# shuaigroup/Renormalizer

Measured on AMD Instinct MI355X. Metric: TDVP-PS sweep site-updates/sec at (Nsite=50, Dbond=256, dphys=2/16), higher is better.
Workload: dtype c128

## Files before the change

### renormalizer_amd/csrc/mpse_cholqr.hip

```cpp
#include <type_traits>

#include "mpse_device.h"
#include "mpse_internal.h"

typedef double v4d __attribute__((ext_vector_type(4)));

namespace {

struct CqBlk {
  long long ws_off;
  long long part_off;
  long long t_off;
  long long row_off, col_off;
  int mm, nn, P, T;
  int nchunk, rpc;
  int koff, pad;
};

__device__ __forceinline__ v4d mfma(double a, double b, v4d c) {
  return __builtin_amdgcn_mfma_f64_16x16x4f64(a, b, c, 0, 0, 0);
}
__device__ __forceinline__ double readlane_d(double v, int l) {
  const int lo = __builtin_amdgcn_readlane(__double2loint(v), l);
  const int hi = __builtin_amdgcn_readlane(__double2hiint(v), l);
// ... 487 lines not shown
        }
        ar[s][r] = gr;
        ai[s][r] = gi;
      }
    }
  }
  int bad = 0;
  for (int p = 0; p < P; ++p) {
    const int buf = p & 1;
#pragma unroll
    for (int s = 0; s < NS; ++s)
      if (tq[s] == p) {
#pragma unroll
        for (int r = 0; r < 4; ++r) sRow[buf][tc[s] - p][(kq + 4 * r) * 16 + x] = make_double2(ar[s][r], ai[s][r]);
      }
    __syncthreads();
    int badp = 0;
    panel_eliminate<CPLX>(sRow[buf], 16 * (P - p), p, P, nn, Rt, sDinv, last, tid, &badp, dyn ? sThr + 16 * p : nullptr);
    if (badp) bad = 1;
    __syncthreads();
#pragma unroll
    for (int s = 0; s < NS; ++s)
      if (tq[s] > p) {
        const double2* ta = sRow[buf][tq[s] - p];
        const double2* tb = sRow[buf][tc[s] - p];
#pragma unroll
        for (int kk = 0; kk < 4; ++kk) {
          const double2 xv = ta[(4 * kk + kq) * 16 + x], yv = tb[(4 * kk + kq) * 16 + x];
          ar[s] = mfma(-xv.x, yv.x, ar[s]);
          if constexpr (CPLX) {
            ar[s] = mfma(-xv.y, yv.y, ar[s]);
            ai[s] = mfma(-xv.x, yv.y, ai[s]);
            ai[s] = mfma(xv.y, yv.x, ai[s]);
          }
        }
      }
  }
  if (bad) {
    atomicOr(status, 1);
    if (gflag) atomicOr(gflag, 1);
  }
}

template <bool CPLX>
__global__ __launch_bounds__(256) void k_cq_trsm(double* __restrict__ ws, const double* __restrict__ R,
                                                  const double* __restrict__ Rprev, double* __restrict__ Rout,
                                                  const CqBlk* __restrict__ blks, const int* __restrict__ status, int nrb_max,
                                                  int rmul, const int* __restrict__ done) {
  constexpr int E = CPLX ? 2 : 1;
  if (done && done[blockIdx.y]) return;
  const CqBlk B = blks[blockIdx.y];
  const int tid = threadIdx.x, lane = tid & 63, wave = __builtin_amdgcn_readfirstlane(tid >> 6), x = lane & 15, kq = lane >> 4;
  const int P = B.P, nn = B.nn;
  const double* Rt = R + B.t_off * 256 * E;
  __shared__ double sXr[2][16 * 17], sXi[2][16 * 17];
  __shared__ double2 sAcc[4][256];
  if ((int)blockIdx.x >= nrb_max) {
    if (!rmul) return;
    const int t = (int)blockIdx.x - nrb_max;
    if (t >= B.T) return;
    int q, c;
    tile_decode(t, P, q, c);
    const double* Rp = Rprev + B.t_off * 256 * E;
    v4d ar = {0, 0, 0, 0}, ai = {0, 0, 0, 0};
    for (int s = q + wave; s <= c; s += 4) {
      const double* ta = Rt + (long long)tile_index(q, s, P) * 256 * E;
      const double* tb = Rp + (long long)tile_index(s, c, P) * 256 * E;
#pragma unroll
      for (int kk = 0; kk < 4; ++kk) {
        double xr, xi, yr, yi;
        ld2<CPLX>(ta, x * 16 + 4 * kk + kq, xr, xi);
        ld2<CPLX>(tb, (4 * kk + kq) * 16 + x, yr, yi);
        ar = mfma(xr, yr, ar);
        if constexpr (CPLX) {
          ar = mfma(-xi, yi, ar);
          ai = mfma(xr, yi, ai);
          ai = mfma(xi, yr, ai);
        }
      }
    }
#pragma unroll
    for (int r = 0; r < 4; ++r) sAcc[wave][(kq + 4 * r) * 16 + x] = make_double2(ar[r], ai[r]);
    __syncthreads();
    double2 v = sAcc[0][tid];
#pragma unroll
    for (int w = 1; w < 4; ++w) {
      v.x += sAcc[w][tid].x;
      v.y += sAcc[w][tid].y;
    }
    st2<CPLX>(Rout + B.t_off * 256 * E, (long long)t * 256 + tid, v.x, v.y);
    return;
  }
  const int r0 = 16 * blockIdx.x;
  if (r0 >= B.mm) return;
  double* A = ws + B.ws_off * E;
  const long long mm = B.mm;
  const int mode = status[1 + blockIdx.y];
  v4d ar[4], ai[4];
#pragma unroll
  for (int s = 0; s < 4; ++s) {
    const int p = wave + 4 * s;
    ar[s] = v4d{0, 0, 0, 0};
    ai[s] = v4d{0, 0, 0, 0};
    if (p < P) {
      const int col = min(16 * p + x, nn - 1);
#pragma unroll
      for (int r = 0; r < 4; ++r) {
        const int row = min(r0 + kq + 4 * r, B.mm - 1);
        double vr, vi;
        ld2<CPLX>(A, (long long)col * mm + row, vr, vi);
        ar[s][r] = vr;
        ai[s][r] = vi;
      }
    }
  }
  asm volatile("" ::: "memory");
#pragma unroll
  for (int s = 0; s < 4; ++s) {
    const int p = wave + 4 * s;
    if (p < P) {
#pragma unroll
      for (int r = 0; r < 4; ++r)
        if (!(r0 + kq + 4 * r < B.mm && 16 * p + x < nn)) ar[s][r] = ai[s][r] = 0.0;
    }
  }
  auto store_panel = [&](int p, const v4d& vr, const v4d& vi) {
    const int col = 16 * p + x;
    if (col < nn) {
#pragma unroll
      for (int r = 0; r < 4; ++r) {
        const int row = r0 + kq + 4 * r;
        if (row < B.mm) st2<CPLX>(A, (long long)col * mm + row, vr[r], vi[r]);
      }
    }
  };
  if (mode == 1) {
    const int arow = min(r0 + x, B.mm - 1);
    const bool rok = r0 + x < B.mm;
#pragma unroll
    for (int s = 0; s < 4; ++s) {
      const int p = wave + 4 * s;
      if (p >= P) break;
      for (int q = 0; q <= p; ++q) {
        const double* tb = Rt + (long long)tile_index(q, p, P) * 256 * E;
#pragma unroll
        for (int kk = 0; kk < 4; ++kk) {
          const int acol = 16 * q + 4 * kk + kq;
          double xr = 0.0, xi = 0.0, yr, yi;
          ld2<CPLX>(A, (long long)min(acol, nn - 1) * mm + arow, xr, xi);
          if (!(rok && acol < nn)) xr = xi = 0.0;
          ld2<CPLX>(tb, (4 * kk + kq) * 16 + x, yr, yi);
          if (q == p && 4 * kk + kq == x) yr -= 1.0;
          ar[s] = mfma(-xr, yr, ar[s]);
          if constexpr (CPLX) {
            ar[s] = mfma(xi, yi, ar[s]);
            ai[s] = mfma(-xr, yi, ai[s]);
            ai[s] = mfma(-xi, yr, ai[s]);
          }
        }
      }
    }
    __syncthreads();
#pragma unroll
    for (int s = 0; s < 4; ++s)
      if (wave + 4 * s < P) store_panel(wave + 4 * s, ar[s], ai[s]);
    return;
  }
  double rr[16], ri[16];
  auto load_rcol = [&](int q) {
    const double* td = Rt + (long long)tile_index(q, q, P) * 256 * E;
#pragma unroll
    for (int t = 0; t < 16; ++t) ld2<CPLX>(td, t * 16 + x, rr[t], ri[t]);
  };
  for (int q = 0; q < P; ++q) {
    const int owner = q & 3, slot = q >> 2, buf = q & 1;
    if (wave == owner) {
      load_rcol(q);
      asm volatile("" ::: "memory");
      double dj = rr[0];
#pragma unroll
      for (int t = 1; t < 16; ++t) dj = x == t ? rr[t] : dj;
      const double dinv = fast_rcp(dj);
#pragma unroll
      for (int t = 0; t < 16; ++t) {
        if (t >= x) rr[t] = ri[t] = 0.0;
      }
      v4d vr, vi;
      vr = slot == 0 ? ar[0] : slot == 1 ? ar[1] : slot == 2 ? ar[2] : ar[3];
      vi = slot == 0 ? ai[0] : slot == 1 ? ai[1] : slot == 2 ? ai[2] : ai[3];
      auto step = [&](auto tc) {
        constexpr int t = decltype(tc)::value;
        const double dt = row_share<t>(dinv);
#pragma unroll
        for (int r = 0; r < 4; ++r) {
          const double br = row_share<t>(vr[r]) * dt;
          const double bi = CPLX ? row_share<t>(vi[r]) * dt : 0.0;
          vr[r] -= br * rr[t] - bi * ri[t];
          if constexpr (CPLX) vi[r] -= br * ri[t] + bi * rr[t];
        }
      };
      step(std::integral_constant<int, 0>{});
      step(std::integral_constant<int, 1>{});
      step(std::integral_constant<int, 2>{});
      step(std::integral_constant<int, 3>{});
      step(std::integral_constant<int, 4>{});
      step(std::integral_constant<int, 5>{});
      step(std::integral_constant<int, 6>{});
      step(std::integral_constant<int, 7>{});
      step(std::integral_constant<int, 8>{});
      step(std::integral_constant<int, 9>{});
      step(std::integral_constant<int, 10>{});
      step(std::integral_constant<int, 11>{});
      step(std::integral_constant<int, 12>{});
      step(std::integral_constant<int, 13>{});
      step(std::integral_constant<int, 14>{});
#pragma unroll
      for (int r = 0; r < 4; ++r) {
        vr[r] *= dinv;
        vi[r] *= dinv;
      }
#pragma unroll
      for (int r = 0; r < 4; ++r) {
        sXr[buf][(kq + 4 * r) * 17 + x] = vr[r];
        sXi[buf][(kq + 4 * r) * 17 + x] = vi[r];
      }
      store_panel(q, vr, vi);
    }
    lds_barrier();
#pragma unroll
    for (int s = 0; s < 4; ++s) {
      const int p = wave + 4 * s;
      if (p > q && p < P) {
        const double* tb = Rt + (long long)tile_index(q, p, P) * 256 * E;
        double yr[4], yi[4];
#pragma unroll
        for (int kk = 0; kk < 4; ++kk) ld2<CPLX>(tb, (4 * kk + kq) * 16 + x, yr[kk], yi[kk]);
        asm volatile("" ::: "memory");
#pragma unroll
        for (int kk = 0; kk < 4; ++kk) {
          const double xr = sXr[buf][x * 17 + 4 * kk + kq], xi = sXi[buf][x * 17 + 4 * kk + kq];
          ar[s] = mfma(-xr, yr[kk], ar[s]);
          if constexpr (CPLX) {
            ar[s] = mfma(xi, yi[kk], ar[s]);
            ai[s] = mfma(-xr, yi[kk], ai[s]);
            ai[s] = mfma(-xi, yr[kk], ai[s]);
          }
        }
      }
    }
  }
}

template <bool CPLX>
__global__ void k_cq_scatter(double* U, double* Vt, const double* __restrict__ ws, const double* __restrict__ R,
                             const double* __restrict__ R2, long long K,
                             long long ncol, const long long* __restrict__ drows, const long long* __restrict__ dcols,
                             const CqBlk* __restrict__ blks, int herm, const int* __restrict__ status, double* dstat,
                             const int* __restrict__ done, int* __restrict__ words) {
  constexpr int E = CPLX ? 2 : 1;
  const CqBlk B = blks[blockIdx.y];
  if (blockIdx.x == 0 && blockIdx.y == 0 && threadIdx.x == 0) {
    dstat[0] = (double)status[0];
    int n2 = 0;
    for (int b = 0; b < (int)gridDim.y; ++b) n2 += done[b] != 0;
    dstat[1] = (double)n2;
    if (words) {
      atomicAdd(words + 2, (int)gridDim.y);
      atomicAdd(words + 3, n2);
    }
  }
  const double* q = ws + B.ws_off * E;
  const double* Rt = (done[blockIdx.y] ? R2 : R) + B.t_off * 256 * E;
  const long long* rows = drows + B.row_off;
  const long long* cols = dcols + B.col_off;
  const int mm = B.mm, nn = B.nn, k = B.nn;
  const long long koff = B.koff;
  const long long tq = (long long)mm * k, total = tq + (long long)k * nn;
  const long long stride = (long long)gridDim.x * blockDim.x;
  for (long long t = (long long)blockIdx.x * blockDim.x + threadIdx.x; t < total; t += stride) {
    if (t < tq) {
      double vr, vi;
      if (!herm) {
        const int c = (int)(t % k), r = (int)(t / k);
        ld2<CPLX>(q, r + (long long)c * mm, vr, vi);
        st2<CPLX>(U, rows[r] * K + koff + c, vr, vi);
      } else {
        const int r = (int)(t % mm), c = (int)(t / mm);
        ld2<CPLX>(q, r + (long long)c * mm, vr, vi);
        st2<CPLX>(Vt, (koff + c) * ncol + cols[r], vr, -vi);
      }
    } else {
      const long long u = t - tq;
      const int c = (int)(u % nn), i = (int)(u / nn);
      double vr = 0.0, vi = 0.0;
      if (i <= c) ld2<CPLX>(Rt, (long long)tile_index(i >> 4, c >> 4, B.P) * 256 + (i & 15) * 16 + (c & 15), vr, vi);
      if (!herm)
        st2<CPLX>(Vt, (koff + i) * ncol + cols[c], vr, vi);
      else
        st2<CPLX>(U, rows[c] * K + koff + i, vr, -vi);
    }
  }
}

template <bool CPLX>
int cholqr_run(mpse_ctx* ctx, double* ws, const QrBlk* blks, int nblk, const long long* drows, const long long* dcols,
               int herm, void* U, void* Vt, long long K, long long ncol, bool* ok) {
  MPSE_TRY(qr_words(ctx));
  int* gflag = ctx->qr_optimistic ? ctx->qr_words_dev : nullptr;
  constexpr size_t es = CPLX ? 16 : 8;
  std::vector<CqBlk> cb(nblk);
  long long part_tot = 0, t_tot = 0;
  int max_gram = 1, max_T = 1, max_nrb = 1, max_P = 1;
  long long max_sc = 1;
  long long groups = 0;
  for (int b = 0; b < nblk; ++b) {
    const int P2 = ((blks[b].nn + 15) / 16 + 1) / 2;
    groups += P2 * (P2 + 1) / 2;
  }
  for (int b = 0; b < nblk; ++b) {
    CqBlk& c = cb[b];
    c.ws_off = blks[b].ws_off;
    c.mm = blks[b].mm;
    c.nn = blks[b].nn;
    c.P = (c.nn + 15) / 16;
    c.T = c.P * (c.P + 1) / 2;
    c.row_off = blks[b].row_off;
    c.col_off = blks[b].col_off;
    c.koff = blks[b].prm_off;
    c.pad = 0;
    int want = (int)((8LL * ctx->n_cu + groups - 1) / groups);
    if (want < 1) want = 1;
    if (want > 64) want = 64;
    int rpc = (c.mm + want - 1) / want;
    if (rpc < 32) rpc = 32;
    rpc = (rpc + 3) & ~3;
    c.rpc = rpc;
    c.nchunk = (c.mm + rpc - 1) / rpc;
    c.part_off = part_tot;
    c.t_off = t_tot;
    part_tot += (long long)((c.nchunk + 3) / 4) * c.T * 256;
    t_tot += c.T;
    {
      const int P2 = (c.P + 1) / 2, T2 = P2 * (P2 + 1) / 2;
      max_gram = std::max(max_gram, ((c.nchunk + 3) / 4) * T2);
    }
    max_T = std::max(max_T, c.T);
    max_P = std::max(max_P, c.P);
    max_nrb = std::max(max_nrb, (c.mm + 15) / 16);
    max_sc = std::max<long long>(max_sc, (long long)c.mm * c.nn + (long long)c.nn * c.nn);
  }
  const size_t db = (size_t(nblk) * sizeof(CqBlk) + 15) & ~size_t(15);
  const size_t pb = size_t(part_tot) * es, tb = size_t(t_tot) * 256 * es, ib = size_t(t_tot) * 2 * sizeof(double);
  const size_t sb = ((2 * size_t(nblk) + 1) * sizeof(int) + 15) & ~size_t(15);
  TmpBuf M(ctx);
  MPSE_TRY(M.alloc(db + pb + 6 * tb + ib + sb + 16));
  char* base = static_cast<char*>(M.p);
  MPSE_TRY(stage_h2d(ctx, base, cb.data(), size_t(nblk) * sizeof(CqBlk)));
  const CqBlk* dblk = reinterpret_cast<const CqBlk*>(base);
  double* part = reinterpret_cast<double*>(base + db);
  double* G = reinterpret_cast<double*>(base + db + pb);
  double* Rb[5];
  for (int i = 0; i < 5; ++i) Rb[i] = reinterpret_cast<double*>(base + db + pb + (1 + i) * tb);
  double* tinfo = reinterpret_cast<double*>(base + db + pb + 6 * tb);
  int* status = reinterpret_cast<int*>(base + db + pb + 6 * tb + ib);
  const int* done = status + 1 + nblk;
  double* dstat = reinterpret_cast<double*>(base + db + pb + 6 * tb + ib + sb);
  static const double theta = [] {
    const char* e = getenv("MPSE_CHOLQR_THETA");
    return e ? atof(e) : 1e-12;
  }();
  static const double tau = [] {
    const char* e = getenv("MPSE_CHOLQR_TAU");
    return e ? atof(e) : 0.1;
  }();
  const double* racc = nullptr;
  for (int pass = 1; pass <= 3; ++pass) {
    double* Rcur = Rb[pass - 1];
    const int* dn = pass == 3 ? done : nullptr;
    hipLaunchKernelGGL((k_cq_gram<CPLX>), dim3(max_gram, nblk), dim3(256), 0, ctx->stream, (const double*)ws, part, dblk,
                       status, pass == 1 ? 2 * nblk + 1 : 0, dn);
    hipLaunchKernelGGL((k_cq_reduce<CPLX>), dim3(max_T, nblk), dim3(256), 0, ctx->stream, (const double*)part, G, tinfo, dblk,
                       dn);
    if (max_P <= 10)
      hipLaunchKernelGGL((k_cq_chol_rl<CPLX>), dim3(nblk), dim3(512), 0, ctx->stream, (const double*)G,
                         (const double*)tinfo, Rcur, dblk, status, pass, gflag, nblk, theta, tau);
    else
      hipLaunchKernelGGL((k_cq_chol<CPLX>), dim3(nblk), dim3(512), 0, ctx->stream, (const double*)G, (const double*)tinfo,
                         Rcur, dblk, status, pass, gflag, nblk, theta, tau);
    double* Rout = pass == 2 ? Rb[3] : Rb[4];
    const int rmul = pass >= 2 ? 1 : 0;
    const dim3 tg(max_nrb + (rmul ? max_T : 0), nblk);
    hipLaunchKernelGGL((k_cq_trsm<CPLX>), tg, dim3(256), 0, ctx->stream, ws, (const double*)Rcur, racc, Rout, dblk,
                       (const int*)status, max_nrb, rmul, dn);
    racc = pass == 1 ? Rcur : Rout;
  }
  int nb = (int)((max_sc + 255) / 256);
  if (nb > 8192) nb = 8192;
  hipLaunchKernelGGL((k_cq_scatter<CPLX>), dim3(nb, nblk), dim3(256), 0, ctx->stream, (double*)U, (double*)Vt, (const double*)ws,
                     (const double*)Rb[4], (const double*)Rb[3], K, ncol, drows, dcols, dblk, herm, (const int*)status, dstat,
                     done, ctx->qr_words_dev);
  MPSE_HIP(ctx, hipGetLastError());
  if (gflag) {
    *ok = true;
    return MPSE_OK;
  }
  MPSE_TRY(publish_and_wait(ctx, dstat, 1, mpse_ctx::PIN_QR_STATUS));
  *ok = ctx->pinned[mpse_ctx::PIN_QR_STATUS] == 0.0;
  return MPSE_OK;
}

}

bool cholqr_eligible(const mpse_ctx* ctx, const QrBlk* blks, int nblk) {
  static const int env_mode = [] {
    const char* e = getenv("MPSE_CHOLQR");
    return e ? atoi(e) : 1;
  }();
  const int mode = ctx->qr_scheme >= 0 ? ctx->qr_scheme : env_mode;
  static const int min_rows = [] {
    const char* e = getenv("MPSE_CHOLQR_MINROWS");
    return e ? atoi(e) : 256;
  }();
  if (mode == 0 || nblk <= 0) return false;
  int max_mm = 0, max_nn = 0;
  for (int b = 0; b < nblk; ++b) {
    if (blks[b].mm < blks[b].nn || blks[b].k != blks[b].nn || blks[b].nn > 256) return false;
    max_mm = std::max(max_mm, blks[b].mm);
    max_nn = std::max(max_nn, blks[b].nn);
  }
  if (mode >= 2) return true;
  return max_mm >= min_rows && max_nn >= 96;
}

int cholqr_blocks(mpse_ctx* ctx, bool cplx, double* ws, const QrBlk* blks, int nblk, const long long* drows,
                  const long long* dcols, int herm, void* U, void* Vt, long long K, long long ncol, bool* ok) {
  *ok = false;
  if (cplx) return cholqr_run<true>(ctx, ws, blks, nblk, drows, dcols, herm, U, Vt, K, ncol, ok);
  return cholqr_run<false>(ctx, ws, blks, nblk, drows, dcols, herm, U, Vt, K, ncol, ok);
}
```

### renormalizer_amd/csrc/mpse_core.hip

```cpp
#include "mpse_internal.h"
#include "mpse_plans.h"

int mpse_fail(mpse_ctx* ctx, int code, const char* fmt, ...) {
  if (ctx) {
    va_list ap;
    va_start(ap, fmt);
    vsnprintf(ctx->err, sizeof(ctx->err), fmt, ap);
    va_end(ap);
  }
  return code;
}

__global__ __launch_bounds__(256) void k_zero8(unsigned long long* dst, long long n) {
  for (long long i = (long long)blockIdx.x * 256 + threadIdx.x; i < n; i += (long long)gridDim.x * 256) dst[i] = 0ull;
}
__global__ __launch_bounds__(256) void k_copy8(unsigned long long* dst, const unsigned long long* __restrict__ src,
                                               long long n) {
  for (long long i = (long long)blockIdx.x * 256 + threadIdx.x; i < n; i += (long long)gridDim.x * 256) dst[i] = src[i];
}

__global__ __launch_bounds__(256) void k_zero8x2(unsigned long long* a, long long na, unsigned long long* b, long long nb) {
  for (long long i = (long long)blockIdx.x * 256 + threadIdx.x; i < na + nb; i += (long long)gridDim.x * 256) {
    if (i < na)
      a[i] = 0ull;
    else
      b[i - na] = 0ull;
  }
}

int device_zero2(mpse_ctx* ctx, void* a, size_t abytes, void* b, size_t bbytes) {
  if (((reinterpret_cast<uintptr_t>(a) | reinterpret_cast<uintptr_t>(b) | abytes | bbytes) & 7) != 0 || !abytes || !bbytes) {
    MPSE_TRY(device_zero(ctx, a, abytes));
    return device_zero(ctx, b, bbytes);
  }
  const long long na = (long long)(abytes / 8), nb = (long long)(bbytes / 8);
  long long blocks = (na + nb + 255) / 256;
  if (blocks > 2048) blocks = 2048;
  hipLaunchKernelGGL(k_zero8x2, dim3((unsigned)blocks), dim3(256), 0, ctx->stream, static_cast<unsigned long long*>(a), na,
                     static_cast<unsigned long long*>(b), nb);
  MPSE_HIP(ctx, hipGetLastError());
  return MPSE_OK;
}

int device_zero(mpse_ctx* ctx, void* dst, size_t bytes) {
  if (!bytes) return MPSE_OK;
  if ((reinterpret_cast<uintptr_t>(dst) & 7) == 0 && (bytes & 7) == 0) {
    const long long n = (long long)(bytes / 8);
    long long blocks = (n + 255) / 256;
    if (blocks > 2048) blocks = 2048;
    hipLaunchKernelGGL(k_zero8, dim3((unsigned)blocks), dim3(256), 0, ctx->stream, static_cast<unsigned long long*>(dst), n);
    MPSE_HIP(ctx, hipGetLastError());
    return MPSE_OK;
  }
  MPSE_HIP(ctx, hipMemsetAsync(dst, 0, bytes, ctx->stream));
  return MPSE_OK;
}

int stage_h2d(mpse_ctx* ctx, void* dst, const void* src_host, size_t bytes) {
  if (!bytes) return MPSE_OK;
  if (!ctx->stage || bytes > ctx->stage_size / 4) return mpse_memcpy_h2d(ctx, dst, src_host, bytes);
  const size_t need = (bytes + 255) & ~size_t(255);
  if (ctx->stage_pos + need > ctx->stage_size) {
    MPSE_HIP(ctx, hipStreamSynchronize(ctx->stream));
    ctx->stage_pos = 0;
  }
  char* slot = ctx->stage + ctx->stage_pos;
  memcpy(slot, src_host, bytes);
  if (ctx->stage_dev && (reinterpret_cast<uintptr_t>(dst) & 7) == 0 && (bytes & 7) == 0 && bytes <= (size_t(1) << 20)) {
    const size_t words = bytes / 8;
    ctx->stage_pos += need;
    __sync_synchronize();
    long long blocks = (long long)((words + 255) / 256);
    if (blocks > 256) blocks = 256;
    hipLaunchKernelGGL(k_copy8, dim3((unsigned)blocks), dim3(256), 0, ctx->stream, static_cast<unsigned long long*>(dst),
                       reinterpret_cast<const unsigned long long*>(ctx->stage_dev + (slot - ctx->stage)),
                       (long long)words);
    MPSE_HIP(ctx, hipGetLastError());
    return MPSE_OK;
  }
  ctx->stage_pos += need;
  MPSE_HIP(ctx, hipMemcpyAsync(dst, slot, bytes, hipMemcpyHostToDevice, ctx->stream));
  return MPSE_OK;
}

void prof_drain(mpse_ctx* ctx) {
  for (auto& r : ctx->prof_pending) {
    float ms = 0.f;
    if (hipEventElapsedTime(&ms, r.e0, r.e1) == hipSuccess) {
      ctx->prof_ms[r.variant] += ms;
      ctx->prof_flops[r.variant] += r.flops;
      ctx->prof_bytes[r.variant] += r.bytes;
      ctx->prof_launches[r.variant] += 1;
    }
    ctx->prof_free_events.push_back(r.e0);
    ctx->prof_free_events.push_back(r.e1);
  }
  ctx->prof_pending.clear();
}

bool prof_begin(mpse_ctx* ctx, int variant, double flops, double bytes, mpse_ctx::ProfRec* rec) {
  if (!ctx->prof_on || (variant != 6 && ctx->prof_counter++ % ctx->prof_stride != 0)) return false;
  auto get_event = [&](hipEvent_t* e) {
    if (!ctx->prof_free_events.empty()) {
      *e = ctx->prof_free_events.back();
      ctx->prof_free_events.pop_back();
      return true;
    }
    return hipEventCreate(e) == hipSuccess;
  };
  if (!get_event(&rec->e0)) return false;
  if (!get_event(&rec->e1)) {
    ctx->prof_free_events.push_back(rec->e0);
    return false;
  }
  rec->variant = variant;
  rec->flops = flops;
  rec->bytes = bytes;
  if (hipEventRecord(rec->e0, ctx->stream) != hipSuccess) {
    ctx->prof_free_events.push_back(rec->e0);
    ctx->prof_free_events.push_back(rec->e1);
    return false;
  }
  return true;
}

void prof_end(mpse_ctx* ctx, const mpse_ctx::ProfRec& rec) {
  (void)hipEventRecord(rec.e1, ctx->stream);
  ctx->prof_pending.push_back(rec);
}

namespace {
__global__ void k_copy16(double2* __restrict__ dst, const double2* __restrict__ src, long long n) {
  const long long stride = (long long)gridDim.x * blockDim.x;
  for (long long i = (long long)blockIdx.x * blockDim.x + threadIdx.x; i < n; i += stride) dst[i] = src[i];
}
}

static void defer_update_hold(mpse_ctx* ctx) {
  const bool hold = ctx->defer_recording >= 0 || !ctx->defer_ops[0].empty() || !ctx->defer_ops[1].empty();
  std::lock_guard<std::mutex> lock(ctx->pool_mu);
  ctx->defer_hold = hold;
  if (hold) return;
  for (void* p : ctx->defer_frees) {
    auto it = ctx->live.find(p);
    if (it == ctx->live.end()) continue;
    ctx->free_blocks.emplace(it->second, p);
    ctx->in_use_bytes -= it->second;
    ctx->live.erase(it);
  }
  ctx->defer_frees.clear();
}

int defer_replay(mpse_ctx* ctx, int status) {
  const int list = ctx->defer_armed;
  if (list < 0) return status;
  ctx->defer_armed = -1;
  std::vector<std::function<int()>> ops;
  ops.swap(ctx->defer_ops[list]);
  if (status == MPSE_OK)
    for (auto& f : ops) {
      status = f();
      if (status != MPSE_OK) break;
    }
  ops.clear();
  defer_update_hold(ctx);
  return status;
}

extern "C" {

int mpse_prof_enable(mpse_ctx* ctx, int on) {
  if (!ctx) return MPSE_ERR_ARG;
  MPSE_HIP(ctx, hipStreamSynchronize(ctx->stream));
  prof_drain(ctx);
  ctx->prof_on = on != 0;
  ctx->prof_stride = on > 1 ? on : 1;
  ctx->prof_counter = 0;
  return MPSE_OK;
}

int mpse_prof_reset(mpse_ctx* ctx) {
  if (!ctx) return MPSE_ERR_ARG;
  MPSE_HIP(ctx, hipStreamSynchronize(ctx->stream));
  prof_drain(ctx);
  for (int i = 0; i < mpse_ctx::PROF_NVAR; ++i) {
    ctx->prof_ms[i] = ctx->prof_flops[i] = ctx->prof_bytes[i] = 0;
    ctx->prof_launches[i] = 0;
  }
  ctx->prof_svd_sweeps = 0;
  if (ctx->prof_ktiles) {
    MPSE_HIP(ctx, hipMemsetAsync(ctx->prof_ktiles, 0, 4 * sizeof(unsigned long long), ctx->stream));
    MPSE_HIP(ctx, hipStreamSynchronize(ctx->stream));
  }
  return MPSE_OK;
}

int mpse_prof_get_ktiles(mpse_ctx* ctx, int variant, int64_t* ktiles) {
  if (!ctx || !ktiles || variant < 0 || variant > 3) return MPSE_ERR_ARG;
  MPSE_BIND(ctx);
  *ktiles = 0;
  if (!ctx->prof_ktiles) return MPSE_OK;
  unsigned long long v[4];
  MPSE_HIP(ctx, hipMemcpyAsync(v, ctx->prof_ktiles, sizeof(v), hipMemcpyDeviceToHost, ctx->stream));
  MPSE_HIP(ctx, hipStreamSynchronize(ctx->stream));
  *ktiles = (int64_t)v[variant];
  return MPSE_OK;
}

int mpse_prof_get_svd_sweeps(mpse_ctx* ctx, int64_t* sweeps) {
  if (!ctx || !sweeps) return MPSE_ERR_ARG;
  *sweeps = ctx->prof_svd_sweeps;
  return MPSE_OK;
}

int mpse_prof_get(mpse_ctx* ctx, int variant, double* total_ms, double* total_flops, double* total_bytes,
                  int64_t* launches) {
  if (!ctx || variant < 0 || variant >= mpse_ctx::PROF_NVAR) return MPSE_ERR_ARG;
  MPSE_HIP(ctx, hipStreamSynchronize(ctx->stream));
  prof_drain(ctx);
  if (variant == 0 && ctx->gemm_trace) {
    const char* path = getenv("MPSE_GEMM_TRACE");
    unsigned long long n = 0;
    if (path && hipMemcpy(&n, ctx->gemm_trace, sizeof(n), hipMemcpyDeviceToHost) == hipSuccess) {
      if (n > GEMM_TRACE_CAP) n = GEMM_TRACE_CAP;
      std::vector<unsigned long long> rec(size_t(n) * GEMM_TRACE_WORDS);
      if (n && hipMemcpy(rec.data(), ctx->gemm_trace + 1, rec.size() * sizeof(unsigned long long), hipMemcpyDeviceToHost) == hipSuccess) {
        if (FILE* fh = fopen(path, "wb")) {
          fwrite(rec.data(), sizeof(unsigned long long), rec.size(), fh);
          fclose(fh);
        }
      }
    }
  }
  if (total_ms) *total_ms = ctx->prof_ms[variant];
  if (total_flops) *total_flops = ctx->prof_flops[variant];
  if (total_bytes) *total_bytes = ctx->prof_bytes[variant];
  if (launches) *launches = ctx->prof_launches[variant];
  return MPSE_OK;
}

const char* mpse_version(void) { return "mpsengine 0.1 (gfx950)"; }

const char* mpse_last_error(const mpse_ctx* ctx) { return ctx ? ctx->err : "null context"; }

int mpse_ctx_create(int device, mpse_ctx** out) {
  if (!out) return MPSE_ERR_ARG;
  *out = nullptr;
  int ndev = 0;
  if (hipGetDeviceCount(&ndev) != hipSuccess || ndev <= 0) return MPSE_ERR_HIP;
  if (device < 0 || device >= ndev) return MPSE_ERR_ARG;
  mpse_ctx* ctx = new mpse_ctx();
  ctx->device = device;
  if (hipSetDevice(device) != hipSuccess) {
    delete ctx;
    return MPSE_ERR_HIP;
  }
  hipDeviceProp_t prop;
  if (hipGetDeviceProperties(&prop, device) == hipSuccess) {
    ctx->n_cu = prop.multiProcessorCount;
    if (ctx->n_cu > 0) mpse_plan::fold_cus() = ctx->n_cu;
    snprintf(ctx->dev_name, sizeof(ctx->dev_name), "%s (%s)", prop.name, prop.gcnArchName);
  }
  if (hipStreamCreateWithFlags(&ctx->stream, hipStreamNonBlocking) != hipSuccess ||
      hipHostMalloc((void**)&ctx->pinned, mpse_ctx::PIN_DOUBLES * sizeof(double)) != hipSuccess ||
      hipMalloc((void**)&ctx->dscratch, (size_t(1) << 16) * sizeof(double)) != hipSuccess ||
      hipMalloc((void**)&ctx->prof_ktiles, 4 * sizeof(unsigned long long)) != hipSuccess ||
      hipHostMalloc((void**)&ctx->stage, size_t(8) << 20) != hipSuccess) {
    delete ctx;
    return MPSE_ERR_HIP;
  }
  (void)hipMemsetAsync(ctx->dscratch + (size_t(1) << 16) - 8, 0, 8 * sizeof(double), ctx->stream);
  (void)hipMemsetAsync(ctx->prof_ktiles, 0, 4 * sizeof(unsigned long long), ctx->stream);
  (void)hipStreamSynchronize(ctx->stream);
  const char* pin_map = getenv("MPSE_PINNED_MAP");
  if ((pin_map && pin_map[0] == '0') || hipHostGetDevicePointer((void**)&ctx->pinned_dev, ctx->pinned, 0) != hipSuccess)
    ctx->pinned_dev = nullptr;
  {
    if (hipHostGetDevicePointer((void**)&ctx->stage_dev, ctx->stage, 0) != hipSuccess)
      ctx->stage_dev = nullptr;
    (void)hipGetLastError();
  }
  ctx->pinned[mpse_ctx::PIN_SEQ] = 0.0;
  ctx->stage_size = size_t(8) << 20;
  *out = ctx;
  return MPSE_OK;
}

static int pool_trim_locked(mpse_ctx* ctx) {
  MPSE_HIP(ctx, hipStreamSynchronize(ctx->stream));
  for (auto& kv : ctx->free_blocks) {
    (void)hipFree(kv.second);
    ctx->pool_bytes -= kv.first;
  }
  ctx->free_blocks.clear();
  return MPSE_OK;
}

int mpse_pool_trim(mpse_ctx* ctx) {
  if (!ctx) return MPSE_ERR_ARG;
  MPSE_BIND(ctx);
  std::lock_guard<std::mutex> lock(ctx->pool_mu);
  return pool_trim_locked(ctx);
}

int mpse_ctx_destroy(mpse_ctx* ctx) {
  if (!ctx) return MPSE_ERR_ARG;
  (void)hipSetDevice(ctx->device);
  (void)hipStreamSynchronize(ctx->stream);
  prof_drain(ctx);
  for (auto e : ctx->prof_free_events) (void)hipEventDestroy(e);
  for (auto& kv : ctx->free_blocks) (void)hipFree(kv.second);
  for (auto& kv : ctx->live) (void)hipFree(kv.first);
  if (ctx->pinned) (void)hipHostFree(ctx->pinned);
  if (ctx->stage) (void)hipHostFree(ctx->stage);
  if (ctx->dscratch) (void)hipFree(ctx->dscratch);
  if (ctx->prof_ktiles) (void)hipFree(ctx->prof_ktiles);
  if (ctx->stream) (void)hipStreamDestroy(ctx->stream);
  delete ctx;
  return MPSE_OK;
}

int mpse_sync(mpse_ctx* ctx) {
  if (!ctx) return MPSE_ERR_ARG;
  MPSE_BIND(ctx);
  MPSE_HIP(ctx, hipStreamSynchronize(ctx->stream));
  if (!ctx->prof_pending.empty()) prof_drain(ctx);
  return MPSE_OK;
}

int mpse_device_info(mpse_ctx* ctx, char* name, size_t name_len, int* n_cu, void** stream) {
  if (!ctx) return MPSE_ERR_ARG;
  if (name && name_len) snprintf(name, name_len, "%s", ctx->dev_name);
  if (n_cu) *n_cu = ctx->n_cu;
  if (stream) *stream = (void*)ctx->stream;
  return MPSE_OK;
}

static size_t bucket_of(size_t bytes) {
  if (bytes < 256) return 256;
  if (bytes <= (size_t(1) << 20)) return (bytes + 255) & ~size_t(255);
  size_t p = size_t(1) << 20;
  while ((p << 1) <= bytes) p <<= 1;
  size_t step = p >> 3;
  return ((bytes + step - 1) / step) * step;
}

int mpse_malloc(mpse_ctx* ctx, size_t bytes, void** dptr) {
  if (!ctx || !dptr) return MPSE_ERR_ARG;
  MPSE_BIND(ctx);
  std::lock_guard<std::mutex> lock(ctx->pool_mu);
  size_t b = bucket_of(bytes);
  auto it = ctx->free_blocks.find(b);
  void* p = nullptr;
  if (it != ctx->free_blocks.end()) {
    p = it->second;
    ctx->free_blocks.erase(it);
  } else {
    hipError_t e = hipMalloc(&p, b);
    ++ctx->n_device_allocs;
    if (e != hipSuccess) {
      (void)hipGetLastError();
      pool_trim_locked(ctx);
      e = hipMalloc(&p, b);
      if (e != hipSuccess) {
        (void)hipGetLastError();
        *dptr = nullptr;
        return mpse_fail(ctx, MPSE_ERR_OOM, "hipMalloc(%zu) failed: %s (pool %zu B, in use %zu B)", b,
                         hipGetErrorString(e), ctx->pool_bytes, ctx->in_use_bytes);
      }
    }
    ctx->pool_bytes += b;
  }
  ctx->live[p] = b;
  ctx->in_use_bytes += b;
  *dptr = p;
  return MPSE_OK;
}

int mpse_free(mpse_ctx* ctx, void* dptr) {
  if (!ctx) return MPSE_ERR_ARG;
  if (!dptr) return MPSE_OK;
  std::lock_guard<std::mutex> lock(ctx->pool_mu);
  auto it = ctx->live.find(dptr);
  if (it == ctx->live.end()) return mpse_fail(ctx, MPSE_ERR_ARG, "mpse_free: unknown pointer %p", dptr);
  if (!ctx->wsite_info.empty()) ctx->wsite_info.erase(dptr);
  if (ctx->defer_hold) {
    ctx->defer_frees.push_back(dptr);
    return MPSE_OK;
  }
  ctx->free_blocks.emplace(it->second, dptr);
  ctx->in_use_bytes -= it->second;
  ctx->live.erase(it);
  return MPSE_OK;
}


int mpse_defer_begin(mpse_ctx* ctx, int list) {
  if (!ctx || list < 0 || list > 1) return MPSE_ERR_ARG;
  if (ctx->defer_recording >= 0) return mpse_fail(ctx, MPSE_ERR_ARG, "mpse_defer_begin: already recording");
  if (ctx->defer_armed == list) return mpse_fail(ctx, MPSE_ERR_ARG, "mpse_defer_begin: list %d is armed", list);
  ctx->defer_ops[list].clear();
  ctx->defer_recording = list;
  defer_update_hold(ctx);
  return MPSE_OK;
}

int mpse_defer_end(mpse_ctx* ctx) {
  if (!ctx) return MPSE_ERR_ARG;
  if (ctx->defer_recording < 0) return mpse_fail(ctx, MPSE_ERR_ARG, "mpse_defer_end: not recording");
  ctx->defer_recording = -1;
  defer_update_hold(ctx);
  return MPSE_OK;
}

int mpse_defer_arm(mpse_ctx* ctx, int list) {
  if (!ctx || list < 0 || list > 1) return MPSE_ERR_ARG;
  if (ctx->defer_recording >= 0) return mpse_fail(ctx, MPSE_ERR_ARG, "mpse_defer_arm: still recording");
  ctx->defer_armed = list;
  return MPSE_OK;
}

int mpse_defer_discard(mpse_ctx* ctx) {
  if (!ctx) return MPSE_ERR_ARG;
  ctx->defer_ops[0].clear();
  ctx->defer_ops[1].clear();
  ctx->defer_recording = ctx->defer_armed = -1;
  defer_update_hold(ctx);
  return MPSE_OK;
}

int mpse_defer_run(mpse_ctx* ctx, int list) {
  if (!ctx || list < 0 || list > 1) return MPSE_ERR_ARG;
  if (ctx->defer_recording >= 0) return mpse_fail(ctx, MPSE_ERR_ARG, "mpse_defer_run: still recording");
  MPSE_BIND(ctx);
  ctx->defer_armed = list;
  return defer_replay(ctx, MPSE_OK);
}


int mpse_mem_info(mpse_ctx* ctx, size_t* pool_bytes, size_t* in_use_bytes, size_t* device_free,
                  size_t* device_total) {
  if (!ctx) return MPSE_ERR_ARG;
  MPSE_BIND(ctx);
  if (pool_bytes) *pool_bytes = ctx->pool_bytes;
  if (in_use_bytes) *in_use_bytes = ctx->in_use_bytes;
  size_t f = 0, t = 0;
  MPSE_HIP(ctx, hipMemGetInfo(&f, &t));
  if (device_free) *device_free = f;
  if (device_total) *device_total = t;
  return MPSE_OK;
}

int mpse_memcpy_h2d(mpse_ctx* ctx, void* dst, const void* src_host, size_t bytes) {
  if (!ctx || (bytes && (!dst || !src_host))) return MPSE_ERR_ARG;
  MPSE_BIND(ctx);
  if (!bytes) return MPSE_OK;
  wsite_written(ctx, dst, bytes);
  MPSE_HIP(ctx, hipMemcpyAsync(dst, src_host, bytes, hipMemcpyHostToDevice, ctx->stream));
  MPSE_HIP(ctx, hipStreamSynchronize(ctx->stream));
  return MPSE_OK;
}

int mpse_memcpy_d2h(mpse_ctx* ctx, void* dst_host, const void* src, size_t bytes) {
  if (!ctx || (bytes && (!dst_host || !src))) return MPSE_ERR_ARG;
  MPSE_BIND(ctx);
  if (!bytes) return MPSE_OK;
  MPSE_HIP(ctx, hipMemcpyAsync(dst_host, src, bytes, hipMemcpyDeviceToHost, ctx->stream));
  MPSE_HIP(ctx, hipStreamSynchronize(ctx->stream));
  return MPSE_OK;
}

int mpse_memcpy_d2d(mpse_ctx* ctx, void* dst, const void* src, size_t bytes) {
  if (!ctx || (bytes && (!dst || !src))) return MPSE_ERR_ARG;
  MPSE_BIND(ctx);
  if (!bytes) return MPSE_OK;
  wsite_written(ctx, dst, bytes);
  if (((reinterpret_cast<uintptr_t>(dst) | reinterpret_cast<uintptr_t>(src)) & 15) == 0 && (bytes & 15) == 0) {
    const size_t n = bytes / 16;
    size_t blocks = (n + 255) / 256;
    if (blocks > 4096) blocks = 4096;
    hipLaunchKernelGGL(k_copy16, dim3((unsigned)blocks), dim3(256), 0, ctx->stream, reinterpret_cast<double2*>(dst),
                       reinterpret_cast<const double2*>(src), (long long)n);
    MPSE_HIP(ctx, hipGetLastError());
    return MPSE_OK;
  }
  MPSE_HIP(ctx, hipMemcpyAsync(dst, src, bytes, hipMemcpyDeviceToDevice, ctx->stream));
  return MPSE_OK;
}

int mpse_memcpy_2d(mpse_ctx* ctx, void* dst, size_t dpitch, const void* src, size_t spitch, size_t width_bytes,
                   size_t height) {
  if (!ctx || ((width_bytes && height) && (!dst || !src))) return MPSE_ERR_ARG;
  MPSE_BIND(ctx);
  if (!width_bytes || !height) return MPSE_OK;
  wsite_written(ctx, dst, dpitch * (height - 1) + width_bytes);
  MPSE_HIP(ctx, hipMemcpy2DAsync(dst, dpitch, src, spitch, width_bytes, height, hipMemcpyDeviceToDevice, ctx->stream));
  return MPSE_OK;
}

int mpse_memset_zero(mpse_ctx* ctx, void* dst, size_t bytes) {
  if (!ctx || (bytes && !dst)) return MPSE_ERR_ARG;
  MPSE_BIND(ctx);
  wsite_written(ctx, dst, bytes);
  return device_zero(ctx, dst, bytes);
}

}

namespace {
__global__ void k_publish(const double* __restrict__ src, double* dst, int count, volatile double* seq_slot, double seq) {
  for (int i = threadIdx.x; i < count; i += blockDim.x) dst[i] = src[i];
  __threadfence_system();
  __syncthreads();
  if (threadIdx.x == 0) {
    *seq_slot = seq;
    __threadfence_system();
  }
}
}

int publish_wait_seq(mpse_ctx* ctx, double seq, const double* dsrc, int count, int slot) {
  volatile double* flag = ctx->pinned + mpse_ctx::PIN_SEQ;
  for (long long spins = 0; *flag != seq; ++spins) {
    if (spins > 2000000000LL || ((spins & 0xfffff) == 0xfffff && hipStreamQuery(ctx->stream) == hipSuccess && *flag != seq)) {
      MPSE_HIP(ctx, hipStreamSynchronize(ctx->stream));
      MPSE_HIP(ctx, hipMemcpy(ctx->pinned + slot, dsrc, size_t(count) * sizeof(double), hipMemcpyDeviceToHost));
      return MPSE_OK;
    }
  }
  __sync_synchronize();
  return MPSE_OK;
}

PublishAt publish_target(mpse_ctx* ctx, bool wait_here, int slot) {
  if (!wait_here || !ctx->pinned_dev) return PublishAt{nullptr, nullptr, 0.0};
  return PublishAt{ctx->pinned_dev + slot, ctx->pinned_dev + mpse_ctx::PIN_SEQ, double(++ctx->publish_seq)};
}

static int publish_wait(mpse_ctx* ctx, const PublishAt& at, const void* dsrc, size_t stride, int B, int W, int slot) {
  if (at.seq != 0.0) {
    MPSE_TRY(publish_wait_seq(ctx, at.seq, static_cast<const double*>(dsrc), W, slot));
    if (B == 1 || ctx->pinned[mpse_ctx::PIN_SEQ] == at.seq) return MPSE_OK;
  }
  const size_t row = size_t(W) * sizeof(double);
  if (B == 1)
    MPSE_HIP(ctx, hipMemcpyAsync(ctx->pinned + slot, dsrc, row, hipMemcpyDeviceToHost, ctx->stream));
  else
    MPSE_HIP(ctx, hipMemcpy2DAsync(ctx->pinned + slot, row, dsrc, stride, row, size_t(B), hipMemcpyDeviceToHost, ctx->stream));
  MPSE_HIP(ctx, hipStreamSynchronize(ctx->stream));
  return MPSE_OK;
}

int publish_collect(mpse_ctx* ctx, const PublishAt& at, const void* dsrc, size_t stride, int B, int W, int slot,
                    void* host_out) {
  MPSE_TRY(publish_wait(ctx, at, dsrc, stride, B, W, slot));
  if (ctx->prof_pending.size() > 2048) prof_drain(ctx);
  memcpy(host_out, ctx->pinned + slot, size_t(B) * W * sizeof(double));
  return MPSE_OK;
}

int publish_and_wait(mpse_ctx* ctx, const double* dsrc, int count, int slot) {
  if (count < 0 || count > 1024 || slot < 0 || slot + count > mpse_ctx::PIN_SLOTS_END)
    return mpse_fail(ctx, MPSE_ERR_ARG, "publish: range");
  const PublishAt at = publish_target(ctx, true, slot);
  if (at.pub) {
    hipLaunchKernelGGL(k_publish, dim3(1), dim3(64), 0, ctx->stream, dsrc, at.pub, count, at.seq_slot, at.seq);
    MPSE_HIP(ctx, hipGetLastError());
  }
  return publish_wait(ctx, at, dsrc, 0, 1, count, slot);
}
```

### renormalizer_amd/csrc/mpse_gemm.hip

```cpp
#include <cstdlib>

#include "mpse_device.h"
#include "mpse_internal.h"
#include "mpse_plans.h"

typedef double v4d __attribute__((ext_vector_type(4)));

static unsigned long long* gemm_trace_ptr(const mpse_ctx* ctx) {
  static const bool f0_only = [] {
    const char* e = getenv("MPSE_GEMM_TRACE_ONLY");
    return e && e[0] == 'f';
  }();
  return (ctx->prof_on && !f0_only) ? ctx->gemm_trace : nullptr;
}

namespace {

struct IdxMap {
  long long s_hi, s_lo;
  int ext, lo;
};

constexpr int GMAX_GRP = 8, GMAX_SEG = 4, GMAX_MIX = 8;
struct GMix {
// ... 597 lines not shown
  int kt_done = 0;
  if constexpr (KS && MPSE_GEMM_PIPE) {
    int nk = kt_end;
    if (kt < kt_end) {
      stage_to_lds(0);
      nk = next_kt(kt + 1);
      if (nk < kt_end) {
        load_tile(nk);
      }
      lds_barrier();
      if (g.trace) tr2 = __builtin_readcyclecounter();
      read_frag(0, 0);
    }
    const bool any = kt < kt_end;
    while (nk < kt_end) {
      ++kt_done;
      read_frag(1, 1);
      mfma_group(0);
      read_frag(0, 2);
      mfma_group(1);
      read_frag(1, 3);
      mfma_group(0);
      lds_barrier();
      mfma_group_staging(1);
      const int after = next_kt(nk + 1);
      if (after < kt_end) load_tile(after);
      kt = nk;
      nk = after;
      lds_barrier();
      read_frag(0, 0);
    }
    if (any) {
      ++kt_done;
      read_frag(1, 1);
      mfma_group(0);
      read_frag(0, 2);
      mfma_group(1);
      read_frag(1, 3);
      mfma_group(0);
      mfma_group(1);
    }
  } else {
  while (kt < kt_end) {
    ++kt_done;
    __syncthreads();
    if (g.trace && kt_done == 1) tr2 = __builtin_readcyclecounter();
    stage_to_lds(0);
    __syncthreads();
    const int nk = next_kt(kt + 1);
    if (nk < kt_end) {
      load_tile(nk);
    }
    kt = nk;

    read_frag(0, 0);
#pragma unroll
    for (int kk = 0; kk < BK / 4; ++kk) {
      const int cb = kk & 1;
      if (kk + 1 < BK / 4) read_frag(cb ^ 1, kk + 1);
      mfma_group(cb);
    }
  }
  }

  if (g.trace) tr3 = __builtin_readcyclecounter();
  struct TraceEnd {
    const GemmArgs& g;
    unsigned long long t0, rt0, &t1, &t2, &t3;
    int tid;
    int& ktd;
    __device__ ~TraceEnd() {
      if (g.trace && tid == 0) trace_record(g, CA, CB, t0, rt0, t1, t2, t3, ktd);
    }
  } trace_end{g, tr0, rt0, tr1, tr2, tr3, tid, kt_done};
  if (g.kt_counter && tid == 0 && kt_done) atomicAdd(g.kt_counter, (unsigned long long)kt_done);
  if constexpr (M3) {
#pragma unroll
    for (int i = 0; i < WI; ++i)
#pragma unroll
      for (int j = 0; j < 2; ++j) {
        acc_im[i][j] = acc_im[i][j] - acc_re[i][j] - acc_t2[i][j];
        acc_re[i][j] = acc_re[i][j] - acc_t2[i][j];
      }
  }
  if (g.ksplit > 1) {
    double* wsb = g.ws + (long long)bs * g.M * g.N * EC;
#pragma unroll
    for (int j = 0; j < 2; ++j) {
      const int gj = tn * TBN + wn * 32 + j * 16 + (lane & 15);
      if (gj >= g.N) continue;
#pragma unroll
      for (int i = 0; i < WI; ++i)
#pragma unroll
        for (int r = 0; r < 4; ++r) {
          const int gi = tm * TBM + wm * WROWS + i * 16 + (lane >> 4) + 4 * r;
          if (gi >= g.M) continue;
          double* p = wsb + ((long long)gi * g.N + gj) * EC;
          if constexpr (CC)
            *reinterpret_cast<double2*>(p) = make_double2(acc_re[i][j][r], acc_im[i][j][r]);
          else
            *p = acc_re[i][j][r];
        }
    }
    return;
  }
  double dre = 0.0, dim = 0.0;
  constexpr bool PRE = CA && CB;
  double2 pre_c[PRE ? WI : 1][2][4], pre_y[PRE ? WI : 1][2][4];
  const bool need_c = GRP ? (gp.use_beta != 0 && half == 0) : g.use_beta != 0, need_y = g.dot_y != nullptr;
  bool mix_on = false;
  if constexpr (GRP && PRE) mix_on = need_c && g.gg.nmix > 0 && grp == g.gg.mix_grp;
  if constexpr (GRP && PRE) {
    if (mix_on) {
      const int d = g.gg.mix_d;
      __syncthreads();
      for (int x = tid; x < g.gg.nmix * BM; x += NT) {
        const GMix& m = g.gg.mix[x / BM];
        const int sg = (x % BM) % d, e = sg + m.delta;
        double w = 0.0;
        if (e >= 0 && e < d) w = g.gg.mix_w[(((long long)m.b * d + sg) * d + e) * g.gg.mix_wr + m.f];
        smem[x] = w;
      }
      __syncthreads();
#pragma unroll
      for (int j = 0; j < 2; ++j)
#pragma unroll
        for (int i = 0; i < WI; ++i)
#pragma unroll
          for (int r = 0; r < 4; ++r) pre_c[i][j][r] = make_double2(0.0, 0.0);
      for (int t = 0; t < g.gg.nmix; ++t) {
        const double* src = g.gg.mix[t].src;
        const int delta = g.gg.mix[t].delta;
        double2 v[WI][2][4];
#pragma unroll
        for (int j = 0; j < 2; ++j) {
          const int gj = min(tn * TBN + wn * 32 + j * 16 + (lane & 15), g.N - 1);
#pragma unroll
          for (int i = 0; i < WI; ++i)
#pragma unroll
            for (int r = 0; r < 4; ++r) {
              const int gi = tm * TBM + wm * WROWS + i * 16 + (lane >> 4) + 4 * r + delta;
              const int gc = min(max(gi, 0), g.M - 1);
              v[i][j][r] = *reinterpret_cast<const double2*>(src + ((long long)gc * g.gg.mix_ld + gj) * 2);
            }
        }
#pragma unroll
        for (int i = 0; i < WI; ++i)
#pragma unroll
          for (int r = 0; r < 4; ++r) {
            const double w = smem[t * BM + wm * WROWS + i * 16 + (lane >> 4) + 4 * r];
#pragma unroll
            for (int j = 0; j < 2; ++j) {
              pre_c[i][j][r].x = w != 0.0 ? fma(w, v[i][j][r].x, pre_c[i][j][r].x) : pre_c[i][j][r].x;
              pre_c[i][j][r].y = w != 0.0 ? fma(w, v[i][j][r].y, pre_c[i][j][r].y) : pre_c[i][j][r].y;
            }
          }
      }
    }
  }
  if (PRE && (need_c || need_y)) {
#pragma unroll
    for (int j = 0; j < 2; ++j) {
      const int gj = min(tn * TBN + wn * 32 + j * 16 + (lane & 15), g.N - 1);
      const long long coffn = idx_off(g.nC, gj);
      const long long cinn = g.Cin ? idx_off(g.nCin, gj) : 0;
#pragma unroll
      for (int i = 0; i < WI; ++i)
#pragma unroll
        for (int r = 0; r < 4; ++r) {
          const int gi = min(tm * TBM + wm * WROWS + i * 16 + (lane >> 4) + 4 * r, g.M - 1);
          const long long co = idx_off(g.mC, gi) + coffn;
          if (need_c && !mix_on) {
            const double* pin = g.Cin ? g.Cin + (idx_off(g.mCin, gi) + cinn) * EC : C + co * EC;
            if constexpr (CC)
              pre_c[i][j][r] = *reinterpret_cast<const double2*>(pin);
            else
              pre_c[i][j][r] = make_double2(*pin, 0.0);
          }
          if (need_y) {
            if constexpr (CC)
              pre_y[i][j][r] = reinterpret_cast<const double2*>(g.dot_y)[co];
            else
              pre_y[i][j][r] = make_double2(g.dot_y[co], 0.0);
          }
        }
    }
  }
  constexpr bool HAND = GRP && PRE && WI == 1;
  bool hand = false;
  auto hslot = [&]() { return smem + 1024 + (((wm >> 1) * 2 + wn) * 64 + lane) * 2; };
  if constexpr (HAND) {
    hand = g.gg.dot4 != 0 && need_y;
    if (hand) __syncthreads();
  }
#pragma unroll
  for (int j = 0; j < 2; ++j) {
    const int gj = tn * TBN + wn * 32 + j * 16 + (lane & 15);
    if (gj >= g.N) continue;
    if constexpr (HAND) {
      if (hand) {
        if (wm & 1) __syncthreads();
        if ((wm & 1) || j > 0) dre = hslot()[0], dim = hslot()[1];
      }
    }
    const long long coffn = idx_off(g.nC, gj);
#pragma unroll
    for (int i = 0; i < WI; ++i) {
#pragma unroll
      for (int r = 0; r < 4; ++r) {
        const int gi = tm * TBM + wm * WROWS + i * 16 + (lane >> 4) + 4 * r;
        if (gi >= g.M) continue;
        const long long co = idx_off(g.mC, gi) + coffn;
        double* p = C + co * EC;
        const double xr = acc_re[i][j][r];
        if constexpr (CC) {
          const double xi = acc_im[i][j][r];
          double2 o;
          o.x = g.alpha_re * xr - g.alpha_im * xi;
          o.y = g.alpha_re * xi + g.alpha_im * xr;
          if (need_c) {
            double2 c0;
            if constexpr (PRE)
              c0 = pre_c[i][j][r];
            else
              c0 = *reinterpret_cast<const double2*>(g.Cin ? g.Cin + (idx_off(g.mCin, gi) + idx_off(g.nCin, gj)) * EC : C + co * EC);
            o.x += g.beta_re * c0.x - g.beta_im * c0.y;
            o.y += g.beta_re * c0.y + g.beta_im * c0.x;
          }
          *reinterpret_cast<double2*>(p) = o;
          if (need_y) {
            if constexpr (PRE)
              dot_acc(dre, dim, o, pre_y[i][j][r]);
            else
              dot_acc(dre, dim, o, reinterpret_cast<const double2*>(g.dot_y)[co]);
          }
        } else {
          double o = g.alpha_re * xr;
          if (need_c) o += g.beta_re * (g.Cin ? g.Cin[idx_off(g.mCin, gi) + idx_off(g.nCin, gj)] : *p);
          *p = o;
          if (need_y) dre += o * g.dot_y[co];
        }
      }
    }
    if constexpr (HAND) {
      if (hand) {
        if (!((wm & 1) && j == 1)) hslot()[0] = dre, hslot()[1] = dim;
        if (!(wm & 1)) {
          __syncthreads();
          if (j == 0) __syncthreads();
        } else if (j == 0) {
          __syncthreads();
        }
      }
    }
  }
  if constexpr (HAND) {
    if (hand && !(wm & 1)) dre = dim = 0.0;
  }
  if constexpr (WS == 2) {
    if (g.dot_y) {
      __shared__ double s_dot[2 * (NT / 64)];
      dre = wave_sum(dre);
      dim = wave_sum(dim);
      if (lane == 0) {
        s_dot[2 * wave] = dre;
        s_dot[2 * wave + 1] = dim;
      }
      __syncthreads();
      dre = dim = 0.0;
#pragma unroll
      for (int w = 0; w < NT / 64; ++w) {
        dre += s_dot[2 * w];
        dim += s_dot[2 * w + 1];
      }
      if (tid == 0) {
        const long long slot = (long long)bs * ntile + (long long)tm * g.tiles_n + tn;
        g.dot_part[2 * slot] = dre;
        g.dot_part[2 * slot + 1] = dim;
      }
    }
  }
}

__device__ __forceinline__ void bitonic_desc(unsigned* key, int tid, int n) {
  for (int size = 2; size <= n; size <<= 1)
    for (int stride = size >> 1; stride > 0; stride >>= 1) {
      if (tid < (n >> 1)) {
        const int lo = 2 * tid - (tid & (stride - 1)), hi = lo + stride;
        const bool desc = (lo & size) == 0;
        const unsigned a = key[lo], b = key[hi];
        if ((a < b) == desc) {
          key[lo] = b;
          key[hi] = a;
        }
      }
      __syncthreads();
    }
}
__device__ __forceinline__ int pow2_at_least(int x) {
  int n = 2;
  while (n < x) n <<= 1;
  return n;
}
__global__ __launch_bounds__(1024) void k_tile_order(const unsigned long long* __restrict__ amask,
                                                       const unsigned long long* __restrict__ bmask, int nkw, int nkt,
                                                       int tiles_m, int tiles_n, int by_die, int* __restrict__ perm,
                                                       const int* __restrict__ skip, const GemmGroups gg,
                                                       unsigned char* __restrict__ flags_out, int flags_pitch,
                                                       int om_M, int om_N) {
  if (skip && *skip) return;
  __shared__ unsigned key[2048], ckey[2048];
  __shared__ int colw[2048];
  __shared__ unsigned char die_of[2048], dead[2048];
  const int ntile = tiles_m * tiles_n, tid = threadIdx.x;
  const bool part = by_die && tiles_n % 8 == 0 && tiles_n <= 2048;
  for (int c = tid; c < 2048; c += 1024) colw[c] = 0;
  __syncthreads();
  for (int i = tid; i < 2048; i += 1024) {
    unsigned cnt = 0;
    dead[i] = 0;
    if (i < ntile) {
      const int tm = i / tiles_n, tn = i - tm * tiles_n;
      if (gg.ngrp > 0) {
        const int grp = tm / gg.tiles_m_grp, tml = tm - grp * gg.tiles_m_grp;
        const GGrp& G = gg.g[grp];
        const bool off = gg.omask && !mpse_plan::out_tile_live(gg.omask, gg.om_pitch, gg.om_d, om_N, om_M, tm, tn);
        dead[i] = off ? 1 : 0;
        for (int q = 0; q < G.nseg; ++q)
          for (int l = 0; l < gg.nkt_seg; ++l) {
            unsigned v = off ? 0 : 1;
            if (G.seg[q].am) v &= G.seg[q].am[(long long)tml * gg.am_pitch + l];
            if (G.seg[q].bm) v &= G.seg[q].bm[(long long)tn * gg.bm_pitch + l];
            cnt += v;
            if (flags_out) flags_out[(long long)i * flags_pitch + q * gg.nkt_seg + l] = (unsigned char)v;
          }
        if (flags_out)
          for (int l = G.nseg * gg.nkt_seg; l < flags_pitch; ++l) flags_out[(long long)i * flags_pitch + l] = 0;
      } else {
        for (int w = 0; w < nkw; ++w) {
          unsigned long long x = 0x0101010101010101ull;
          if (amask) x &= amask[(long long)tm * nkw + w];
          if (bmask) x &= bmask[(long long)tn * nkw + w];
          const int valid = nkt - 8 * w;
          if (valid < 8) x &= (1ull << (8 * valid)) - 1ull;
          cnt += __popcll(x);
        }
      }
      if (part) atomicAdd(&colw[tn], (int)cnt);
    }
    key[i] = cnt;
  }
  __syncthreads();
  if (part) {
    for (int c = tid; c < 2048; c += 1024) ckey[c] = c < tiles_n ? ((unsigned)colw[c] << 11) | (unsigned)(2047 - c) : 0u;
    __syncthreads();
    bitonic_desc(ckey, tid, pow2_at_least(tiles_n));
    for (int r = tid; r < tiles_n; r += 1024) {
      const int c = 2047 - (int)(ckey[r] & 2047u), r16 = r & 15;
      die_of[c] = (unsigned char)(r16 < 8 ? r16 : 15 - r16);
    }
    __syncthreads();
  }
  for (int i = tid; i < 2048; i += 1024) {
    unsigned k = 0;
    if (i < ntile) {
      const unsigned die = part ? die_of[i % tiles_n] : 0u;
      k = (die << 28) | (key[i] << 16) | (unsigned)(0xFFFF - i);
    }
    key[i] = k;
  }
  __syncthreads();
  bitonic_desc(key, tid, pow2_at_least(ntile));
  const int per_die = ntile / 8;
  for (int i = tid; i < ntile; i += 1024) {
    const int s = part ? (7 - (i & 7)) * per_die + (i >> 3) : i;
    const int t = 0xFFFF - (int)(key[s] & 0xFFFFu);
    perm[i] = dead[t] ? ~t : t;
  }
}

template <bool CC>
__global__ __launch_bounds__(256) void k_splitk_reduce(const GemmArgs g, int batch) {
  constexpr int EC = CC ? 2 : 1;
  if (g.skip && *g.skip) return;
  const long long mn = (long long)g.M * g.N;
  const int rows = g.M * batch;
  double dre = 0.0, dim = 0.0;
  for (int row = blockIdx.y; row < rows; row += gridDim.y) {
    const int b = row / g.M;
    const int i = row - b * g.M;
    const double* wrow = g.ws + ((long long)b * g.ksplit * mn + (long long)i * g.N) * EC;
    double* crow = g.C + ((long long)b * g.sbC + idx_off(g.mC, i)) * EC;
    for (int j = blockIdx.x * 256 + threadIdx.x; j < g.N; j += gridDim.x * 256) {
      const double* w = wrow + (long long)j * EC;
      double xr = 0, xi = 0;
      int s = 0;
      for (; s + 4 <= g.ksplit; s += 4) {
        if constexpr (CC) {
          const double2 v0 = *reinterpret_cast<const double2*>(w + (long long)s * mn * EC);
          const double2 v1 = *reinterpret_cast<const double2*>(w + (long long)(s + 1) * mn * EC);
          const double2 v2 = *reinterpret_cast<const double2*>(w + (long long)(s + 2) * mn * EC);
          const double2 v3 = *reinterpret_cast<const double2*>(w + (long long)(s + 3) * mn * EC);
          xr += v0.x;
          xi += v0.y;
          xr += v1.x;
          xi += v1.y;
          xr += v2.x;
          xi += v2.y;
          xr += v3.x;
          xi += v3.y;
        } else {
          const double v0 = w[(long long)s * mn], v1 = w[(long long)(s + 1) * mn];
          const double v2 = w[(long long)(s + 2) * mn], v3 = w[(long long)(s + 3) * mn];
          xr += v0;
          xr += v1;
          xr += v2;
          xr += v3;
        }
      }
      for (; s < g.ksplit; ++s) {
        if constexpr (CC) {
          const double2 v = *reinterpret_cast<const double2*>(w + (long long)s * mn * EC);
          xr += v.x;
          xi += v.y;
        } else {
          xr += w[(long long)s * mn];
        }
      }
      const long long co = idx_off(g.nC, j);
      double* p = crow + co * EC;
      const double* pin = g.Cin ? g.Cin + (idx_off(g.mCin, i) + idx_off(g.nCin, j)) * EC : p;
      if constexpr (CC) {
        double2 o = make_double2(g.alpha_re * xr - g.alpha_im * xi, g.alpha_re * xi + g.alpha_im * xr);
        if (g.use_beta) {
          const double2 c0 = *reinterpret_cast<const double2*>(pin);
          o.x += g.beta_re * c0.x - g.beta_im * c0.y;
          o.y += g.beta_re * c0.y + g.beta_im * c0.x;
        }
        *reinterpret_cast<double2*>(p) = o;
        if (g.dot_y) dot_acc(dre, dim, o, reinterpret_cast<const double2*>(g.dot_y)[idx_off(g.mC, i) + co]);
      } else {
        double o = g.alpha_re * xr;
        if (g.use_beta) o += g.beta_re * (*pin);
        *p = o;
        if (g.dot_y) dre += o * g.dot_y[idx_off(g.mC, i) + co];
      }
    }
  }
  if (g.dot_y) {
    block_allsum2(dre, dim);
    if (threadIdx.x == 0) {
      const long long bid = (long long)blockIdx.y * gridDim.x + blockIdx.x;
      g.dot_part[2 * bid] = dre;
      g.dot_part[2 * bid + 1] = dim;
    }
  }
}

struct OccOperand {
  const double* base;
  IdxMap rmap, kmap;
  int nrows, tiles, cplx, kfast;
  long long sb;
  unsigned char* flags;
};
__global__ __launch_bounds__(256) void k_tile_occ(OccOperand oa, OccOperand ob, int K, int nkw, int batch,
                                                  const int* skip) {
  if (skip && *skip) return;
  const int wave = threadIdx.x >> 6, lane = threadIdx.x & 63;
  const int kt = blockIdx.x * 4 + wave, t = blockIdx.y;
  const bool second = (int)blockIdx.z >= batch;
  const OccOperand& o = second ? ob : oa;
  const int b = second ? blockIdx.z - batch : blockIdx.z;
  if (t >= o.tiles || kt * BK >= K) return;
  const int E = o.cplx ? 2 : 1;
  const double* base = o.base + (long long)b * o.sb * E;
  bool nz = false;
  if (o.kfast) {
    const int k = kt * BK + (lane & 15);
    const bool kin = k < K;
    const long long ko = idx_off(o.kmap, kin ? k : K - 1);
    double v0[16], v1[16];
#pragma unroll
    for (int i = 0; i < 16; ++i) {
      const int r = min(t * BM + i * 4 + (lane >> 4), o.nrows - 1);
      const double* q = base + (idx_off(o.rmap, r) + ko) * E;
      v0[i] = q[0];
      v1[i] = o.cplx ? q[1] : 0.0;
    }
#pragma unroll
    for (int i = 0; i < 16; ++i) {
      const bool in = (t * BM + i * 4 + (lane >> 4)) < o.nrows && kin;
      nz |= in && (v0[i] != 0.0 || v1[i] != 0.0);
    }
  } else {
    const int r = t * BM + lane;
    if (r < o.nrows) {
      const double* p = base + idx_off(o.rmap, r) * E;
      double v0[16], v1[16];
#pragma unroll
      for (int i = 0; i < 16; ++i) {
        const int k = min(kt * BK + i, K - 1);
        const double* q = p + idx_off(o.kmap, k) * E;
        v0[i] = q[0];
        v1[i] = o.cplx ? q[1] : 0.0;
      }
#pragma unroll
      for (int i = 0; i < 16; ++i) nz |= (kt * BK + i < K) && (v0[i] != 0.0 || v1[i] != 0.0);
    }
  }
  const bool any = __ballot(nz) != 0ull;
  if (lane == 0) o.flags[((long long)b * o.tiles + t) * nkw * 8 + kt] = any ? 1 : 0;
}

bool to_map(const mpse_index& s, IdxMap* m) {
  if (s.ext < 0 || s.ext > 0x7fffffffLL) return false;
  m->ext = (int)s.ext;
  long long lo = s.lo_ext <= 0 ? 1 : s.lo_ext;
  m->s_hi = s.s_hi;
  m->s_lo = s.s_lo;
  if (lo >= s.ext) {
    m->s_hi = 0;
  } else if (lo == 1) {
    m->s_lo = s.s_hi;
    m->s_hi = 0;
    lo = s.ext;
  } else if (s.s_hi == lo * s.s_lo) {
    m->s_hi = 0;
    lo = s.ext;
  }
  if (lo >= s.ext) lo = 0x7fffffffLL;
  m->lo = (int)lo;
  return true;
}

inline bool is_single(const IdxMap& m) { return m.lo == 0x7fffffff; }

template <bool CPLX>
__global__ __launch_bounds__(256) void k_transpose_inner(double* out, const double* in, long long d0, int d1,
                                                         int d2, int conj) {
  constexpr int E = CPLX ? 2 : 1;
  __shared__ double tile[32][33 * E];
  const int tx = threadIdx.x & 31, ty = threadIdx.x >> 5;
  const int t1 = (d1 + 31) / 32, t2 = (d2 + 31) / 32;
  long long bid = blockIdx.x;
  const long long b0 = bid / ((long long)t1 * t2);
  const int rem = (int)(bid - b0 * t1 * t2);
  const int by = rem / t2, bx = rem - by * t2;
  const double* src = in + b0 * (long long)d1 * d2 * E;
  double* dst = out + b0 * (long long)d1 * d2 * E;
  for (int yy = ty; yy < 32; yy += 8) {
    int y = by * 32 + yy, x = bx * 32 + tx;
    if (y < d1 && x < d2) {
      const double* p = src + ((long long)y * d2 + x) * E;
      tile[yy][tx * E] = p[0];
      if (CPLX) tile[yy][tx * E + 1] = conj ? -p[1] : p[1];
    }
  }
  __syncthreads();
  for (int yy = ty; yy < 32; yy += 8) {
    int x = bx * 32 + yy, y = by * 32 + tx;
    if (y < d1 && x < d2) {
      double* p = dst + ((long long)x * d1 + y) * E;
      p[0] = tile[tx][yy * E];
      if (CPLX) p[1] = tile[tx][yy * E + 1];
    }
  }
}

inline int n_cu_of(const mpse_ctx* ctx) { return ctx->n_cu > 0 ? ctx->n_cu : 256; }

long long fastest(const IdxMap& m) { return m.ext <= 1 ? (long long)1 << 60 : (m.s_lo < 0 ? -m.s_lo : m.s_lo); }

bool span_ok(const IdxMap& m, const IdxMap& k, bool cplx) {
  if (m.s_hi < 0 || m.s_lo < 0 || k.s_hi < 0 || k.s_lo < 0) return false;
  auto span = [](const IdxMap& x) {
    if (x.ext <= 1) return 0.0;
    if (x.lo == 0x7fffffff) return double(x.ext - 1) * double(x.s_lo);
    return double((x.ext - 1) / x.lo) * double(x.s_hi) + double(x.lo - 1) * double(x.s_lo);
  };
  return (span(m) + span(k) + 1.0) * (cplx ? 16.0 : 8.0) < 4.0e9;
}
bool fast_ok(const GemmArgs& g, bool ca, bool cb) { return span_ok(g.mA, g.kA, ca) && span_ok(g.nB, g.kB, cb); }

bool fill_maps(GemmArgs& g, const mpse_index& ma, const mpse_index& ka, const mpse_index& kb, const mpse_index& nb,
               const mpse_index& mc, const mpse_index& nc) {
  if (!to_map(ma, &g.mA) || !to_map(ka, &g.kA) || !to_map(kb, &g.kB) || !to_map(nb, &g.nB) || !to_map(mc, &g.mC) ||
      !to_map(nc, &g.nC))
    return false;
  g.M = g.mA.ext, g.N = g.nB.ext, g.K = g.kA.ext;
  g.tiles_m = g.mtiles_m = (g.M + BM - 1) / BM;
  g.tiles_n = g.mtiles_n = (g.N + BN - 1) / BN;
  g.a_kfast = fastest(g.kA) <= fastest(g.mA);
  g.b_kfast = fastest(g.kB) <= fastest(g.nB);
  return true;
}

SolveScope::OccKey occ_key(const void* p, const IdxMap& rm, const IdxMap& km, long long sb, long long batch, bool cplx) {
  SolveScope::OccKey k;
  memset(&k, 0, sizeof(k));
  k.ptr = p;
  k.r_ext = rm.ext, k.r_lo = rm.lo, k.r_shi = rm.s_hi, k.r_slo = rm.s_lo;
  k.k_ext = km.ext, k.k_lo = km.lo, k.k_shi = km.s_hi, k.k_slo = km.s_lo;
  k.sb = sb, k.nrows = rm.ext, k.tiles = (rm.ext + BM - 1) / BM, k.nkw = ((km.ext + BK - 1) / BK + 7) / 8;
  k.batch = (int)batch, k.K = km.ext, k.cplx = cplx ? 1 : 0;
  return k;
}
size_t occ_bytes(const SolveScope::OccKey& k) { return size_t(k.batch) * k.tiles * k.nkw * 8; }

struct OccMask {
  void* mask = nullptr;
  bool scan = false;
  bool stable = true;
};
int occ_mask_source(mpse_ctx* ctx, SolveScope* keep, const SolveScope::OccKey& key, const void* given, void* tmp,
                    OccMask* m) {
  m->stable = keep || given;
  if (keep)
    for (const auto& e : keep->occ_cache)
      if (memcmp(&e.key, &key, sizeof(key)) == 0) {
        m->mask = e.mask;
        return MPSE_OK;
      }
  m->scan = !given;
  if (given) {
    m->mask = const_cast<void*>(given);
  } else if (keep) {
    MPSE_TRY(mpse_malloc(ctx, occ_bytes(key), &m->mask));
    keep->occ_cache.push_back({key, m->mask});
  } else {
    m->mask = tmp;
  }
  return MPSE_OK;
}
OccOperand occ_operand(const SolveScope::OccKey& k, const IdxMap& rm, const IdxMap& km, int kfast, const OccMask& m) {
  return OccOperand{static_cast<const double*>(k.ptr), rm, km, k.nrows, m.scan ? k.tiles : 0, k.cplx, kfast, k.sb,
                    static_cast<unsigned char*>(m.mask)};
}

int perm_source(mpse_ctx* ctx, SolveScope* keep, SolveScope::PermEntry key, size_t bytes, TmpBuf& tmp, int** perm,
                bool* sort) {
  *sort = false;
  if (keep)
    for (const auto& e : keep->perm_cache)
      if (e.amask == key.amask && e.bmask == key.bmask && e.tiles_m == key.tiles_m && e.tiles_n == key.tiles_n &&
          e.nkt == key.nkt) {
        *perm = static_cast<int*>(e.perm);
        return MPSE_OK;
      }
  *sort = true;
  if (keep) {
    MPSE_TRY(mpse_malloc(ctx, bytes, &key.perm));
    keep->perm_cache.push_back(key);
    *perm = static_cast<int*>(key.perm);
  } else {
    MPSE_TRY(tmp.alloc(bytes));
    *perm = tmp.as<int>();
  }
  return MPSE_OK;
}

void launch_gemm(mpse_ctx* ctx, const GemmArgs& g, long long nwg, bool ca, bool cb, bool fast, bool wide, bool grouped,
                 dim3 rgrid = dim3(0), int batch = 1) {
  using Kern = void (*)(const GemmArgs);
  static const Kern plain[4][3] = {
      {k_gemm<true, true, true, 2, 1>, k_gemm<true, true, true, 2>, k_gemm<true, true, false, 2>},
      {k_gemm<true, false, true, 2, 1>, k_gemm<true, false, true, 2>, k_gemm<true, false, false, 2>},
      {k_gemm<false, true, true, 2, 1>, k_gemm<false, true, true, 2>, k_gemm<false, true, false, 2>},
      {k_gemm<false, false, true, 2, 1>, k_gemm<false, false, true, 2>, k_gemm<false, false, false, 2>}};
  static void (*const reduce[2])(const GemmArgs, int) = {k_splitk_reduce<true>, k_splitk_reduce<false>};
  static const Kern groups[2][2] = {
      {k_gemm<true, true, true, 2, 1, true>, k_gemm<true, true, true, 2, 2, true>},
      {k_gemm<false, true, true, 2, 1, true>, k_gemm<false, true, true, 2, 2, true>}};
  const int form = fast && wide ? 0 : fast ? 1 : 2;
  const Kern k = grouped ? groups[ca ? 0 : 1][form] : plain[(ca ? 0 : 2) + (cb ? 0 : 1)][form];
  hipLaunchKernelGGL(k, dim3((unsigned)nwg), dim3(form == 0 ? 512 : 256), 0, ctx->stream, g);
  if (rgrid.x) hipLaunchKernelGGL(reduce[(ca || cb) ? 0 : 1], rgrid, dim3(256), 0, ctx->stream, g, batch);
}

void count_paths(long long* gp, const mpse_plan::GemmPlan& p, bool batched) {
  const bool masked = p.fast && p.masks;
  ++gp[mpse_ctx::GP_LAUNCH];
  gp[mpse_ctx::GP_GENERAL] += !p.fast;
  gp[mpse_ctx::GP_WIDE] += p.wide;
  gp[mpse_ctx::GP_SPLIT_B1] += p.ksplit > 1 && !batched;
  gp[mpse_ctx::GP_SPLIT_BN] += p.ksplit > 1 && batched;
  gp[mpse_ctx::GP_DIE1] += p.die_group == 1;
  gp[mpse_ctx::GP_DIE2] += p.die_group == 2;
  gp[mpse_ctx::GP_SKEW] += !p.order && !p.die_group;
  gp[mpse_ctx::GP_ORDER] += p.order;
  gp[mpse_ctx::GP_MASK] += masked;
  gp[mpse_ctx::GP_MASK_GLOBAL] += masked && p.nkw > 64;
}
void count_paths(long long* gp, const GroupedDesc& d) {
  ++gp[mpse_ctx::GP_GROUPED];
  gp[mpse_ctx::GP_GROUPED_SPLIT2] += d.split2;
  gp[mpse_ctx::GP_GROUPED_MIX] += d.nmix > 0;
}

}

static int gemm_impl(mpse_ctx* ctx, const mpse_gemm_desc* d, const void* A, const void* B, void* C, int skip_zero,
                     SolveScope* sc, ProductReq* rq) {
  if (!ctx || !d) return MPSE_ERR_ARG;
  MPSE_BIND(ctx);
  if ((d->dtype_a != MPSE_F64 && d->dtype_a != MPSE_C128) || (d->dtype_b != MPSE_F64 && d->dtype_b != MPSE_C128))
    return mpse_fail(ctx, MPSE_ERR_ARG, "mpse_gemm: unknown dtype");
  if (d->m_a.ext != d->m_c.ext || d->n_b.ext != d->n_c.ext || d->k_a.ext != d->k_b.ext)
    return mpse_fail(ctx, MPSE_ERR_SHAPE, "mpse_gemm: extents disagree (M %lld/%lld N %lld/%lld K %lld/%lld)",
                     (long long)d->m_a.ext, (long long)d->m_c.ext, (long long)d->n_b.ext, (long long)d->n_c.ext,
                     (long long)d->k_a.ext, (long long)d->k_b.ext);
  if (d->m_a.ext == 0 || d->n_b.ext == 0 || d->batch <= 0) return MPSE_OK;
  if (!A || !B || !C) return mpse_fail(ctx, MPSE_ERR_ARG, "mpse_gemm: null operand");
  GemmArgs g = {};
  g.A = (const double*)A;
  g.B = (const double*)B;
  g.C = (double*)C;
  if (!fill_maps(g, d->m_a, d->k_a, d->k_b, d->n_b, d->m_c, d->n_c))
    return mpse_fail(ctx, MPSE_ERR_SHAPE, "mpse_gemm: extent out of range");
  g.sbA = d->sb_a;
  g.sbB = d->sb_b;
  g.sbC = d->sb_c;
  const bool ca = d->dtype_a == MPSE_C128, cb = d->dtype_b == MPSE_C128;
  g.conjA = d->conj_a && ca;
  g.conjB = d->conj_b && cb;
  g.alpha_re = d->alpha_re;
  g.alpha_im = d->alpha_im;
  g.beta_re = d->beta_re;
  g.beta_im = d->beta_im;
  g.use_beta = (d->beta_re != 0.0 || d->beta_im != 0.0);
  if (rq && rq->cin) {
    if (d->batch != 1 || !g.use_beta || !to_map(rq->cin_m, &g.mCin) || !to_map(rq->cin_n, &g.nCin) ||
        g.mCin.ext != g.mC.ext || g.nCin.ext != g.nC.ext)
      return mpse_fail(ctx, MPSE_ERR_ARG, "mpse_gemm: beta source needs batch == 1, beta != 0 and the extents of C");
    g.Cin = static_cast<const double*>(rq->cin);
  }
  g.skip = sc ? sc->skip : nullptr;
  g.skew = 1;
  if (!ctx->gemm_trace_checked) {
    ctx->gemm_trace_checked = true;
    if (getenv("MPSE_GEMM_TRACE")) {
      void* pt = nullptr;
      if (hipMalloc(&pt, (1 + GEMM_TRACE_CAP * GEMM_TRACE_WORDS) * sizeof(unsigned long long)) == hipSuccess) {
        (void)hipMemsetAsync(pt, 0, sizeof(unsigned long long), ctx->stream);
        ctx->gemm_trace = static_cast<unsigned long long*>(pt);
      }
    }
  }
  g.trace = gemm_trace_ptr(ctx);

  MatvecReq::Dot* dot = rq ? rq->dot : nullptr;
  const bool compact = is_single(g.mC) && is_single(g.nC) && g.mC.s_lo == g.N && (g.nC.s_lo == 1 || g.N == 1);
  const bool slices = rq && rq->slices && compact && d->alpha_re == 1.0 && d->alpha_im == 0.0;
  const mpse_plan::GemmPlan p = mpse_plan::launch_plan(
      {g.M, g.N, g.K, d->batch, n_cu_of(ctx), ca, cb, skip_zero, is_single(g.kA) && is_single(g.kB), fast_ok(g, ca, cb),
       dot != nullptr, dot ? dot->cap : 0, slices, slices ? rq->slices_cap : 0, g.use_beta != 0});
  if (p.nwg > 0x7fffffffLL) return mpse_fail(ctx, MPSE_ERR_SHAPE, "mpse_gemm: grid too large");
  g.ksplit = p.ksplit;
  g.kt_per_split = p.kt_per_split;
  g.slice_fast = g.ksplit > 1 && d->batch == 1;
  g.die_group = p.die_group;
  TmpBuf WSB(ctx), MSK(ctx), PERM(ctx);
  if (p.leave_slices) {
    g.ws = static_cast<double*>(rq->slices);
    rq->slices_used = g.ksplit;
  } else if (g.ksplit > 1) {
    MPSE_TRY(WSB.alloc(p.ws_bytes));
    g.ws = WSB.as<double>();
  }
  if (p.dot_producers) {
    g.dot_y = static_cast<const double*>(dot->y);
    g.dot_part = dot->part;
    dot->nb_out = (int)p.dot_producers;
  }
  mpse_ctx::ProfRec rec;
  const int variant = (ca ? 1 : 0) + (cb ? 2 : 0);
  const double mnk = double(g.M) * double(g.N) * double(g.K) * double(d->batch);
  const bool prof_this = prof_begin(
      ctx, variant, mnk * ((ca && cb) ? 8.0 : (ca || cb) ? 4.0 : 2.0),
      double(d->batch) * (double(g.M) * g.K * (ca ? 16 : 8) + double(g.K) * g.N * (cb ? 16 : 8) +
                          double(g.M) * g.N * ((ca || cb) ? 16 : 8) * (g.use_beta ? 2 : 1)),
      &rec);
  g.kt_counter = prof_this && ctx->prof_ktiles ? ctx->prof_ktiles + variant : nullptr;

  OccMask ma, mb;
  if (p.masks) {
    g.nkw = p.nkw;
    const bool sa = skip_zero & 1, sb = skip_zero & 2;
    const SolveScope::OccKey ka = occ_key(g.A, g.mA, g.kA, g.sbA, d->batch, ca);
    const SolveScope::OccKey kb = occ_key(g.B, g.nB, g.kB, g.sbB, d->batch, cb);
    SolveScope* const keep_a = sa && sc && sc->in_env(g.A) ? sc : nullptr;
    SolveScope* const keep_b = sb && sc && sc->in_env(g.B) ? sc : nullptr;
    const void* centre = (sb && sc && sc->in_krylov(g.B) && d->batch == 1 && (long long)occ_bytes(kb) == sc->cmask.bytes)
                             ? sc->cmask.ptr : nullptr;
    const size_t tmp_a = sa && !keep_a ? occ_bytes(ka) : 0, tmp_b = sb && !keep_b && !centre ? occ_bytes(kb) : 0;
    if (tmp_a + tmp_b) MPSE_TRY(MSK.alloc(tmp_a + tmp_b));
    if (sa) MPSE_TRY(occ_mask_source(ctx, keep_a, ka, nullptr, MSK.p, &ma));
    if (sb) MPSE_TRY(occ_mask_source(ctx, keep_b, kb, centre, MSK.as<char>() + tmp_a, &mb));
    if (ma.scan || mb.scan) {
      const OccOperand oa = occ_operand(ka, g.mA, g.kA, g.a_kfast, ma), ob = occ_operand(kb, g.nB, g.kB, g.b_kfast, mb);
      const dim3 og((p.nkt + 3) / 4, oa.tiles > ob.tiles ? oa.tiles : ob.tiles, (unsigned)(2 * d->batch));
      hipLaunchKernelGGL(k_tile_occ, og, dim3(256), 0, ctx->stream, oa, ob, g.K, g.nkw, (int)d->batch, g.skip);
    }
    g.amask = static_cast<const unsigned long long*>(ma.mask);
    g.bmask = static_cast<const unsigned long long*>(mb.mask);
  }

  if (p.order) {
    SolveScope* const keep = sc && sc->keeps_env_masks && ma.stable && mb.stable ? sc : nullptr;
    int* pp = nullptr;
    bool sort = false;
    MPSE_TRY(perm_source(ctx, keep, {g.amask, g.bmask, g.tiles_m, g.tiles_n, p.nkt, nullptr},
                         size_t(g.tiles_m) * g.tiles_n * sizeof(int), PERM, &pp, &sort));
    if (sort)
      hipLaunchKernelGGL(k_tile_order, dim3(1), dim3(1024), 0, ctx->stream, g.amask, g.bmask, g.nkw, p.nkt, g.tiles_m,
                         g.tiles_n, 1, pp, g.skip, GemmGroups(), (unsigned char*)nullptr, 0, 0, 0);
    g.perm = pp;
  }

  count_paths(ctx->gemm_paths, p, d->batch > 1);
  const bool reduce = g.ksplit > 1 && !p.leave_slices;
  launch_gemm(ctx, g, p.nwg, ca, cb, p.fast, p.wide, false, reduce ? dim3((unsigned)p.rgx, (unsigned)p.rgy) : dim3(0),
              (int)d->batch);
  if (prof_this) prof_end(ctx, rec);
  MPSE_HIP(ctx, hipGetLastError());
  return MPSE_OK;
}

int occ_mask_get(mpse_ctx* ctx, SolveScope* sc, const void* ptr, int dtype, mpse_index r, mpse_index k,
                 TmpBuf& tmp, const unsigned char** flags, int* pitch, bool* stable) {
  IdxMap rm, km;
  if (!to_map(r, &rm) || !to_map(k, &km) || !is_single(km))
    return mpse_fail(ctx, MPSE_ERR_SHAPE, "occupancy scan: K index must be single level");
  const SolveScope::OccKey key = occ_key(ptr, rm, km, 0, 1, dtype == MPSE_C128);
  SolveScope* const keep = sc && sc->in_env(ptr) ? sc : nullptr;
  OccMask m;
  if (!keep) MPSE_TRY(tmp.alloc(occ_bytes(key)));
  MPSE_TRY(occ_mask_source(ctx, keep, key, nullptr, tmp.p, &m));
  if (m.scan) {
    const OccOperand oa = occ_operand(key, rm, km, fastest(km) <= fastest(rm), m);
    OccOperand ob = oa;
    ob.tiles = 0;
    hipLaunchKernelGGL(k_tile_occ, dim3(((key.K + BK - 1) / BK + 3) / 4, key.tiles, 2), dim3(256), 0, ctx->stream, oa, ob,
                       key.K, key.nkw, 1, sc ? sc->skip : nullptr);
    MPSE_HIP(ctx, hipGetLastError());
  }
  *flags = static_cast<const unsigned char*>(m.mask);
  *pitch = key.nkw * 8;
  *stable = m.stable;
  return MPSE_OK;
}

static double grouped_bytes(const GroupedDesc& d, double M, double N, double K, bool ca) {
  const void* seen[3][GMAX_GRP * GMAX_SEG + GMAX_MIX];
  int n[3] = {0, 0, 0};
  auto fresh = [&](int w, const void* p) {
    for (int i = 0; i < n[w]; ++i)
      if (seen[w][i] == p) return false;
    seen[w][n[w]++] = p;
    return true;
  };
  double bytes = 0.0, betas = 0.0;
  for (int i = 0; i < d.ngrp; ++i) {
    for (int q = 0; q < d.grp[i].nseg; ++q) {
      if (fresh(0, d.grp[i].seg[q].A)) bytes += M * K * (ca ? 16.0 : 8.0);
      if (fresh(1, d.grp[i].seg[q].B)) bytes += K * N * 16.0;
    }
    bytes += M * N * 16.0;
    betas += d.grp[i].beta != 0.0 ? 1.0 : 0.0;
  }
  if (d.nmix > 0) {
    betas -= 1.0;
    const int w = (K == N && ca) ? 0 : 2;
    for (int t = 0; t < d.nmix; ++t)
      if (fresh(w, d.mix[t].src)) bytes += M * N * 16.0;
  }
  return bytes + betas * M * N * 16.0;
}

int gemm_grouped(mpse_ctx* ctx, const GroupedDesc& d, SolveScope* sc, MatvecReq::Dot* dot,
                 const MatvecReq::OutMask* om) {
  GemmArgs g = {};
  if (d.ngrp < 1 || d.ngrp > GMAX_GRP) return mpse_fail(ctx, MPSE_ERR_ARG, "grouped product: 1 .. %d groups", GMAX_GRP);
  if (!fill_maps(g, d.ma, d.ka, d.kb, d.nb, d.mc, d.nc))
    return mpse_fail(ctx, MPSE_ERR_SHAPE, "grouped product: extent out of range");
  if (g.M != g.mC.ext || g.N != g.nC.ext || g.K != g.kB.ext) return mpse_fail(ctx, MPSE_ERR_SHAPE, "grouped product: extents disagree");
  if (g.M == 0 || g.N == 0) return MPSE_OK;
  const bool ca = d.dta == MPSE_C128, cb = d.dtb == MPSE_C128;
  if (!is_single(g.kA) || !is_single(g.kB) || !fast_ok(g, ca, cb) || g.K % BK != 0 || g.K < BK ||
      (d.ngrp > 1 && g.M % BM != 0) || !cb)
    return mpse_fail(ctx, MPSE_ERR_SHAPE, "grouped product: needs single-level K indices, K a multiple of %d, group "
                     "heights a multiple of %d and a complex second operand", BK, BM);
  if (d.split2 && (d.ngrp != 1 || !d.c2 || g.M % BM != 0))
    return mpse_fail(ctx, MPSE_ERR_ARG, "grouped product: halved tiles need one group, whole tile rows and a second result");
  g.alpha_re = 1.0, g.beta_re = 1.0;
  g.ksplit = 1;
  g.skip = sc ? sc->skip : nullptr;
  g.skew = 1;
  g.trace = gemm_trace_ptr(ctx);
  GemmGroups& gg = g.gg;
  gg.ngrp = d.ngrp, gg.tiles_m_grp = g.mtiles_m, gg.nkt_seg = g.K / BK;
  gg.am_pitch = d.am_pitch, gg.bm_pitch = d.bm_pitch;
  gg.split2 = d.split2 ? 1 : 0;
  gg.C2 = static_cast<double*>(d.c2);
  gg.cpd = n_cu_of(ctx) / 8;
  int max_seg = 0;
  double segs = 0;
  bool any_mask = false, any_beta = false;
  for (int i = 0; i < d.ngrp; ++i) {
    const GroupedGrp& s = d.grp[i];
    if (s.nseg < 1 || s.nseg > GMAX_SEG || !s.C) return mpse_fail(ctx, MPSE_ERR_ARG, "grouped product: bad group");
    gg.g[i].C = static_cast<double*>(s.C);
    gg.g[i].nseg = s.nseg;
    gg.g[i].use_beta = s.beta != 0.0 ? 1 : 0;
    if (s.beta != 0.0 && s.beta != 1.0) return mpse_fail(ctx, MPSE_ERR_ARG, "grouped product: beta must be 0 or 1");
    any_beta = any_beta || s.beta != 0.0;
    for (int q = 0; q < s.nseg; ++q) {
      if (!s.seg[q].A || !s.seg[q].B) return mpse_fail(ctx, MPSE_ERR_ARG, "grouped product: null operand");
      gg.g[i].seg[q] = GSeg{static_cast<const double*>(s.seg[q].A), static_cast<const double*>(s.seg[q].B), s.seg[q].am, s.seg[q].bm};
      any_mask = any_mask || s.seg[q].am || s.seg[q].bm;
    }
    max_seg = s.nseg > max_seg ? s.nseg : max_seg;
    segs += s.nseg;
  }
  g.A = gg.g[0].seg[0].A, g.B = gg.g[0].seg[0].B, g.C = gg.g[0].C;
  g.use_beta = any_beta;
  if (d.nmix > 0) {
    if (!ca || d.nmix > GMAX_MIX || d.mix_grp < 0 || d.mix_grp >= d.ngrp || d.grp[d.mix_grp].beta != 1.0 || !d.mix_w ||
        d.mix_d < 1 || BM % d.mix_d != 0 || g.M % BM != 0 || d.mix_wr < 1 || d.mix_ld < g.N)
      return mpse_fail(ctx, MPSE_ERR_ARG, "grouped product: bad epilogue mix");
    gg.nmix = d.nmix, gg.mix_grp = d.mix_grp, gg.mix_d = d.mix_d, gg.mix_wr = d.mix_wr, gg.mix_ld = d.mix_ld;
    gg.mix_w = static_cast<const double*>(d.mix_w);
    for (int t = 0; t < d.nmix; ++t) {
      if (!d.mix[t].src || d.mix[t].delta <= -d.mix_d || d.mix[t].delta >= d.mix_d)
        return mpse_fail(ctx, MPSE_ERR_ARG, "grouped product: bad epilogue mix term");
      gg.mix[t] = GMix{static_cast<const double*>(d.mix[t].src), d.mix[t].b, d.mix[t].f, d.mix[t].delta, 0};
    }
  }

  const int nkt_max = max_seg * gg.nkt_seg;
  const long long nwg_all = (long long)((g.M + BM - 1) / BM) * g.tiles_n * (d.split2 ? 2 : 1);
  const int om_d = om && om->mask && om->row > 0 && om->row % g.N == 0 ? om->row / g.N : 0;
  const bool om_fits = om_d > 0 && d.ngrp == 1 && dot && nwg_all <= dot->cap && g.M % om_d == 0 &&
                       (g.M / om_d + 15) / 16 <= om->pitch && om->row % 64 == 0;
  const mpse_plan::GroupedPlan p =
      mpse_plan::grouped_plan(g.M, g.N, d.ngrp, nkt_max, any_mask, d.split2, ca, n_cu_of(ctx), om_fits);
  const long long ntile = (long long)p.tiles_m * p.tiles_n;
  if (ntile > 0x7fffffffLL) return mpse_fail(ctx, MPSE_ERR_SHAPE, "grouped product: grid too large");
  g.tiles_m = p.tiles_m;
  g.nkw = p.nkw;
  g.die_group = p.die_group;
  if (dot && d.ngrp == 1 && p.nwg >= 1 && p.nwg <= dot->cap) {
    g.dot_y = static_cast<const double*>(dot->y);
    g.dot_part = dot->part;
    dot->nb_out = (int)p.nwg;
  }
  const bool out_mask = om_fits && p.order && g.dot_y;
  if (out_mask) gg.omask = om->mask, gg.om_pitch = om->pitch, gg.om_d = om_d;
  mpse_ctx::ProfRec rec;
  const int variant = (ca ? 1 : 0) + (cb ? 2 : 0);
  const double mnk = double(g.M) * double(g.N) * double(g.K) * segs;
  const bool prof_this = prof_begin(ctx, variant, mnk * ((ca && cb) ? 8.0 : 4.0),
                                    grouped_bytes(d, double(g.M), double(g.N), double(g.K), ca),
                                    &rec);
  g.kt_counter = prof_this && ctx->prof_ktiles ? ctx->prof_ktiles + variant : nullptr;

  TmpBuf PERM(ctx);
  if (p.order) {
    const size_t perm_bytes = (size_t(ntile) * sizeof(int) + 7) & ~size_t(7), flag_pitch = size_t(g.nkw) * 8;
    int* pp = nullptr;
    bool sort = false;
    MPSE_TRY(perm_source(ctx, sc && sc->keeps_env_masks && d.masks_stable ? sc : nullptr,
                         {gg.g[0].seg[0].am, gg.g[0].seg[0].bm, g.tiles_m, g.tiles_n,
                          nkt_max + 1000 * d.ngrp + (out_mask ? 1000000 : 0), nullptr},
                         perm_bytes + size_t(ntile) * flag_pitch, PERM, &pp, &sort));
    if (sort)
      hipLaunchKernelGGL(k_tile_order, dim3(1), dim3(1024), 0, ctx->stream, (const unsigned long long*)nullptr,
                         (const unsigned long long*)nullptr, 0, nkt_max, g.tiles_m, g.tiles_n, d.split2 ? 0 : 1, pp,
                         g.skip, gg, reinterpret_cast<unsigned char*>(pp) + perm_bytes, (int)flag_pitch, g.M, g.N);
    g.perm = pp;
    g.gg.flags = reinterpret_cast<const unsigned long long*>(reinterpret_cast<const char*>(pp) + perm_bytes);
  }

  count_paths(ctx->gemm_paths, d);
  ctx->gemm_paths[mpse_ctx::GP_GROUPED_OUTMASK] += out_mask;
  const bool om_wide = out_mask && d.split2 && ca && !p.wide && g.N % BN == 0;
  gg.dot4 = om_wide ? 1 : 0;
  launch_gemm(ctx, g, p.nwg, ca, cb, true, p.wide || om_wide, true);
  if (prof_this) prof_end(ctx, rec);
  MPSE_HIP(ctx, hipGetLastError());
  return MPSE_OK;
}

extern "C" int mpse_gemm(mpse_ctx* ctx, const mpse_gemm_desc* d, const void* A, const void* B, void* C) {
  if (ctx && d && MPSE_RECORDING(ctx)) {
    const mpse_gemm_desc dc = *d;
    ctx->defer_ops[ctx->defer_recording].push_back([ctx, dc, A, B, C] { return mpse_gemm(ctx, &dc, A, B, C); });
    return MPSE_OK;
  }
  return gemm_impl(ctx, d, A, B, C, d ? (d->skip_zero_tiles & 3) : 0, nullptr, nullptr);
}

extern "C" int mpse_gemm_path_stats(mpse_ctx* ctx, int64_t* counts, int n) {
  if (!ctx || n < 0 || (n > 0 && !counts)) return MPSE_ERR_ARG;
  for (int i = 0; i < n && i < mpse_ctx::GP_COUNT; ++i) counts[i] = ctx->gemm_paths[i];
  return MPSE_OK;
}

int gemm_call(mpse_ctx* ctx, int dta, int dtb, int conja, int conjb, mpse_index ma, mpse_index ka, mpse_index kb,
              mpse_index nb, mpse_index mc, mpse_index nc, int64_t batch, int64_t sba, int64_t sbb, int64_t sbc,
              const void* A, const void* B, void* C, double alpha, double beta, int skip_zero, SolveScope* sc,
              ProductReq* rq) {
  mpse_gemm_desc d;
  d.dtype_a = dta;
  d.dtype_b = dtb;
  d.conj_a = conja;
  d.conj_b = conjb;
  d.m_a = ma;
  d.k_a = ka;
  d.k_b = kb;
  d.n_b = nb;
  d.m_c = mc;
  d.n_c = nc;
  d.batch = batch;
  d.sb_a = sba;
  d.sb_b = sbb;
  d.sb_c = sbc;
  d.alpha_re = alpha;
  d.alpha_im = 0.0;
  d.beta_re = beta;
  d.beta_im = 0.0;
  d.skip_zero_tiles = skip_zero;
  return gemm_impl(ctx, &d, A, B, C, skip_zero, sc, rq);
}

extern "C" int mpse_transpose_inner(mpse_ctx* ctx, int dtype, void* out, const void* in, int64_t d0, int64_t d1,
                                    int64_t d2, int conj) {
  if (!ctx) return MPSE_ERR_ARG;
  MPSE_BIND(ctx);
  if (d0 <= 0 || d1 <= 0 || d2 <= 0) return MPSE_OK;
  if (!out || !in) return MPSE_ERR_ARG;
  long long nblk = d0 * ((d1 + 31) / 32) * ((d2 + 31) / 32);
  if (nblk > 0x7fffffffLL) return mpse_fail(ctx, MPSE_ERR_SHAPE, "transpose grid too large");
  wsite_written(ctx, out, size_t(d0) * size_t(d1) * size_t(d2) * dtype_size(dtype));
  if (dtype == MPSE_C128)
    hipLaunchKernelGGL((k_transpose_inner<true>), dim3((unsigned)nblk), dim3(256), 0, ctx->stream, (double*)out,
                       (const double*)in, (long long)d0, (int)d1, (int)d2, conj);
  else
    hipLaunchKernelGGL((k_transpose_inner<false>), dim3((unsigned)nblk), dim3(256), 0, ctx->stream, (double*)out,
                       (const double*)in, (long long)d0, (int)d1, (int)d2, 0);
  MPSE_HIP(ctx, hipGetLastError());
  return MPSE_OK;
}
```

### renormalizer_amd/csrc/mpse_heff0.hip

```cpp
#include "mpse_device.h"
#include "mpse_internal.h"

typedef double v4d __attribute__((ext_vector_type(4)));

namespace {

__device__ __forceinline__ v4d mfma(double a, double b, v4d c) {
  return __builtin_amdgcn_mfma_f64_16x16x4f64(a, b, c, 0, 0, 0);
}

constexpr int F0_TMAX = 16;
struct F0Term {
  int b, e, x, pad;
  double w;
};
struct F0Info {
  int unit;
  int nt;
  unsigned long long lts;
  unsigned long long frn;
  unsigned long long cts;
  unsigned bpack, epack;
  double w[4];
};
struct F0Args {
  const double* L;
  const double* Rt;
  const double* C;
  double* parts;
  const double* y;
  double* dot_part;
  const unsigned char* FL;
  const unsigned char* FC;
  const unsigned char* FR;
  const unsigned long long* mask;
  const F0Term* terms;
  const int* nterm;
  const int* skip;
  const F0Info* info;
  long long n;
  int Dl, Dr, wl, wr, d, ntl, ntr, nkc, fc_pitch;
  unsigned long long* trace;
};

__device__ __forceinline__ void f0_transpose(double2* __restrict__ rt, const double2* __restrict__ r, int D, int w, int blk,
                                             int nblk) {
  const long long n = (long long)D * w * D;
  const long long stride = (long long)nblk * 256;
  for (long long i = (long long)blk * 256 + threadIdx.x; i < n; i += stride) {
    const int l = (int)(i % D);
    const long long bk = i / D;
    rt[i] = r[(long long)l * w * D + bk];
  }
}

__device__ __forceinline__ void f0_flags(const double2* __restrict__ E, int D, int w, int nt, unsigned char* __restrict__ F,
                                         int rt, int b) {
  __shared__ int s_f[64];
  const int row = threadIdx.x >> 4, col = threadIdx.x & 15;
  if (threadIdx.x < 64) s_f[threadIdx.x] = 0;
  __syncthreads();
  const double2* base = E + ((long long)(16 * rt + row) * w + b) * D;
  for (int ct = 0; ct < nt; ++ct) {
    const double2 v = base[16 * ct + col];
    if (v.x != 0.0 || v.y != 0.0) s_f[ct] = 1;
  }
  __syncthreads();
  if ((int)threadIdx.x < nt) F[((long long)rt * w + b) * nt + threadIdx.x] = s_f[threadIdx.x] ? 1 : 0;
}

__global__ __launch_bounds__(256) void k_f0_prepare(const double2* __restrict__ L, const double2* __restrict__ R,
                                                     double2* __restrict__ rt, unsigned char* __restrict__ FL,
                                                     unsigned char* __restrict__ FR, int Dl, int Dr, int wl, int wr, int ntl,
                                                     int ntr, const int* __restrict__ skip) {
  if (skip && *skip) return;
  int blk = blockIdx.x;
  if (blk < ntl * wl) {
    f0_flags(L, Dl, wl, ntl, FL, blk / wl, blk % wl);
    return;
  }
  blk -= ntl * wl;
  if (blk < ntr * wr) {
    f0_flags(R, Dr, wr, ntr, FR, blk / wr, blk % wr);
    return;
  }
  blk -= ntr * wr;
  f0_transpose(rt, R, Dr, wr, blk, (int)gridDim.x - ntl * wl - ntr * wr);
}

__global__ __launch_bounds__(1024) void k_f0_valid(const unsigned char* __restrict__ FL, const unsigned char* __restrict__ FC,
                                                    const unsigned char* __restrict__ FR, const F0Term* __restrict__ terms,
                                                    const int* __restrict__ nterm, int wl, int wr, int d, int ntl, int ntr,
                                                    int nkc, int fc_pitch, unsigned long long* __restrict__ mask,
                                                    const int* __restrict__ skip) {
  if (skip && *skip) return;
  __shared__ unsigned long long s1[64], s2[64];
  const int nparts = wr * nkc, tid = threadIdx.x;
  if (tid < 64) s1[tid] = s2[tid] = 0;
  __syncthreads();
  for (int t = tid; t < ntl * nparts; t += 1024) {
    const int at = t / nparts, s = t - at * nparts, f = s / nkc, kc = s - f * nkc;
    bool any = false;
    for (int q = 0; q < nterm[f]; ++q) {
      const F0Term tm = terms[f * F0_TMAX + q];
      for (int ct = 0; ct < ntl; ++ct)
        any = any || (FL[((long long)at * wl + tm.b) * ntl + ct] && (!FC || FC[(tm.e * nkc + kc) * fc_pitch + ct]));
    }
    if (any) atomicOr(&s1[at], 1ull << s);
  }
  for (int t = tid; t < ntr * nparts; t += 1024) {
    const int lt = t / nparts, s = t - lt * nparts, f = s / nkc, kc = s - f * nkc;
    bool any = false;
    for (int j = 0; j < 4; ++j) {
      const int kt = 4 * kc + j;
      if (kt < ntr) any = any || FR[((long long)lt * wr + f) * ntr + kt];
    }
    if (any) atomicOr(&s2[lt], 1ull << s);
  }
  __syncthreads();
  for (int t = tid; t < ntl * d * ntr; t += 1024) {
    const int row = t / ntr, lt = t - row * ntr;
    mask[t] = s1[row / d] & s2[lt];
  }
}

__global__ __launch_bounds__(1024) void k_f0_plan(const unsigned char* __restrict__ FL, const unsigned char* __restrict__ FC,
                                                   const unsigned char* __restrict__ FR, const F0Term* __restrict__ terms,
                                                   const int* __restrict__ nterm, int wl, int wr, int d, int ntl, int ntr,
                                                   int nkc, int fc_pitch, unsigned long long* __restrict__ mask, int n_cu,
                                                   F0Info* __restrict__ info, int compact, const int* __restrict__ skip) {
  if (skip && *skip) return;
  constexpr int WMAX = 256, MROWS = 1024;
  __shared__ unsigned long long s1[64], s2[64];
  __shared__ int hist[WMAX], start[WMAX], s_nw;
  __shared__ unsigned long long mL[MROWS], mR[MROWS], mC[64];
  __shared__ F0Term sT[16 * F0_TMAX];
  __shared__ int sNT[16];
  const int nparts = wr * nkc, tid = threadIdx.x, lane = tid & 63, wave = tid >> 6, nu = ntl * nparts * d;
  auto rows_to_masks = [&](const unsigned char* F, int nrows, int nt, int pitch, unsigned long long* out) {
    for (int r0 = wave; r0 < nrows; r0 += 64) {
      unsigned char v[4];
#pragma unroll
      for (int j = 0; j < 4; ++j) {
        const int r = r0 + 16 * j;
        v[j] = (r < nrows && lane < nt) ? F[(long long)r * pitch + lane] : (unsigned char)0;
      }
#pragma unroll
      for (int j = 0; j < 4; ++j) {
        const int r = r0 + 16 * j;
        const unsigned long long m = __ballot(v[j] != 0);
        if (r < nrows && lane == 0) out[r] = m;
      }
    }
  };
  rows_to_masks(FL, ntl * wl, ntl, ntl, mL);
  rows_to_masks(FR, ntr * wr, ntr, ntr, mR);
  if (FC) rows_to_masks(FC, d * nkc, ntl, fc_pitch, mC);
  for (int i = tid; i < wr * F0_TMAX; i += 1024) sT[i] = terms[i];
  if (tid < wr) sNT[tid] = nterm[tid];
  if (tid < 64) s1[tid] = s2[tid] = 0;
  for (int i = tid; i < WMAX; i += 1024) hist[i] = 0;
  if (tid == 0) s_nw = 0;
  __syncthreads();
  const unsigned long long all_c = ntl >= 64 ? ~0ull : ((1ull << ntl) - 1);
  auto c_tiles = [&](int at, const F0Term& tm, int kc) {
    return mL[at * wl + tm.b] & (FC ? mC[tm.e * nkc + kc] : all_c);
  };
  auto k_tiles = [&](int lt, int f, int kc) {
    return (unsigned)((mR[lt * wr + f] >> (4 * kc)) & 0xfull);
  };
  for (int t = tid; t < ntl * nparts; t += 1024) {
    const int at = t / nparts, sp = t - at * nparts, f = sp / nkc, kc = sp - f * nkc;
    bool any = false;
    for (int q = 0; q < sNT[f]; ++q) any = any || c_tiles(at, sT[f * F0_TMAX + q], kc) != 0;
    if (any) atomicOr(&s1[at], 1ull << sp);
  }
  for (int t = tid; t < ntr * nparts; t += 1024) {
    const int lt = t / nparts, sp = t - lt * nparts, f = sp / nkc, kc = sp - f * nkc;
    if (k_tiles(lt, f, kc)) atomicOr(&s2[lt], 1ull << sp);
  }
  __syncthreads();
  for (int t = tid; t < ntl * d * ntr; t += 1024) {
    const int row = t / ntr, lt = t - row * ntr;
    mask[t] = s1[row / d] & s2[lt];
  }
  auto record = [&](int u, F0Info& I) {
    const int x = u % d, wg0 = u / d, at = wg0 / nparts, sp = wg0 - at * nparts, f = sp / nkc, kc = sp - f * nkc;
    I = F0Info{};
    I.unit = u;
    I.nt = -1;
    int nlt = 0, nct = 0, nt = 0;
    if ((s1[at] >> sp) & 1ull)
      for (int lt = 0; lt < ntr; ++lt)
        if ((s2[lt] >> sp) & 1ull) {
          ++nlt;
          I.lts |= 1ull << lt;
          if (lt < 16) I.frn |= (unsigned long long)k_tiles(lt, f, kc) << (4 * lt);
        }
    if (nlt)
      for (int q = 0; q < sNT[f]; ++q) {
        const F0Term tm = sT[f * F0_TMAX + q];
        if (tm.x != x) continue;
        const unsigned long long c = c_tiles(at, tm, kc);
        nct += __builtin_popcountll(c);
        if (compact && nt < 4) {
          I.cts |= (c & 0xffffull) << (16 * nt);
          I.bpack |= (unsigned)tm.b << (8 * nt), I.epack |= (unsigned)tm.e << (8 * nt), I.w[nt] = tm.w;
        }
        ++nt;
      }
    if (compact) I.nt = nt;
    return nlt ? min(WMAX - 1, 1 + nct + nlt) : 0;
  };
  F0Info mine;
  int myw = 0;
  for (int u = tid; u < nu; u += 1024) {
    F0Info I;
    const int w = record(u, I);
    if (u == tid) mine = I, myw = w;
    atomicAdd(&hist[w], 1);
    if (w) atomicAdd(&s_nw, 1);
  }
  __syncthreads();
  if (tid < WMAX) {
    int acc = 0;
    for (int w = tid + 1; w < WMAX; ++w) acc += hist[w];
    start[tid] = acc;
  }
  __syncthreads();
  const int nw = s_nw;
  for (int u = tid; u < nu; u += 1024) {
    F0Info I;
    int w;
    if (u == tid)
      I = mine, w = myw;
    else
      w = record(u, I);
    const int rank = start[w] + atomicAdd(&hist[w], -1) - 1;
    int pos = rank;
    if (rank >= n_cu && rank < nw) pos = n_cu + (nw - 1 - rank);
    info[pos] = I;
  }
}

__global__ __launch_bounds__(256, 2) void k_heff0_fused(const F0Args g) {
  constexpr int DX = 1;
  constexpr int NW = 4;
  const int tid = threadIdx.x, lane = tid & 63, wave = __builtin_amdgcn_readfirstlane(tid >> 6), x = lane & 15,
            kq = lane >> 4;
  __shared__ double sTr[DX][16 * 65], sTi[DX][16 * 65];
  __shared__ double s_dot[8];
  F0Info I;
  if (g.info) {
    I = g.info[blockIdx.x];
  } else {
    I.unit = (int)blockIdx.x;
    I.nt = -1;
  }
  asm volatile("" ::: "memory");
  if (g.skip && *g.skip) return;
  unsigned long long tr[4] = {0, 0, 0, 0};
  const unsigned long long rt0 = g.trace ? __builtin_amdgcn_s_memrealtime() : 0ull;
  if (g.trace) tr[0] = __builtin_readcyclecounter();
  int tr_ct = 0, tr_lt = 0, tr_x = 0;
  auto trace_out = [&]() {
    if (g.trace && tid == 0) {
      const unsigned long long slot = atomicAdd(g.trace, 1ull);
      if (slot < GEMM_TRACE_CAP) {
        unsigned long long* r = g.trace + 1 + slot * GEMM_TRACE_WORDS;
        const unsigned hw = __builtin_amdgcn_s_getreg((31 << 11) | 4), xc = __builtin_amdgcn_s_getreg((31 << 11) | 20);
        r[0] = ((unsigned long long)(gridDim.x / g.d) << 32) | (unsigned long long)blockIdx.x;
        r[1] = (1ull << 63) | ((unsigned long long)g.d << 32) | (unsigned long long)tr_x;
        r[2] = (unsigned long long)(unsigned)tr_ct | ((unsigned long long)(unsigned)tr_lt << 16) |
               ((unsigned long long)(((xc & 0xf) << 16) | (hw & 0xffff)) << 32);
        r[3] = tr[0], r[4] = tr[1], r[5] = tr[2], r[6] = tr[3];
        r[7] = __builtin_readcyclecounter();
        r[8] = rt0;
        r[9] = __builtin_amdgcn_s_memrealtime();
      }
    }
  };
  const int nparts = g.wr * g.nkc;
  const bool compact = I.nt >= 0;
  const int wg = I.unit;
  const int wg0 = wg / g.d;
  const int xo_wg = wg - wg0 * g.d;
  tr_x = xo_wg;
  const int at = wg0 / nparts, s = wg0 - at * nparts, f = s / g.nkc, kc = s - f * g.nkc;
  const unsigned long long lts =
      compact ? I.lts
              : __ballot(lane < g.ntr && ((g.mask[(long long)at * g.d * g.ntr + min(lane, g.ntr - 1)] >> s) & 1ull));
  if (lts == 0) {
    if (g.dot_part && tid == 0) {
      g.dot_part[2 * wg] = 0.0;
      g.dot_part[2 * wg + 1] = 0.0;
    }
    trace_out();
    return;
  }
  const int wcolt = wave;
  const int a0 = 16 * at, k0 = 64 * kc + 16 * wcolt;
  const bool wcol = k0 < g.Dr;
  unsigned frn = 0;
  if (compact) {
    frn = lane < 16 ? (unsigned)((I.frn >> (4 * lane)) & 0xfull) : 0u;
  } else if (lane < g.ntr) {
#pragma unroll
    for (int jj = 0; jj < 4; ++jj) {
      const int kt = 4 * kc + jj;
      if (kt < g.ntr && g.FR[((long long)lane * g.wr + f) * g.ntr + kt]) frn |= 1u << jj;
    }
  }
  const int lc = min(lane, g.ntl - 1);
  const int nt = compact ? I.nt : g.nterm[f];
  v4d t1[DX], t2[DX], t3[DX];
#pragma unroll
  for (int i = 0; i < DX; ++i) {
    t1[i] = v4d{0, 0, 0, 0};
    t2[i] = v4d{0, 0, 0, 0};
    t3[i] = v4d{0, 0, 0, 0};
  }
  double2 av[3][4], bv[3][4];
  for (int q = 0; q < nt; ++q) {
    int b, te;
    double wv;
    unsigned long long cts;
    if (compact) {
      b = (int)((I.bpack >> (8 * q)) & 0xffu), te = (int)((I.epack >> (8 * q)) & 0xffu);
      wv = q == 0 ? I.w[0] : q == 1 ? I.w[1] : q == 2 ? I.w[2] : I.w[3];
      cts = (I.cts >> (16 * q)) & 0xffffull;
    } else {
      const F0Term tm = g.terms[f * F0_TMAX + q];
      b = tm.b, te = tm.e, wv = tm.w;
      if (tm.x != xo_wg) continue;
      cts = __ballot(lane < g.ntl && g.FL[((long long)at * g.wl + b) * g.ntl + lc] &&
                     (!g.FC || g.FC[(long long)(te * g.nkc + kc) * g.fc_pitch + lc]));
    }
    const double2* La = reinterpret_cast<const double2*>(g.L) + ((long long)(a0 + x) * g.wl + b) * g.Dl + kq;
    const double2* Cb = reinterpret_cast<const double2*>(g.C) + ((long long)kq * g.d + te) * g.Dr + (wcol ? k0 : 0) + x;
    const long long cstride = (long long)g.d * g.Dr;
    auto load1 = [&](int slot, int ct) {
#pragma unroll
      for (int kk = 0; kk < 4; ++kk) {
        const int c = 16 * ct + 4 * kk;
        av[slot][kk] = La[c];
        bv[slot][kk] = Cb[(long long)c * cstride];
      }
    };
    auto mul1 = [&](int slot) {
#pragma unroll
      for (int kk = 0; kk < 4; ++kk) {
        const double ar = av[slot][kk].x * wv, ai = av[slot][kk].y * wv;
#pragma unroll
        for (int i = 0; i < DX; ++i) {
          {
            t1[i] = mfma(ar, bv[slot][kk].x, t1[i]);
            t2[i] = mfma(ai, bv[slot][kk].y, t2[i]);
            t3[i] = mfma(ar + ai, bv[slot][kk].x + bv[slot][kk].y, t3[i]);
          }
        }
      }
    };
    if (g.trace) {
      if (!tr[1]) tr[1] = __builtin_readcyclecounter();
      tr_ct += __builtin_popcountll(cts);
    }
    if (wcol && cts) {
      unsigned long long m = cts;
      auto next_ct = [&]() {
        const int ct = m ? (int)__builtin_ctzll(m) : -1;
        m &= m - (m ? 1 : 0);
        return ct;
      };
      int c0 = next_ct(), c1 = next_ct(), c2 = next_ct();
      if (c0 >= 0) load1(0, c0);
      if (c1 >= 0) load1(1, c1);
      if (c2 >= 0) load1(2, c2);
      while (c0 >= 0) {
        asm volatile("" ::: "memory");
        mul1(0);
        c0 = next_ct();
        if (c0 >= 0) load1(0, c0);
        asm volatile("" ::: "memory");
        if (c1 < 0) break;
        mul1(1);
        c1 = next_ct();
        if (c1 >= 0) load1(1, c1);
        asm volatile("" ::: "memory");
        if (c2 < 0) break;
        mul1(2);
        c2 = next_ct();
        if (c2 >= 0) load1(2, c2);
      }
    }
  }
  if (g.trace) {
    tr[2] = __builtin_readcyclecounter();
    tr_lt = __builtin_popcountll(lts);
  }
  double dre = 0.0, dim = 0.0;
  const double2* Rb = reinterpret_cast<const double2*>(g.Rt) + ((long long)f * g.Dr + 64 * kc + kq) * g.Dr + x;
  double2* part = reinterpret_cast<double2*>(g.parts) + (long long)s * g.n;
  auto nth_tile = [&](unsigned long long m, int n) {
    for (int i = 0; i < n && m; ++i) m &= m - 1;
    return m ? (int)__builtin_ctzll(m) : -1;
  };
  auto k_tiles = [&](int lt) {
    return (unsigned)__builtin_amdgcn_readlane((int)frn, lt);
  };
  double2 rv[2][16], yv2[2][DX][4];
  auto load2 = [&](int slot, int lt) {
#pragma unroll
    for (int ks = 0; ks < 16; ++ks) {
      const long long krow = min((long long)(4 * ks), (long long)(g.Dr - 1 - 64 * kc - kq));
      rv[slot][ks] = Rb[krow * g.Dr + 16 * lt];
    }
    if (g.y) {
#pragma unroll
      for (int i = 0; i < DX; ++i)
#pragma unroll
        for (int r = 0; r < 4; ++r)
          yv2[slot][i][r] =
              reinterpret_cast<const double2*>(g.y)[((long long)(a0 + kq + 4 * r) * g.d + xo_wg) * g.Dr + 16 * lt + x];
    }
  };
  auto mul2 = [&](int slot, int lt, unsigned kts) {
#pragma unroll
    for (int i = 0; i < DX; ++i) {
      v4d o1 = {0, 0, 0, 0}, o2 = {0, 0, 0, 0}, o3 = {0, 0, 0, 0};
#pragma unroll
      for (int ks = 0; ks < 16; ++ks) {
        if ((kts >> (ks >> 2)) & 1u) {
          const double xr = sTr[i][x * 65 + 4 * ks + kq], xi = sTi[i][x * 65 + 4 * ks + kq];
          o1 = mfma(xr, rv[slot][ks].x, o1);
          o2 = mfma(xi, rv[slot][ks].y, o2);
          o3 = mfma(xr + xi, rv[slot][ks].x + rv[slot][ks].y, o3);
        }
      }
      const v4d orr = o1 - o2, oi = o3 - o1 - o2;
#pragma unroll
      for (int r = 0; r < 4; ++r) {
        const long long e = ((long long)(a0 + kq + 4 * r) * g.d + xo_wg) * g.Dr + 16 * lt + x;
        part[e] = make_double2(orr[r], oi[r]);
        if (g.y) {
          const double2 yv = yv2[slot][i][r];
          dre += orr[r] * yv.x + oi[r] * yv.y;
          dim += orr[r] * yv.y - oi[r] * yv.x;
        }
      }
    }
  };
  int idx = wave;
  int lt0 = nth_tile(lts, idx), lt1 = -1;
  unsigned kt0 = 0, kt1 = 0;
  if (lt0 >= 0) {
    kt0 = k_tiles(lt0);
    load2(0, lt0);
  }
  asm volatile("" ::: "memory");
#pragma unroll
  for (int i = 0; i < DX; ++i)
#pragma unroll
    for (int r = 0; r < 4; ++r) {
      sTr[i][(kq + 4 * r) * 65 + 16 * wcolt + x] = t1[i][r] - t2[i][r];
      sTi[i][(kq + 4 * r) * 65 + 16 * wcolt + x] = t3[i][r] - t1[i][r] - t2[i][r];
    }
  __syncthreads();
  while (lt0 >= 0) {
    idx += NW;
    lt1 = nth_tile(lts, idx);
    if (lt1 >= 0) {
      kt1 = k_tiles(lt1);
      load2(1, lt1);
    }
    asm volatile("" ::: "memory");
    mul2(0, lt0, kt0);
    if (lt1 < 0) break;
    idx += NW;
    lt0 = nth_tile(lts, idx);
    if (lt0 >= 0) {
      kt0 = k_tiles(lt0);
      load2(0, lt0);
    }
    asm volatile("" ::: "memory");
    mul2(1, lt1, kt1);
  }
  if (g.trace) tr[3] = __builtin_readcyclecounter();
  if (g.dot_part) {
    dre = wave_sum(dre);
    dim = wave_sum(dim);
    if (lane == 0) {
      s_dot[2 * wave] = dre;
      s_dot[2 * wave + 1] = dim;
    }
    __syncthreads();
    if (tid == 0) {
      double ar = 0.0, ai = 0.0;
#pragma unroll
      for (int w8 = 0; w8 < NW; ++w8) {
        ar += s_dot[2 * w8];
        ai += s_dot[2 * w8 + 1];
      }
      g.dot_part[2 * wg] = ar;
      g.dot_part[2 * wg + 1] = ai;
    }
  }
  trace_out();
}

}

int heff0_fused_parts(const mpse_heff* h, int dtype) {
  static const int mode = [] {
    const char* e = getenv("MPSE_HEFF0");
    return e ? atoi(e) : 1;
  }();
  if (mode == 0 || dtype != MPSE_C128 || h->l_dtype != MPSE_C128 || h->r_dtype != MPSE_C128) return 0;
  const mpse_dims& d = h->dims;
  const int64_t Dl = d.Dl_ket, Dr = d.Dr_ket;
  if (h->nsite == 0) {
    if (d.wr != d.wl) return 0;
  } else if (h->nsite == 1) {
    if (d.d0 != 2 || h->w_dtype != MPSE_F64 || !h->W0 || Dr % 64) return 0;
  } else {
    return 0;
  }
  if ((d.Dl_bra > 0 && d.Dl_bra != Dl) || (d.Dr_bra > 0 && d.Dr_bra != Dr) || d.danc > 1) return 0;
  if (Dl % 16 || Dr % 16 || Dl > 1024 || Dr > 1024 || d.wl < 1 || d.wr < 1 || d.wl > 16 || d.wr > 16) return 0;
  const int64_t min_d = mode >= 2 ? 16 : 128;
  if (Dl < min_d || Dr < min_d) return 0;
  const int64_t nparts = d.wr * ((Dr + 63) / 64);
  if (nparts > 64) return 0;
  return (int)nparts;
}

int heff0_fused_try(mpse_ctx* ctx, int dtype, const mpse_heff* h, const void* C, const double* w_host,
                    SolveScope* sc, MatvecReq* mv, bool* taken) {
  *taken = false;
  const int nparts = heff0_fused_parts(h, dtype);
  if (nparts == 0 || !mv || !mv->parts.ptr || !mv->parts.masked_ok) return MPSE_OK;
  MatvecReq::Parts& pr = mv->parts;
  MatvecReq::Dot* dot = mv->dot.y ? &mv->dot : nullptr;
  const int Dl = (int)h->dims.Dl_ket, Dr = (int)h->dims.Dr_ket, wl = (int)h->dims.wl, wr = (int)h->dims.wr;
  const int d = h->nsite == 1 ? (int)h->dims.d0 : 1;
  if (h->nsite == 1 && !w_host) return MPSE_OK;
  const long long n = (long long)Dl * d * Dr;
  if (pr.n != n || pr.cap_elems < (long long)nparts * n) return MPSE_OK;
  const int ntl = Dl / 16, ntr = Dr / 16, nkc = (Dr + 63) / 64;
  const int nwg = ntl * nparts;
  if (dot && nwg * d > dot->cap) return MPSE_OK;
  std::vector<F0Term> terms(size_t(wr) * F0_TMAX);
  std::vector<int> nterm(wr, 0);
  for (int f = 0; f < wr; ++f) {
    if (h->nsite == 0) {
      terms[size_t(f) * F0_TMAX] = F0Term{f, 0, 0, 0, 1.0};
      nterm[f] = 1;
      continue;
    }
    for (int b = 0; b < wl; ++b)
      for (int x = 0; x < d; ++x)
        for (int e = 0; e < d; ++e) {
          const double v = w_host[((size_t(b) * d + x) * d + e) * wr + f];
          if (v == 0.0) continue;
          if (nterm[f] == F0_TMAX) return MPSE_OK;
          terms[size_t(f) * F0_TMAX + nterm[f]++] = F0Term{b, e, x, 0, v};
        }
  }
  const unsigned char* FC = nullptr;
  int fc_pitch = 0;
  {
    const long long nkw = (ntl + 7) / 8;
    const char* pc = static_cast<const char*>(C);
    if (sc && sc->in_krylov(pc) && sc->cmask.bytes == (long long)d * nkc * nkw * 8) {
      FC = static_cast<const unsigned char*>(sc->cmask.ptr);
      fc_pitch = (int)(nkw * 8);
    }
  }
  const size_t rt_bytes = size_t(wr) * Dr * Dr * 16;
  const size_t fl_bytes = (size_t(ntl) * wl * ntl + 15) & ~size_t(15), fr_bytes = (size_t(ntr) * wr * ntr + 15) & ~size_t(15);
  const size_t tm_bytes = terms.size() * sizeof(F0Term), nt_bytes = (size_t(wr) * sizeof(int) + 15) & ~size_t(15);
  const size_t mk_bytes = size_t(ntl) * d * ntr * 8;
  const size_t nu = size_t(nwg) * d;
  const size_t od_bytes = (nu * sizeof(F0Info) + 15) & ~size_t(15);
  bool compact = ntl <= 16 && ntr <= 16 && wl <= 255 && d <= 255;
  for (int f = 0; f < wr && compact; ++f)
    for (int x = 0; x < d; ++x) {
      int c = 0;
      for (int q = 0; q < nterm[f]; ++q) c += terms[size_t(f) * F0_TMAX + q].x == x;
      if (c > 4) compact = false;
    }
  if (!sc) return MPSE_OK;
  const int* skip = sc->skip;
  SolveScope::F0Cache& fc = sc->f0;
  char* base = nullptr;
  const bool hit = fc.buf && fc.L == h->L && fc.R == h->R && fc.W == h->W0 && fc.cmask == (const void*)FC && fc.Dl == Dl &&
                   fc.Dr == Dr && fc.w == wr && fc.nsite == h->nsite;
  const size_t o_fl = rt_bytes, o_fr = o_fl + fl_bytes, o_tm = o_fr + fr_bytes, o_nt = o_tm + tm_bytes, o_mk = o_nt + nt_bytes;
  const size_t o_od = o_mk + mk_bytes, tot_bytes = o_od + od_bytes;
  static const bool order_on = [] {
    const char* e = getenv("MPSE_F0_ORDER");
    return !(e && e[0] == '0');
  }();
  if (hit) {
    base = static_cast<char*>(fc.buf);
  } else {
    void* p = nullptr;
    if (fc.buf) mpse_free(ctx, fc.buf);
    fc = SolveScope::F0Cache();
    MPSE_TRY(mpse_malloc(ctx, tot_bytes, &p));
    fc.buf = p, fc.L = h->L, fc.R = h->R, fc.W = h->W0, fc.cmask = FC, fc.Dl = Dl, fc.Dr = Dr, fc.w = wr, fc.nsite = h->nsite;
    base = static_cast<char*>(p);
    {
      std::vector<char> up(tm_bytes + nt_bytes, 0);
      memcpy(up.data(), terms.data(), tm_bytes);
      memcpy(up.data() + tm_bytes, nterm.data(), size_t(wr) * sizeof(int));
      MPSE_TRY(stage_h2d(ctx, base + o_tm, up.data(), up.size()));
    }
    const long long nel = (long long)wr * Dr * Dr;
    int nb = (int)((nel + 255) / 256);
    if (nb > 2048) nb = 2048;
    hipLaunchKernelGGL(k_f0_prepare, dim3(ntl * wl + ntr * wr + nb), dim3(256), 0, ctx->stream,
                       static_cast<const double2*>(h->L), static_cast<const double2*>(h->R), reinterpret_cast<double2*>(base),
                       reinterpret_cast<unsigned char*>(base + o_fl), reinterpret_cast<unsigned char*>(base + o_fr), Dl, Dr, wl,
                       wr, ntl, ntr, skip);
    if (order_on)
      hipLaunchKernelGGL(k_f0_plan, dim3(1), dim3(1024), 0, ctx->stream, reinterpret_cast<const unsigned char*>(base + o_fl), FC,
                         reinterpret_cast<const unsigned char*>(base + o_fr), reinterpret_cast<const F0Term*>(base + o_tm),
                         reinterpret_cast<const int*>(base + o_nt), wl, wr, d, ntl, ntr, nkc, fc_pitch,
                         reinterpret_cast<unsigned long long*>(base + o_mk), ctx->n_cu > 0 ? ctx->n_cu : 256,
                         reinterpret_cast<F0Info*>(base + o_od), compact ? 1 : 0, skip);
    else
      hipLaunchKernelGGL(k_f0_valid, dim3(1), dim3(1024), 0, ctx->stream, reinterpret_cast<const unsigned char*>(base + o_fl), FC,
                         reinterpret_cast<const unsigned char*>(base + o_fr), reinterpret_cast<const F0Term*>(base + o_tm),
                         reinterpret_cast<const int*>(base + o_nt), wl, wr, d, ntl, ntr, nkc, fc_pitch,
                         reinterpret_cast<unsigned long long*>(base + o_mk), skip);
  }
  F0Args g{};
  g.L = static_cast<const double*>(h->L);
  g.Rt = reinterpret_cast<const double*>(base);
  g.C = static_cast<const double*>(C);
  g.parts = static_cast<double*>(pr.ptr);
  g.FL = reinterpret_cast<const unsigned char*>(base + o_fl);
  g.FC = FC;
  g.FR = reinterpret_cast<const unsigned char*>(base + o_fr);
  g.terms = reinterpret_cast<const F0Term*>(base + o_tm);
  g.nterm = reinterpret_cast<const int*>(base + o_nt);
  g.mask = reinterpret_cast<const unsigned long long*>(base + o_mk);
  g.skip = skip;
  g.info = order_on ? reinterpret_cast<const F0Info*>(base + o_od) : nullptr;
  g.trace = ctx->prof_on ? ctx->gemm_trace : nullptr;
  g.n = n;
  g.Dl = Dl, g.Dr = Dr, g.wl = wl, g.wr = wr, g.d = d, g.ntl = ntl, g.ntr = ntr, g.nkc = nkc, g.fc_pitch = fc_pitch;
  if (dot) {
    g.y = static_cast<const double*>(dot->y);
    g.dot_part = dot->part;
    dot->nb_out = nwg * d;
  }
  {
    const double fl = h->nsite == 0 ? 8.0 * wr * double(Dl) * Dr * (double(Dl) + Dr)
                                    : 8.0 * double(Dl) * Dl * wl * d * Dr + 4.0 * double(Dl) * Dr * wl * wr * d * d +
                                          8.0 * double(Dl) * Dr * Dr * wr * d;
    const double by = 16.0 * (double(Dl) * wl * Dl + double(Dr) * wr * Dr + 2.0 * double(n));
    ProfScope fprof(ctx, 7, fl, by);
    hipLaunchKernelGGL(k_heff0_fused, dim3(nwg * d), dim3(256), 0, ctx->stream, g);
    fprof.end();
  }
  MPSE_HIP(ctx, hipGetLastError());
  ++ctx->f0_launches[h->nsite == 1 ? 1 : 0];
  pr.used = nparts;
  pr.mask = g.mask;
  pr.mask_row = Dr;
  pr.mask_tiles = ntr;
  *taken = true;
  return MPSE_OK;
}

extern "C" int mpse_heff_fused_stats(mpse_ctx* ctx, int64_t* bond_launches, int64_t* site_launches) {
  if (!ctx) return MPSE_ERR_ARG;
  if (bond_launches) *bond_launches = ctx->f0_launches[0];
  if (site_launches) *site_launches = ctx->f0_launches[1];
  return MPSE_OK;
}
```

### renormalizer_amd/csrc/mpse_internal.h

```cpp
#pragma once
#include <hip/hip_runtime.h>

#include <cstdarg>
#include <cstdlib>
#include <cstdint>
#include <cstdio>
#include <cstring>
#include <functional>
#include <map>
#include <memory>
#include <mutex>
#include <string>
#include <unordered_map>
#include <vector>

#include "../../include/mpsengine.h"

struct mpse_ctx {
  int device = 0;
  hipStream_t stream = nullptr;
  int n_cu = 0;
  char err[512] = {0};
  char dev_name[128] = {0};

  std::mutex pool_mu;
  std::multimap<size_t, void*> free_blocks;
  std::unordered_map<void*, size_t> live;
  size_t pool_bytes = 0;
  size_t in_use_bytes = 0;
  unsigned long long n_device_allocs = 0;

  struct ProfRec {
    hipEvent_t e0, e1;
    int variant;
    double flops, bytes;
  };
  bool prof_on = false;
  int prof_stride = 1;
  long long prof_counter = 0;
  std::vector<ProfRec> prof_pending;
  std::vector<hipEvent_t> prof_free_events;
  static constexpr int PROF_NVAR = 8;
  int64_t prof_svd_sweeps = 0;
  double prof_ms[PROF_NVAR] = {0};
  double prof_flops[PROF_NVAR] = {0};
  double prof_bytes[PROF_NVAR] = {0};
  int64_t prof_launches[PROF_NVAR] = {0};
  unsigned long long* prof_ktiles = nullptr;

  char* stage = nullptr;
  char* stage_dev = nullptr;
  size_t stage_size = 0, stage_pos = 0;

  enum PinnedSlot {
    PIN_SCALAR2 = 0,
    PIN_FLAG = 8,
    PIN_LZ_SCAL = 16,
    PIN_LZ_CTL = 24,
    PIN_ENV_UNIT = 32,
    PIN_PCG_CTL = 40,
    PIN_DAVIDSON = 64,
    PIN_BATCH_CTL = 3700,
    PIN_QR_STATUS = 3990,
    PIN_SLOTS_END = 4000,
    PIN_DOUBLES = 4096,
    PIN_SEQ = PIN_DOUBLES - 1
  };
  double* pinned = nullptr;
  double* pinned_dev = nullptr;
  unsigned long long publish_seq = 0;
  double* dscratch = nullptr;
  unsigned int flag_gen = 0;
  std::unordered_map<unsigned long long, int> lz_hint;
  struct WSiteEntry {
    std::shared_ptr<void> info;
    size_t bytes = 0;
  };
  std::unordered_map<const void*, WSiteEntry> wsite_info;
  std::vector<std::function<int()>> defer_ops[2];
  int defer_recording = -1;
  int defer_armed = -1;
  bool defer_hold = false;
  std::vector<void*> defer_frees;
  struct CMask {
    const void* ptr = nullptr;
    long long bytes = 0;
  } cmask_pending;
  unsigned long long* gemm_trace = nullptr;
  bool gemm_trace_checked = false;
  long long f0_launches[2] = {0, 0};
  enum GemmPath {
    GP_LAUNCH, GP_GENERAL, GP_WIDE, GP_SPLIT_B1, GP_SPLIT_BN, GP_DIE1, GP_DIE2, GP_SKEW, GP_ORDER, GP_MASK,
    GP_MASK_GLOBAL, GP_GROUPED, GP_GROUPED_SPLIT2, GP_GROUPED_MIX, GP_WMIX, GP_GROUPED_OUTMASK, GP_COUNT
  };
  long long gemm_paths[GP_COUNT] = {0};
  long long qr_chol_calls = 0, qr_chol_fallbacks = 0, qr_calls = 0;
  bool qr_optimistic = false;
  int qr_scheme = -1;
  int* qr_words_dev = nullptr;
  long long lz_batch_members = 0, lz_batch_single = 0;
  enum LzPath {
    LP_SYNC, LP_ASYNC_DONE, LP_HOST_FIRST, LP_HOST_LATER, LP_LIMIT, LP_BD_ASYNC, LP_BD_SYNC, LP_FULL, LP_CONV,
    LP_NOCONV, LP_MERGED, LP_WAITS, LP_GROW, LP_PARTS, LP_VMASK, LP_UNVEC, LP_RESCALE, LP_ALIAS_RESTART, LP_COUNT
  };
  long long lz_paths[LP_COUNT] = {0};
  enum PcgStat {
    PS_SOLVES, PS_ITERS, PS_MATVECS, PS_WAITS, PS_END_TOL, PS_END_MAXITER, PS_END_CURVATURE, PS_TWOLAYER, PS_MASKED,
    PS_COUNT
  };
  long long pcg_stats[PS_COUNT] = {0};
  enum PcgSumStat { PSS_SOLVES, PSS_ITERS, PSS_TERM_APPLIES, PSS_WAITS, PSS_DIAGS, PSS_COUNT };
  long long pcg_sum_stats[PSS_COUNT] = {0};
  enum PcgBatchStat { PB_MEMBERS, PB_SINGLE, PB_SETS, PB_MATVEC_LAUNCHES, PB_WAITS, PB_COUNT };
  long long pcg_batch_stats[PB_COUNT] = {0};
  enum OverlapStat { OV_CHAIN, OV_ENQUEUED, OV_SITES, OV_COUNT };
  long long overlap_stats[OV_COUNT] = {0};
  enum SandwichStat { SW_CHAIN, SW_ENQUEUED, SW_SITES, SW_COUNT };
  long long sandwich_stats[SW_COUNT] = {0};
  enum CorrStat { CR_CHAIN, CR_ENQUEUED, CR_SITES, CR_ENTRIES, CR_COUNT };
  long long corr_stats[CR_COUNT] = {0};
  enum Rdm1Stat { RD_CHAIN, RD_ENQUEUED, RD_SITES, RD_MATRICES, RD_COUNT };
  long long rdm1_stats[RD_COUNT] = {0};
  enum Rdm2Stat { RD2_CHAIN, RD2_ENQUEUED, RD2_SITES, RD2_PAIRS, RD2_COUNT };
  long long rdm2_stats[RD2_COUNT] = {0};
};
int qr_words(mpse_ctx* ctx);

int mpse_fail(mpse_ctx* ctx, int code, const char* fmt, ...);
inline int mpse_bind(mpse_ctx* ctx) {
  int cur = -1;
  if (hipGetDevice(&cur) == hipSuccess && cur == ctx->device) return MPSE_OK;
  if (hipSetDevice(ctx->device) != hipSuccess) return mpse_fail(ctx, MPSE_ERR_HIP, "hipSetDevice(%d) failed", ctx->device);
  return MPSE_OK;
}
int stage_h2d(mpse_ctx* ctx, void* dst, const void* src_host, size_t bytes);
int device_zero(mpse_ctx* ctx, void* dst, size_t bytes);
inline void wsite_written(mpse_ctx* ctx, const void* dst, size_t bytes) {
  if (!dst || !bytes) return;
  std::lock_guard<std::mutex> lock(ctx->pool_mu);
  if (ctx->wsite_info.empty()) return;
  const char* lo = static_cast<const char*>(dst);
  for (auto it = ctx->wsite_info.begin(); it != ctx->wsite_info.end();) {
    const char* w = static_cast<const char*>(it->first);
    if (lo < w + it->second.bytes && w < lo + bytes)
      it = ctx->wsite_info.erase(it);
    else
      ++it;
  }
}
void prof_drain(mpse_ctx* ctx);
bool prof_begin(mpse_ctx* ctx, int variant, double flops, double bytes, mpse_ctx::ProfRec* rec);
void prof_end(mpse_ctx* ctx, const mpse_ctx::ProfRec& rec);
struct ProfScope {
  mpse_ctx* ctx;
  mpse_ctx::ProfRec rec;
  bool on;
  ProfScope(mpse_ctx* c, int variant, double flops, double bytes) : ctx(c), on(prof_begin(c, variant, flops, bytes, &rec)) {}
  ProfScope(const ProfScope&) = delete;
  ProfScope& operator=(const ProfScope&) = delete;
  void end() {
    if (on) prof_end(ctx, rec);
    on = false;
  }
  ~ProfScope() {
    if (!on) return;
    ctx->prof_free_events.push_back(rec.e0);
    ctx->prof_free_events.push_back(rec.e1);
  }
};

#define MPSE_HIP(ctx, call)                                                              \
  do {                                                                                   \
    hipError_t _e = (call);                                                              \
    if (_e != hipSuccess)                                                                \
      return mpse_fail((ctx), (_e == hipErrorOutOfMemory) ? MPSE_ERR_OOM : MPSE_ERR_HIP, \
                       "%s:%d %s -> %s", __FILE__, __LINE__, #call, hipGetErrorString(_e)); \
  } while (0)

#define MPSE_TRY(call)            \
  do {                            \
    int _s = (call);              \
    if (_s != MPSE_OK) return _s; \
  } while (0)

#define MPSE_BIND(ctx) MPSE_TRY(mpse_bind(ctx))

template <int COUNT>
static inline int stats_out(const mpse_ctx* ctx, long long (mpse_ctx::*src)[COUNT], int64_t* counts, int n) {
  if (!ctx || n < 0 || (n > 0 && !counts)) return MPSE_ERR_ARG;
  for (int i = 0; i < n; ++i) counts[i] = i < COUNT ? (ctx->*src)[i] : 0;
  return MPSE_OK;
}

#define MPSE_LAUNCH_TF_LDS(ctx, flag, kern, grid, block, lds, ...)                      \
  do {                                                                                  \
    if (flag)                                                                           \
      hipLaunchKernelGGL((kern<true>), grid, block, lds, (ctx)->stream, __VA_ARGS__);   \
    else                                                                                \
      hipLaunchKernelGGL((kern<false>), grid, block, lds, (ctx)->stream, __VA_ARGS__);  \
  } while (0)
#define MPSE_LAUNCH_TF(ctx, flag, kern, grid, block, ...) \
  MPSE_LAUNCH_TF_LDS(ctx, flag, kern, grid, block, 0, __VA_ARGS__)
#define MPSE_LAUNCH_TF_CHK(ctx, ...)     \
  do {                                   \
    MPSE_LAUNCH_TF(ctx, __VA_ARGS__);    \
    MPSE_HIP(ctx, hipGetLastError());    \
  } while (0)

#define MPSE_RECORDING(ctx) ((ctx)->defer_recording >= 0)
int defer_replay(mpse_ctx* ctx, int status);

struct TmpBuf {
  mpse_ctx* ctx;
  void* p = nullptr;
  TmpBuf(mpse_ctx* c) : ctx(c) {}
  int alloc(size_t bytes) { return mpse_malloc(ctx, bytes ? bytes : 16, &p); }
  ~TmpBuf() {
    if (p) mpse_free(ctx, p);
  }
  template <class T>
  T* as() { return reinterpret_cast<T*>(p); }
};

static inline size_t dtype_size(int dt) { return dt == MPSE_C128 ? 16 : 8; }
static inline mpse_index idx1(int64_t ext, int64_t stride) { return mpse_index{ext, ext > 0 ? ext : 1, 0, stride}; }
static inline mpse_index idx2(int64_t hi_ext, int64_t lo_ext, int64_t s_hi, int64_t s_lo) {
  return mpse_index{hi_ext * lo_ext, lo_ext > 0 ? lo_ext : 1, s_hi, s_lo};
}

struct SolveScope {
  mpse_ctx* ctx;
  const int* skip = nullptr;
  bool keeps_env_masks = false;
  const char* env_lo[2] = {nullptr, nullptr};
  const char* env_hi[2] = {nullptr, nullptr};
  mpse_ctx::CMask cmask;
  const char* krylov_lo = nullptr;
  const char* krylov_hi = nullptr;

  struct OccKey {
    const void* ptr;
    long long r_ext, r_lo, r_shi, r_slo, k_ext, k_lo, k_shi, k_slo, sb;
    int nrows, tiles, nkw, batch, K, cplx;
  };
  struct OccEntry {
    OccKey key;
    void* mask;
  };
  std::vector<OccEntry> occ_cache;
  struct PermEntry {
    const void *amask, *bmask;
    int tiles_m, tiles_n, nkt;
    void* perm;
  };
  std::vector<PermEntry> perm_cache;
  struct SmallRt {
    const void* src = nullptr;
    void* rt = nullptr;
    size_t bytes = 0;
  } small_rt;
  struct F0Cache {
    void* buf = nullptr;
    const void *L = nullptr, *R = nullptr, *W = nullptr, *cmask = nullptr;
    int Dl = 0, Dr = 0, w = 0, nsite = -1;
  } f0;

  explicit SolveScope(mpse_ctx* c) : ctx(c) {}
  SolveScope(const SolveScope&) = delete;
  SolveScope& operator=(const SolveScope&) = delete;
  ~SolveScope() {
    for (auto& e : occ_cache) mpse_free(ctx, e.mask);
    for (auto& e : perm_cache) mpse_free(ctx, e.perm);
    if (f0.buf) mpse_free(ctx, f0.buf);
    if (small_rt.rt) mpse_free(ctx, small_rt.rt);
  }
  bool in_env(const void* p) const {
    const char* c = static_cast<const char*>(p);
    return keeps_env_masks && ((c >= env_lo[0] && c < env_hi[0]) || (c >= env_lo[1] && c < env_hi[1]));
  }
  bool in_krylov(const void* p) const {
    const char* c = static_cast<const char*>(p);
    return cmask.ptr && c && c >= krylov_lo && c < krylov_hi;
  }
};

struct MatvecReq {
  struct Dot {
    const void* y = nullptr;
    double* part = nullptr;
    int cap = 0;
    int nb_out = 0;
  } dot;
  struct Parts {
    void* ptr = nullptr;
    long long cap_elems = 0, n = 0;
    int used = 0;
    bool masked_ok = false;
    const unsigned long long* mask = nullptr;
    int mask_row = 0, mask_tiles = 0;
  } parts;
  struct OutMask {
    const unsigned char* mask = nullptr;
    int row = 0, pitch = 0;
  } out_mask;
};

struct ProductReq {
  MatvecReq::Dot* dot = nullptr;
  const void* cin = nullptr;
  mpse_index cin_m{}, cin_n{};
  void* slices = nullptr;
  size_t slices_cap = 0;
  int slices_used = 0;
};

int heff_apply(mpse_ctx* ctx, int dtype, const mpse_heff* h, const void* C, void* out, SolveScope* sc,
               MatvecReq* mv);
int heff_apply2(mpse_ctx* ctx, int dtype, const mpse_heff* h, const void* C, void* out, SolveScope* sc);
int heff_apply_ft(mpse_ctx* ctx, int dtype, const mpse_heff_ft* h, const void* C, void* out, SolveScope* sc);
int heff_small_try(mpse_ctx* ctx, int dtype, const mpse_heff* h, const void* C, void* out, SolveScope* sc,
                   MatvecReq* mv, bool* taken);

struct BatchMember {
  const void* L;
  const void* R;
  const void* W;
  void* Rt;
  const void* C;
  void* out;
};
template <class T>
__host__ __device__ inline T* member_ptr(T* p, unsigned m, long long mstride) {
  return p ? reinterpret_cast<T*>(reinterpret_cast<uintptr_t>(p) + uintptr_t(m) * uintptr_t(mstride)) : p;
}
bool heff_small_batch_plan(const mpse_heff* h, int dtype, int64_t n, int dot_cap, size_t* rt_bytes, int* nparts,
                           int* nb_dot);
int heff_small_batch_rt(mpse_ctx* ctx, int dtype, const mpse_heff* h, int B, const BatchMember* mem, const int* skip0,
                        long long mstride);
int heff_small_batch_apply(mpse_ctx* ctx, int dtype, const mpse_heff* h, int B, const BatchMember* mem,
                           const void* C0, void* parts0, int64_t n, double* dot_part0, int dot_cap, const int* skip0,
                           long long mstride);
constexpr int SM2_WMAX = 8;
constexpr int SM2_DMAX = 16;
constexpr int SM2_BMAX = 64;
constexpr int SM2_LDS_MAX = 65536;
constexpr int SM2_NNZ_LDS = 1024;
struct Small2Plan {
  int Dl, Dr, d, wl, wr;
  int jh, nslice, G;
  int rows, pitch, nnz_lds;
  int ptr_dbl, idx_dbl, csr_dbl;
  int off_A, off_B;
  int lds;
};
struct Pcg2Member {
  const double *L, *R, *W;
  double* Lt;
  int *csr_ptr, *csr_idx;
  double* csr_val;
  const double *mask, *diag, *b;
  double *x, *y, *q, *r, *p;
  double *part_bb, *part_pq, *part_bx, *part_rz0, *part_rz1;
  void* ctl;
  double shift;
};
bool small2_plan(int dtype, int64_t Dl, int64_t d, int64_t Dr, int64_t wl, int64_t wr, Small2Plan* p);
int small2_prep(mpse_ctx* ctx, int dtype, const Small2Plan& p, int B, const Pcg2Member* mem);
int small2_apply(mpse_ctx* ctx, int dtype, const Small2Plan& p, int B, const Pcg2Member* mem, int mode);
int heff0_fused_parts(const mpse_heff* h, int dtype);
int heff0_fused_try(mpse_ctx* ctx, int dtype, const mpse_heff* h, const void* C, const double* w_host,
                    SolveScope* sc, MatvecReq* mv, bool* taken);

int gemm_call(mpse_ctx* ctx, int dta, int dtb, int conja, int conjb, mpse_index ma, mpse_index ka,
              mpse_index kb, mpse_index nb, mpse_index mc, mpse_index nc, int64_t batch, int64_t sba,
              int64_t sbb, int64_t sbc, const void* A, const void* B, void* C, double alpha = 1.0,
              double beta = 0.0, int skip_zero = 0, SolveScope* sc = nullptr, ProductReq* rq = nullptr);

struct GroupedSeg {
  const void* A = nullptr;
  const void* B = nullptr;
  const unsigned char* am = nullptr;
  const unsigned char* bm = nullptr;
};
struct GroupedMixTerm {
  const void* src = nullptr;
  int b = 0, f = 0, delta = 0;
};
struct GroupedGrp {
  GroupedSeg seg[4];
  void* C = nullptr;
  int nseg = 0;
  double beta = 0.0;
};
struct GroupedDesc {
  int dta = MPSE_F64, dtb = MPSE_F64;
  mpse_index ma{}, ka{}, kb{}, nb{}, mc{}, nc{};
  int ngrp = 0;
  GroupedGrp grp[8];
  int am_pitch = 0, bm_pitch = 0;
  bool masks_stable = false;
  bool split2 = false;
  void* c2 = nullptr;
  int nmix = 0, mix_grp = 0;
  GroupedMixTerm mix[8];
  const void* mix_w = nullptr;
  int mix_d = 0, mix_wr = 0;
  long long mix_ld = 0;
};
int gemm_grouped(mpse_ctx* ctx, const GroupedDesc& d, SolveScope* sc, MatvecReq::Dot* dot,
                 const MatvecReq::OutMask* om = nullptr);
int occ_mask_get(mpse_ctx* ctx, SolveScope* sc, const void* ptr, int dtype, mpse_index r, mpse_index k,
                 TmpBuf& tmp, const unsigned char** flags, int* pitch, bool* stable);

int publish_and_wait(mpse_ctx* ctx, const double* dsrc, int count, int slot);
int publish_wait_seq(mpse_ctx* ctx, double seq, const double* dsrc, int count, int slot);
struct PublishAt {
  double* pub;
  volatile double* seq_slot;
  double seq;
};
__attribute__((visibility("hidden"))) PublishAt publish_target(mpse_ctx* ctx, bool wait_here, int slot);
__attribute__((visibility("hidden"))) int publish_collect(mpse_ctx* ctx, const PublishAt& at, const void* dsrc, size_t stride,
                                                          int B, int W, int slot, void* host_out);

int dotc_sync(mpse_ctx* ctx, int dtype, const void* x, const void* y, int64_t n, double* re, double* im);

struct HhParam {
  double tau_re, tau_im;
  double scale_re, scale_im;
  double g[6];
};
struct QrBlk {
  long long ws_off;
  long long q_off;
  int mm, nn, k;
  int prm_off;
  int nq = 0;
  long long row_off = 0, col_off = 0;
};
constexpr int HH_BATCH_MAX_ROWS = 4096;
constexpr unsigned long long GEMM_TRACE_CAP = 1ull << 21;
constexpr int GEMM_TRACE_WORDS = 10;
int hh_qr(mpse_ctx* ctx, bool cplx, double* ws, double* q, HhParam* prm, const QrBlk* blks_host, int nblk, bool form_q,
          const QrBlk* blks_dev = nullptr);
bool cholqr_eligible(const mpse_ctx* ctx, const QrBlk* blks, int nblk);
int cholqr_blocks(mpse_ctx* ctx, bool cplx, double* ws, const QrBlk* blks, int nblk, const long long* drows,
                  const long long* dcols, int herm, void* U, void* Vt, long long K, long long ncol, bool* ok);
int device_zero2(mpse_ctx* ctx, void* a, size_t abytes, void* b, size_t bbytes);
```

### renormalizer_amd/csrc/mpse_qr.hip

```cpp
#include "mpse_cx.h"
#include "mpse_device.h"
#include "mpse_internal.h"

namespace {

template <bool CPLX>
__global__ void k_gather_blocks(double* ws_base, const double* __restrict__ coef, long long ncol,
                                const long long* __restrict__ drows, const long long* __restrict__ dcols,
                                const QrBlk* __restrict__ blks, int herm) {
  const QrBlk B = blks[blockIdx.y];
  double* ws = ws_base + B.ws_off * Cx<CPLX>::E;
  const long long* rows = drows + B.row_off;
  const long long* cols = dcols + B.col_off;
  const int mm = B.mm, nn = B.nn;
  const long long total = (long long)mm * nn;
  const long long stride = (long long)gridDim.x * blockDim.x;
  for (long long t = (long long)blockIdx.x * blockDim.x + threadIdx.x; t < total; t += stride) {
    int r, c;
    if (!herm) {
      c = (int)(t % nn);
      r = (int)(t / nn);
      Cx<CPLX>::st(ws, r + (long long)c * mm, Cx<CPLX>::ld(coef, rows[r] * ncol + cols[c]));
    } else {
      r = (int)(t % mm);
      c = (int)(t / mm);
      double2 v = Cx<CPLX>::ld(coef, rows[c] * ncol + cols[r]);
      v.y = -v.y;
      Cx<CPLX>::st(ws, r + (long long)c * mm, v);
    }
  }
}

template <bool CPLX>
__global__ void k_scatter_blocks(double* U, double* Vt, const double* __restrict__ q_base,
                                 const double* __restrict__ ws_base, long long K, long long ncol,
                                 const long long* __restrict__ drows, const long long* __restrict__ dcols,
                                 const QrBlk* __restrict__ blks, int herm) {
  const QrBlk B = blks[blockIdx.y];
  const double* q = q_base + B.q_off * Cx<CPLX>::E;
  const double* a = ws_base + B.ws_off * Cx<CPLX>::E;
  const long long* rows = drows + B.row_off;
  const long long* cols = dcols + B.col_off;
  const int mm = B.mm, nn = B.nn, k = B.k;
  const long long koff = B.prm_off;
  const long long tq = (long long)mm * k, total = tq + (long long)k * nn;
  const long long stride = (long long)gridDim.x * blockDim.x;
  for (long long t = (long long)blockIdx.x * blockDim.x + threadIdx.x; t < total; t += stride) {
    if (t < tq) {
      if (!herm) {
        const int c = (int)(t % k), r = (int)(t / k);
        Cx<CPLX>::st(U, rows[r] * K + koff + c, Cx<CPLX>::ld(q, r + (long long)c * mm));
      } else {
        const int r = (int)(t % mm), c = (int)(t / mm);
        double2 v = Cx<CPLX>::ld(q, r + (long long)c * mm);
        v.y = -v.y;
        Cx<CPLX>::st(Vt, (koff + c) * ncol + cols[r], v);
      }
    } else {
      const long long u = t - tq;
      const int c = (int)(u % nn), i = (int)(u / nn);
      double2 v = (i <= c) ? Cx<CPLX>::ld(a, i + (long long)c * mm) : make_double2(0.0, 0.0);
      if (!herm) {
        Cx<CPLX>::st(Vt, (koff + i) * ncol + cols[c], v);
      } else {
        v.y = -v.y;
        Cx<CPLX>::st(U, rows[c] * K + koff + i, v);
      }
    }
  }
}

}

int qr_words(mpse_ctx* ctx) {
  if (ctx->qr_words_dev) return MPSE_OK;
  void* p = nullptr;
  MPSE_TRY(mpse_malloc(ctx, 16, &p));
  ctx->qr_words_dev = static_cast<int*>(p);
  return device_zero(ctx, ctx->qr_words_dev, 16);
}

namespace {

template <bool CPLX>
int block_qr_impl(mpse_ctx* ctx, const void* coef, int64_t nrow, int64_t ncol, int nblocks, const int64_t* row_idx,
                  const int64_t* row_off, const int64_t* col_idx, const int64_t* col_off, int herm, bool hh_only, void* U,
                  void* Vt,
                  int64_t K) {
  constexpr size_t es = CPLX ? 16 : 8;
  int64_t ktot = 0, ws_tot = 0, q_tot = 0;
  std::vector<QrBlk> blks;
  std::vector<int> which;
  for (int b = 0; b < nblocks; ++b) {
    const int64_t m = row_off[b + 1] - row_off[b], n = col_off[b + 1] - col_off[b];
    if (m < 0 || n < 0) return mpse_fail(ctx, MPSE_ERR_SHAPE, "block_qr: negative block extent");
    const int64_t k = m < n ? m : n;
    if (k == 0) continue;
    const int64_t mm = herm ? n : m, nn = herm ? m : n;
    blks.push_back(QrBlk{(long long)ws_tot, (long long)q_tot, (int)mm, (int)nn, (int)k, (int)ktot});
    which.push_back(b);
    ws_tot += mm * nn;
    q_tot += mm * k;
    ktot += k;
  }
  if (ktot != K) return mpse_fail(ctx, MPSE_ERR_SHAPE, "block_qr: K=%lld but blocks give %lld", (long long)K, (long long)ktot);
  if (ktot == 0) return mpse_fail(ctx, MPSE_ERR_SHAPE, "Invalid quantum number");
  MPSE_TRY(device_zero2(ctx, U, size_t(nrow * K) * es, Vt, size_t(K * ncol) * es));
  const int64_t nri = row_off[nblocks], nci = col_off[nblocks];
  int64_t max_el = 0, max_sc = 0;
  for (size_t i = 0; i < blks.size(); ++i) {
    blks[i].row_off = row_off[which[i]];
    blks[i].col_off = col_off[which[i]];
    max_el = std::max<int64_t>(max_el, (int64_t)blks[i].mm * blks[i].nn);
    max_sc = std::max<int64_t>(max_sc, (int64_t)blks[i].mm * blks[i].k + (int64_t)blks[i].k * blks[i].nn);
  }
  double qr_flops = 0.0, qr_bytes = 0.0;
  for (const QrBlk& B : blks) {
    const double m = B.mm, n = B.k;
    qr_flops += (CPLX ? 4.0 : 1.0) * (4.0 * m * n * n - 4.0 * n * n * n / 3.0);
    qr_bytes += double(es) * (2.0 * B.mm * B.nn + double(B.mm) * B.k);
  }
  ProfScope qprof(ctx, 5, qr_flops, qr_bytes);
  const size_t ib = size_t(nri + nci) * sizeof(int64_t), db = blks.size() * sizeof(QrBlk);
  static_assert(sizeof(QrBlk) % 8 == 0, "descriptors follow the 8-byte index lists");
  std::vector<char> host(ib + db);
  memcpy(host.data(), row_idx, size_t(nri) * sizeof(int64_t));
  memcpy(host.data() + size_t(nri) * sizeof(int64_t), col_idx, size_t(nci) * sizeof(int64_t));
  memcpy(host.data() + ib, blks.data(), db);
  TmpBuf IDX(ctx), WS(ctx), Q(ctx), PRM(ctx);
  MPSE_TRY(IDX.alloc(ib + db));
  MPSE_TRY(WS.alloc(size_t(ws_tot) * es));
  MPSE_TRY(stage_h2d(ctx, IDX.p, host.data(), ib + db));
  const long long* drows = static_cast<const long long*>(IDX.p);
  const long long* dcols = drows + nri;
  const QrBlk* dblk = reinterpret_cast<const QrBlk*>(static_cast<const char*>(IDX.p) + ib);
  double* ws = static_cast<double*>(WS.p);
  ++ctx->qr_calls;
  hipLaunchKernelGGL((k_gather_blocks<CPLX>), dim3(ew_blocks(max_el), (unsigned)blks.size()), dim3(256), 0, ctx->stream, ws,
                     (const double*)coef, (long long)ncol, drows, dcols, dblk, herm);
  if (!hh_only && cholqr_eligible(ctx, blks.data(), (int)blks.size())) {
    bool ok = false;
    MPSE_TRY(cholqr_blocks(ctx, CPLX, ws, blks.data(), (int)blks.size(), drows, dcols, herm, U, Vt, (long long)K,
                           (long long)ncol, &ok));
    ++ctx->qr_chol_calls;
    if (ok) {
      qprof.end();
      return MPSE_OK;
    }
    ++ctx->qr_chol_fallbacks;
    hipLaunchKernelGGL((k_gather_blocks<CPLX>), dim3(ew_blocks(max_el), (unsigned)blks.size()), dim3(256), 0, ctx->stream,
                       ws, (const double*)coef, (long long)ncol, drows, dcols, dblk, herm);
  }
  MPSE_TRY(Q.alloc(size_t(q_tot) * es));
  MPSE_TRY(PRM.alloc(size_t(ktot + 1) * sizeof(HhParam)));
  double* q = static_cast<double*>(Q.p);
  HhParam* prm = static_cast<HhParam*>(PRM.p);
  MPSE_TRY(hh_qr(ctx, CPLX, ws, q, prm, blks.data(), (int)blks.size(), true, dblk));
  hipLaunchKernelGGL((k_scatter_blocks<CPLX>), dim3(ew_blocks(max_sc), (unsigned)blks.size()), dim3(256), 0, ctx->stream,
                     (double*)U, (double*)Vt, (const double*)q, (const double*)ws, (long long)K, (long long)ncol, drows, dcols,
                     dblk, herm);
  qprof.end();
  MPSE_HIP(ctx, hipGetLastError());
  return MPSE_OK;
}

template <bool CPLX>
__global__ void k_gather_cols(double* out, const double* __restrict__ in, long long nrow, long long ncol_in,
                              const long long* __restrict__ cols, const double* __restrict__ scale, long long ncol_out) {
  const long long total = nrow * ncol_out;
  const long long stride = (long long)gridDim.x * blockDim.x;
  for (long long t = (long long)blockIdx.x * blockDim.x + threadIdx.x; t < total; t += stride) {
    const long long j = t % ncol_out, r = t / ncol_out;
    double2 v = Cx<CPLX>::ld(in, r * ncol_in + cols[j]);
    if (scale) {
      v.x *= scale[j];
      v.y *= scale[j];
    }
    Cx<CPLX>::st(out, t, v);
  }
}

template <bool CPLX>
__global__ void k_gather_rows(double* out, const double* __restrict__ in, long long ncol,
                              const long long* __restrict__ rows, const double* __restrict__ scale, long long nrow_out) {
  const long long total = nrow_out * ncol;
  const long long stride = (long long)gridDim.x * blockDim.x;
  for (long long t = (long long)blockIdx.x * blockDim.x + threadIdx.x; t < total; t += stride) {
    const long long j = t % ncol, r = t / ncol;
    double2 v = Cx<CPLX>::ld(in, rows[r] * ncol + j);
    if (scale) {
      v.x *= scale[r];
      v.y *= scale[r];
    }
    Cx<CPLX>::st(out, t, v);
  }
}

}

extern "C" {

int mpse_block_qr(mpse_ctx* ctx, int dtype, const void* coef, int64_t nrow, int64_t ncol, int nblocks,
                  const int64_t* row_idx_host, const int64_t* row_off_host, const int64_t* col_idx_host,
                  const int64_t* col_off_host, int system_is_R, void* U, void* Vt, int64_t K) {
  if (!ctx || !coef || !U || !Vt || !row_idx_host || !row_off_host || !col_idx_host || !col_off_host)
    return MPSE_ERR_ARG;
  if (MPSE_RECORDING(ctx) && nblocks > 0) {
    std::vector<int64_t> roff(row_off_host, row_off_host + nblocks + 1), coff(col_off_host, col_off_host + nblocks + 1);
    std::vector<int64_t> ridx(row_idx_host, row_idx_host + roff[nblocks]), cidx(col_idx_host, col_idx_host + coff[nblocks]);
    ctx->defer_ops[ctx->defer_recording].push_back(
        [ctx, dtype, coef, nrow, ncol, nblocks, ridx = std::move(ridx), roff = std::move(roff), cidx = std::move(cidx),
         coff = std::move(coff), system_is_R, U, Vt, K] {
          return mpse_block_qr(ctx, dtype, coef, nrow, ncol, nblocks, ridx.data(), roff.data(), cidx.data(), coff.data(),
                               system_is_R, U, Vt, K);
        });
    return MPSE_OK;
  }
  MPSE_BIND(ctx);
  if (nblocks <= 0) return mpse_fail(ctx, MPSE_ERR_SHAPE, "Invalid quantum number");
  if (system_is_R < 0 || system_is_R > 3) return mpse_fail(ctx, MPSE_ERR_ARG, "block_qr: system_is_R = %d", system_is_R);
  if (dtype == MPSE_C128)
    return block_qr_impl<true>(ctx, coef, nrow, ncol, nblocks, row_idx_host, row_off_host, col_idx_host, col_off_host,
                               system_is_R & 1, (system_is_R & 2) != 0, U, Vt, K);
  if (dtype == MPSE_F64)
    return block_qr_impl<false>(ctx, coef, nrow, ncol, nblocks, row_idx_host, row_off_host, col_idx_host,
                                col_off_host, system_is_R & 1, (system_is_R & 2) != 0, U, Vt, K);
  return mpse_fail(ctx, MPSE_ERR_ARG, "block_qr: unknown dtype");
}

int mpse_block_qr_optimistic(mpse_ctx* ctx, int on) {
  if (!ctx) return MPSE_ERR_ARG;
  MPSE_BIND(ctx);
  MPSE_TRY(qr_words(ctx));
  MPSE_TRY(device_zero(ctx, ctx->qr_words_dev, 8));
  ctx->qr_optimistic = on != 0;
  return MPSE_OK;
}

int mpse_block_qr_scheme(mpse_ctx* ctx, int scheme) {
  if (!ctx || scheme < -1 || scheme > 2) return MPSE_ERR_ARG;
  ctx->qr_scheme = scheme;
  return MPSE_OK;
}

int mpse_block_qr_check(mpse_ctx* ctx, int* tripped) {
  if (!ctx || !tripped) return MPSE_ERR_ARG;
  MPSE_BIND(ctx);
  *tripped = 0;
  if (!ctx->qr_words_dev || !ctx->qr_optimistic) return MPSE_OK;
  int v[4] = {0, 0, 0, 0};
  MPSE_TRY(mpse_memcpy_d2h(ctx, v, ctx->qr_words_dev, 16));
  *tripped = v[0] != 0;
  return MPSE_OK;
}

int mpse_block_qr_pass_stats(mpse_ctx* ctx, int64_t* blocks, int64_t* two_pass) {
  if (!ctx) return MPSE_ERR_ARG;
  MPSE_BIND(ctx);
  int v[4] = {0, 0, 0, 0};
  if (ctx->qr_words_dev) MPSE_TRY(mpse_memcpy_d2h(ctx, v, ctx->qr_words_dev, 16));
  if (blocks) *blocks = v[2];
  if (two_pass) *two_pass = v[3];
  return MPSE_OK;
}

int mpse_block_qr_stats(mpse_ctx* ctx, int64_t* calls, int64_t* chol_calls, int64_t* chol_fallbacks) {
  if (!ctx) return MPSE_ERR_ARG;
  if (calls) *calls = ctx->qr_calls;
  if (chol_calls) *chol_calls = ctx->qr_chol_calls;
  if (chol_fallbacks) *chol_fallbacks = ctx->qr_chol_fallbacks;
  return MPSE_OK;
}

int mpse_gather_cols(mpse_ctx* ctx, int dtype, void* out, const void* in, int64_t nrow, int64_t ncol_in,
                     const int64_t* cols_host, const double* scale_host, int64_t ncol_out) {
  if (!ctx || !cols_host || (nrow * ncol_out && (!out || !in))) return MPSE_ERR_ARG;
  MPSE_BIND(ctx);
  if (nrow * ncol_out <= 0) return MPSE_OK;
  wsite_written(ctx, out, size_t(nrow) * size_t(ncol_out) * dtype_size(dtype));
  TmpBuf IDX(ctx);
  MPSE_TRY(IDX.alloc(size_t(ncol_out) * 16));
  MPSE_TRY(stage_h2d(ctx, IDX.p, cols_host, size_t(ncol_out) * 8));
  double* dscale = nullptr;
  if (scale_host) {
    dscale = IDX.as<double>() + ncol_out;
    MPSE_TRY(stage_h2d(ctx, dscale, scale_host, size_t(ncol_out) * 8));
  }
  const int nb = ew_blocks(nrow * ncol_out);
  if (dtype == MPSE_C128)
    hipLaunchKernelGGL((k_gather_cols<true>), dim3(nb), dim3(256), 0, ctx->stream, (double*)out, (const double*)in,
                       (long long)nrow, (long long)ncol_in, IDX.as<const long long>(), (const double*)dscale,
                       (long long)ncol_out);
  else
    hipLaunchKernelGGL((k_gather_cols<false>), dim3(nb), dim3(256), 0, ctx->stream, (double*)out, (const double*)in,
                       (long long)nrow, (long long)ncol_in, IDX.as<const long long>(), (const double*)dscale,
                       (long long)ncol_out);
  MPSE_HIP(ctx, hipGetLastError());
  return MPSE_OK;
}

int mpse_gather_rows(mpse_ctx* ctx, int dtype, void* out, const void* in, int64_t ncol, const int64_t* rows_host,
                     const double* scale_host, int64_t nrow_out) {
  if (!ctx || !rows_host || (nrow_out * ncol && (!out || !in))) return MPSE_ERR_ARG;
  MPSE_BIND(ctx);
  if (nrow_out * ncol <= 0) return MPSE_OK;
  wsite_written(ctx, out, size_t(nrow_out) * size_t(ncol) * dtype_size(dtype));
  TmpBuf IDX(ctx);
  MPSE_TRY(IDX.alloc(size_t(nrow_out) * 16));
  MPSE_TRY(stage_h2d(ctx, IDX.p, rows_host, size_t(nrow_out) * 8));
  double* dscale = nullptr;
  if (scale_host) {
    dscale = IDX.as<double>() + nrow_out;
    MPSE_TRY(stage_h2d(ctx, dscale, scale_host, size_t(nrow_out) * 8));
  }
  const int nb = ew_blocks(nrow_out * ncol);
  if (dtype == MPSE_C128)
    hipLaunchKernelGGL((k_gather_rows<true>), dim3(nb), dim3(256), 0, ctx->stream, (double*)out, (const double*)in,
                       (long long)ncol, IDX.as<const long long>(), (const double*)dscale, (long long)nrow_out);
  else
    hipLaunchKernelGGL((k_gather_rows<false>), dim3(nb), dim3(256), 0, ctx->stream, (double*)out, (const double*)in,
                       (long long)ncol, IDX.as<const long long>(), (const double*)dscale, (long long)nrow_out);
  MPSE_HIP(ctx, hipGetLastError());
  return MPSE_OK;
}

}
```

Measured before the change: 604.0.

## Hoist QR and fused-matvec host setup out of launch path and cache term tables

Block QR now runs a prepare phase (index staging, descriptor upload, CholQR buffer allocation) when the call is recorded, and only the launch runs when deferred ops replay. The fused heff0 matvec caches its term table on the device per W site or bond instead of rebuilding and uploading it on every call. The tile-order kernel gains a word-wide flag computation path, with the old byte path kept behind an env var. The intent is to cut host-side setup and H2D traffic from the sweep's critical path, at the cost of keeping buffers alive longer and added cache-invalidation complexity.

```diff
diff --git a/renormalizer_amd/csrc/mpse_cholqr.hip b/renormalizer_amd/csrc/mpse_cholqr.hip
--- a/renormalizer_amd/csrc/mpse_cholqr.hip
+++ b/renormalizer_amd/csrc/mpse_cholqr.hip
@@ -813,16 +813,17 @@
   }
 }
 
-template <bool CPLX>
-int cholqr_run(mpse_ctx* ctx, double* ws, const QrBlk* blks, int nblk, const long long* drows, const long long* dcols,
-               int herm, void* U, void* Vt, long long K, long long ncol, bool* ok) {
+}
+
+int cholqr_prepare(mpse_ctx* ctx, bool cplx, const QrBlk* blks, int nblk, CholqrPrep* pp) {
+  CholqrPrep& P = *pp;
   MPSE_TRY(qr_words(ctx));
-  int* gflag = ctx->qr_optimistic ? ctx->qr_words_dev : nullptr;
-  constexpr size_t es = CPLX ? 16 : 8;
+  const size_t es = cplx ? 16 : 8;
   std::vector<CqBlk> cb(nblk);
   long long part_tot = 0, t_tot = 0;
-  int max_gram = 1, max_T = 1, max_nrb = 1, max_P = 1;
-  long long max_sc = 1;
+  int &max_gram = P.max_gram, &max_T = P.max_T, &max_nrb = P.max_nrb, &max_P = P.max_P;
+  long long& max_sc = P.max_sc;
+  max_gram = max_T = max_nrb = max_P = 1, max_sc = 1;
   long long groups = 0;
   for (int b = 0; b < nblk; ++b) {
     const int P2 = ((blks[b].nn + 15) / 16 + 1) / 2;
@@ -860,13 +861,27 @@
     max_nrb = std::max(max_nrb, (c.mm + 15) / 16);
     max_sc = std::max<long long>(max_sc, (long long)c.mm * c.nn + (long long)c.nn * c.nn);
   }
-  const size_t db = (size_t(nblk) * sizeof(CqBlk) + 15) & ~size_t(15);
-  const size_t pb = size_t(part_tot) * es, tb = size_t(t_tot) * 256 * es, ib = size_t(t_tot) * 2 * sizeof(double);
-  const size_t sb = ((2 * size_t(nblk) + 1) * sizeof(int) + 15) & ~size_t(15);
-  TmpBuf M(ctx);
-  MPSE_TRY(M.alloc(db + pb + 6 * tb + ib + sb + 16));
-  char* base = static_cast<char*>(M.p);
-  MPSE_TRY(stage_h2d(ctx, base, cb.data(), size_t(nblk) * sizeof(CqBlk)));
+  P.db = (size_t(nblk) * sizeof(CqBlk) + 15) & ~size_t(15);
+  P.pb = size_t(part_tot) * es, P.tb = size_t(t_tot) * 256 * es, P.ib = size_t(t_tot) * 2 * sizeof(double);
+  P.sb = ((2 * size_t(nblk) + 1) * sizeof(int) + 15) & ~size_t(15);
+  MPSE_TRY(P.M.alloc(P.db + P.pb + 6 * P.tb + P.ib + P.sb + 16));
+  MPSE_TRY(stage_h2d(ctx, P.M.p, cb.data(), size_t(nblk) * sizeof(CqBlk)));
+  P.nblk = nblk;
+  P.cplx = cplx;
+  P.ready = true;
+  return MPSE_OK;
+}
+
+namespace {
+
+template <bool CPLX>
+int cholqr_run(mpse_ctx* ctx, double* ws, const CholqrPrep& P, const long long* drows, const long long* dcols, int herm,
+               void* U, void* Vt, long long K, long long ncol, bool* ok) {
+  int* gflag = ctx->qr_optimistic ? ctx->qr_words_dev : nullptr;
+  const int nblk = P.nblk, max_gram = P.max_gram, max_T = P.max_T, max_nrb = P.max_nrb, max_P = P.max_P;
+  const long long max_sc = P.max_sc;
+  const size_t db = P.db, pb = P.pb, tb = P.tb, ib = P.ib, sb = P.sb;
+  char* base = static_cast<char*>(P.M.p);
   const CqBlk* dblk = reinterpret_cast<const CqBlk*>(base);
   double* part = reinterpret_cast<double*>(base + db);
   double* G = reinterpret_cast<double*>(base + db + pb);
@@ -943,9 +958,10 @@
   return max_mm >= min_rows && max_nn >= 96;
 }
 
-int cholqr_blocks(mpse_ctx* ctx, bool cplx, double* ws, const QrBlk* blks, int nblk, const long long* drows,
-                  const long long* dcols, int herm, void* U, void* Vt, long long K, long long ncol, bool* ok) {
+int cholqr_blocks(mpse_ctx* ctx, double* ws, const CholqrPrep& prep, const long long* drows, const long long* dcols,
+                  int herm, void* U, void* Vt, long long K, long long ncol, bool* ok) {
   *ok = false;
-  if (cplx) return cholqr_run<true>(ctx, ws, blks, nblk, drows, dcols, herm, U, Vt, K, ncol, ok);
-  return cholqr_run<false>(ctx, ws, blks, nblk, drows, dcols, herm, U, Vt, K, ncol, ok);
-}
+  if (!prep.ready) return mpse_fail(ctx, MPSE_ERR_ARG, "cholqr: not prepared");
+  if (prep.cplx) return cholqr_run<true>(ctx, ws, prep, drows, dcols, herm, U, Vt, K, ncol, ok);
+  return cholqr_run<false>(ctx, ws, prep, drows, dcols, herm, U, Vt, K, ncol, ok);
+}
diff --git a/renormalizer_amd/csrc/mpse_core.hip b/renormalizer_amd/csrc/mpse_core.hip
--- a/renormalizer_amd/csrc/mpse_core.hip
+++ b/renormalizer_amd/csrc/mpse_core.hip
@@ -307,6 +307,8 @@
   if (!ctx) return MPSE_ERR_ARG;
   (void)hipSetDevice(ctx->device);
   (void)hipStreamSynchronize(ctx->stream);
+  ctx->defer_ops[0].clear();
+  ctx->defer_ops[1].clear();
   prof_drain(ctx);
   for (auto e : ctx->prof_free_events) (void)hipEventDestroy(e);
   for (auto& kv : ctx->free_blocks) (void)hipFree(kv.second);
diff --git a/renormalizer_amd/csrc/mpse_gemm.hip b/renormalizer_amd/csrc/mpse_gemm.hip
--- a/renormalizer_amd/csrc/mpse_gemm.hip
+++ b/renormalizer_amd/csrc/mpse_gemm.hip
@@ -923,12 +923,20 @@
   while (n < x) n <<= 1;
   return n;
 }
+__device__ __forceinline__ unsigned long long flag_word(const unsigned char* p, int n) {
+  const unsigned long long addr = (unsigned long long)p;
+  const int sh = (int)(addr & 7ull) * 8;
+  const unsigned long long* w = reinterpret_cast<const unsigned long long*>(addr - (addr & 7ull));
+  unsigned long long x = w[0] >> sh;
+  if (sh + 8 * n > 64) x |= w[1] << (64 - sh);
+  return n < 8 ? x & ((1ull << (8 * n)) - 1ull) : x;
+}
 __global__ __launch_bounds__(1024) void k_tile_order(const unsigned long long* __restrict__ amask,
                                                        const unsigned long long* __restrict__ bmask, int nkw, int nkt,
                                                        int tiles_m, int tiles_n, int by_die, int* __restrict__ perm,
                                                        const int* __restrict__ skip, const GemmGroups gg,
                                                        unsigned char* __restrict__ flags_out, int flags_pitch,
-                                                       int om_M, int om_N) {
+                                                       int om_M, int om_N, int by_bytes) {
   if (skip && *skip) return;
   __shared__ unsigned key[2048], ckey[2048];
   __shared__ int colw[2048];
@@ -947,16 +955,63 @@
         const GGrp& G = gg.g[grp];
         const bool off = gg.omask && !mpse_plan::out_tile_live(gg.omask, gg.om_pitch, gg.om_d, om_N, om_M, tm, tn);
         dead[i] = off ? 1 : 0;
-        for (int q = 0; q < G.nseg; ++q)
-          for (int l = 0; l < gg.nkt_seg; ++l) {
-            unsigned v = off ? 0 : 1;
-            if (G.seg[q].am) v &= G.seg[q].am[(long long)tml * gg.am_pitch + l];
-            if (G.seg[q].bm) v &= G.seg[q].bm[(long long)tn * gg.bm_pitch + l];
-            cnt += v;
-            if (flags_out) flags_out[(long long)i * flags_pitch + q * gg.nkt_seg + l] = (unsigned char)v;
+        if (by_bytes) {
+          for (int q = 0; q < G.nseg; ++q)
+            for (int l = 0; l < gg.nkt_seg; ++l) {
+              unsigned v = off ? 0 : 1;
+              if (G.seg[q].am) v &= G.seg[q].am[(long long)tml * gg.am_pitch + l];
+              if (G.seg[q].bm) v &= G.seg[q].bm[(long long)tn * gg.bm_pitch + l];
+              cnt += v;
+              if (flags_out) flags_out[(long long)i * flags_pitch + q * gg.nkt_seg + l] = (unsigned char)v;
+            }
+          if (flags_out)
+            for (int l = G.nseg * gg.nkt_seg; l < flags_pitch; ++l) flags_out[(long long)i * flags_pitch + l] = 0;
+        } else {
+          const int cps = (gg.nkt_seg + 7) >> 3, nch = G.nseg * cps;
+          unsigned long long* fo =
+              flags_out ? reinterpret_cast<unsigned long long*>(flags_out + (long long)i * flags_pitch) : nullptr;
+          unsigned long long acc = 0;
+          int fill = 0, wpos = 0;
+          for (int c0 = 0; c0 < nch; c0 += 8) {
+            unsigned long long x[8];
+#pragma unroll
+            for (int j = 0; j < 8; ++j) {
+              x[j] = 0;
+              const int ch = c0 + j;
+              if (ch < nch && !off) {
+                const int q = ch / cps, l0 = (ch - q * cps) * 8;
+                const int n = gg.nkt_seg - l0 < 8 ? gg.nkt_seg - l0 : 8;
+                unsigned long long v = 0x0101010101010101ull;
+                if (n < 8) v &= (1ull << (8 * n)) - 1ull;
+                if (G.seg[q].am) v &= flag_word(G.seg[q].am + (long long)tml * gg.am_pitch + l0, n);
+                if (G.seg[q].bm) v &= flag_word(G.seg[q].bm + (long long)tn * gg.bm_pitch + l0, n);
+                x[j] = v;
+              }
+            }
+#pragma unroll
+            for (int j = 0; j < 8; ++j) {
+              const int ch = c0 + j;
+              if (ch >= nch) break;
+              const int l0 = (ch % cps) * 8;
+              const int n = gg.nkt_seg - l0 < 8 ? gg.nkt_seg - l0 : 8;
+              cnt += __popcll(x[j]);
+              if (fo) {
+                acc |= x[j] << (8 * fill);
+                if (fill + n >= 8) {
+                  fo[wpos++] = acc;
+                  acc = fill ? x[j] >> (8 * (8 - fill)) : 0ull;
+                  fill += n - 8;
+                } else {
+                  fill += n;
+                }
+              }
+            }
           }
-        if (flags_out)
-          for (int l = G.nseg * gg.nkt_seg; l < flags_pitch; ++l) flags_out[(long long)i * flags_pitch + l] = 0;
+          if (fo) {
+            if (fill) fo[wpos++] = acc;
+            for (; wpos < flags_pitch / 8; ++wpos) fo[wpos] = 0ull;
+          }
+        }
       } else {
         for (int w = 0; w < nkw; ++w) {
           unsigned long long x = 0x0101010101010101ull;
@@ -1435,7 +1490,7 @@
                          size_t(g.tiles_m) * g.tiles_n * sizeof(int), PERM, &pp, &sort));
     if (sort)
       hipLaunchKernelGGL(k_tile_order, dim3(1), dim3(1024), 0, ctx->stream, g.amask, g.bmask, g.nkw, p.nkt, g.tiles_m,
-                         g.tiles_n, 1, pp, g.skip, GemmGroups(), (unsigned char*)nullptr, 0, 0, 0);
+                         g.tiles_n, 1, pp, g.skip, GemmGroups(), (unsigned char*)nullptr, 0, 0, 0, 0);
     g.perm = pp;
   }
 
@@ -1595,10 +1650,15 @@
                          {gg.g[0].seg[0].am, gg.g[0].seg[0].bm, g.tiles_m, g.tiles_n,
                           nkt_max + 1000 * d.ngrp + (out_mask ? 1000000 : 0), nullptr},
                          perm_bytes + size_t(ntile) * flag_pitch, PERM, &pp, &sort));
+    static const bool by_bytes = [] {
+      const char* e = getenv("MPSE_TILE_ORDER_BYTES");
+      return e && e[0] == '1';
+    }();
     if (sort)
       hipLaunchKernelGGL(k_tile_order, dim3(1), dim3(1024), 0, ctx->stream, (const unsigned long long*)nullptr,
                          (const unsigned long long*)nullptr, 0, nkt_max, g.tiles_m, g.tiles_n, d.split2 ? 0 : 1, pp,
-                         g.skip, gg, reinterpret_cast<unsigned char*>(pp) + perm_bytes, (int)flag_pitch, g.M, g.N);
+                         g.skip, gg, reinterpret_cast<unsigned char*>(pp) + perm_bytes, (int)flag_pitch, g.M, g.N,
+                         by_bytes ? 1 : 0);
     g.perm = pp;
     g.gg.flags = reinterpret_cast<const unsigned long long*>(reinterpret_cast<const char*>(pp) + perm_bytes);
   }
diff --git a/renormalizer_amd/csrc/mpse_heff0.hip b/renormalizer_amd/csrc/mpse_heff0.hip
--- a/renormalizer_amd/csrc/mpse_heff0.hip
+++ b/renormalizer_amd/csrc/mpse_heff0.hip
@@ -1,5 +1,6 @@
 #include "mpse_device.h"
 #include "mpse_internal.h"
+#include "mpse_plans.h"
 
 typedef double v4d __attribute__((ext_vector_type(4)));
 
@@ -508,6 +509,86 @@
   trace_out();
 }
 
+struct F0TermTable {
+  void* dev = nullptr;
+  bool dense = false;
+  bool compact = true;
+  ~F0TermTable() {
+    if (dev) (void)hipFree(dev);
+  }
+};
+
+int f0_term_table(mpse_ctx* ctx, const mpse_heff* h, const double* w_host, int wl, int d, int wr,
+                  std::shared_ptr<F0TermTable>* out) {
+  const bool site = h->nsite == 1;
+  {
+    std::lock_guard<std::mutex> lock(ctx->pool_mu);
+    std::shared_ptr<void> have;
+    if (site) {
+      auto it = ctx->wsite_info.find(h->W0);
+      if (it != ctx->wsite_info.end() && static_cast<const mpse_plan::WSiteInfo*>(it->second.info.get())->w.data() == w_host)
+        have = it->second.f0_terms;
+    } else {
+      have = ctx->f0_bond_terms[wr];
+    }
+    if (have) {
+      *out = std::static_pointer_cast<F0TermTable>(have);
+      return MPSE_OK;
+    }
+  }
+  auto tab = std::make_shared<F0TermTable>();
+  std::vector<F0Term> terms(size_t(wr) * F0_TMAX);
+  std::vector<int> nterm(wr, 0);
+  for (int f = 0; f < wr && !tab->dense; ++f) {
+    if (!site) {
+      terms[size_t(f) * F0_TMAX] = F0Term{f, 0, 0, 0, 1.0};
+      nterm[f] = 1;
+      continue;
+    }
+    for (int b = 0; b < wl && !tab->dense; ++b)
+      for (int x = 0; x < d && !tab->dense; ++x)
+        for (int e = 0; e < d; ++e) {
+          const double v = w_host[((size_t(b) * d + x) * d + e) * wr + f];
+          if (v == 0.0) continue;
+          if (nterm[f] == F0_TMAX) {
+            tab->dense = true;
+            break;
+          }
+          terms[size_t(f) * F0_TMAX + nterm[f]++] = F0Term{b, e, x, 0, v};
+        }
+  }
+  if (!tab->dense) {
+    for (int f = 0; f < wr; ++f)
+      for (int x = 0; x < d; ++x) {
+        int c = 0;
+        for (int q = 0; q < nterm[f]; ++q) c += terms[size_t(f) * F0_TMAX + q].x == x;
+        if (c > 4) tab->compact = false;
+      }
+    const size_t tm_bytes = terms.size() * sizeof(F0Term), nt_bytes = (size_t(wr) * sizeof(int) + 15) & ~size_t(15);
+    std::vector<char> up(tm_bytes + nt_bytes, 0);
+    memcpy(up.data(), terms.data(), tm_bytes);
+    memcpy(up.data() + tm_bytes, nterm.data(), size_t(wr) * sizeof(int));
+    if (hipMalloc(&tab->dev, up.size()) != hipSuccess) {
+      (void)hipGetLastError();
+      tab->dev = nullptr;
+      return mpse_fail(ctx, MPSE_ERR_OOM, "fused matvec: no memory for the term table");
+    }
+    MPSE_TRY(stage_h2d(ctx, tab->dev, up.data(), up.size()));
+  }
+  {
+    std::lock_guard<std::mutex> lock(ctx->pool_mu);
+    if (site) {
+      auto it = ctx->wsite_info.find(h->W0);
+      if (it != ctx->wsite_info.end() && static_cast<const mpse_plan::WSiteInfo*>(it->second.info.get())->w.data() == w_host)
+        it->second.f0_terms = tab;
+    } else {
+      ctx->f0_bond_terms[wr] = tab;
+    }
+  }
+  *out = tab;
+  return MPSE_OK;
+}
+
 }
 
 int heff0_fused_parts(const mpse_heff* h, int dtype) {
@@ -549,23 +630,10 @@
   const int ntl = Dl / 16, ntr = Dr / 16, nkc = (Dr + 63) / 64;
   const int nwg = ntl * nparts;
   if (dot && nwg * d > dot->cap) return MPSE_OK;
-  std::vector<F0Term> terms(size_t(wr) * F0_TMAX);
-  std::vector<int> nterm(wr, 0);
-  for (int f = 0; f < wr; ++f) {
-    if (h->nsite == 0) {
-      terms[size_t(f) * F0_TMAX] = F0Term{f, 0, 0, 0, 1.0};
-      nterm[f] = 1;
-      continue;
-    }
-    for (int b = 0; b < wl; ++b)
-      for (int x = 0; x < d; ++x)
-        for (int e = 0; e < d; ++e) {
-          const double v = w_host[((size_t(b) * d + x) * d + e) * wr + f];
-          if (v == 0.0) continue;
-          if (nterm[f] == F0_TMAX) return MPSE_OK;
-          terms[size_t(f) * F0_TMAX + nterm[f]++] = F0Term{b, e, x, 0, v};
-        }
-  }
+  if (!sc) return MPSE_OK;
+  std::shared_ptr<F0TermTable> tab;
+  MPSE_TRY(f0_term_table(ctx, h, w_host, wl, d, wr, &tab));
+  if (tab->dense) return MPSE_OK;
   const unsigned char* FC = nullptr;
   int fc_pitch = 0;
   {
@@ -578,23 +646,18 @@
   }
   const size_t rt_bytes = size_t(wr) * Dr * Dr * 16;
   const size_t fl_bytes = (size_t(ntl) * wl * ntl + 15) & ~size_t(15), fr_bytes = (size_t(ntr) * wr * ntr + 15) & ~size_t(15);
-  const size_t tm_bytes = terms.size() * sizeof(F0Term), nt_bytes = (size_t(wr) * sizeof(int) + 15) & ~size_t(15);
+  const size_t tm_bytes = size_t(wr) * F0_TMAX * sizeof(F0Term), nt_bytes = (size_t(wr) * sizeof(int) + 15) & ~size_t(15);
+  const F0Term* const d_terms = static_cast<const F0Term*>(tab->dev);
+  const int* const d_nterm = reinterpret_cast<const int*>(static_cast<const char*>(tab->dev) + tm_bytes);
   const size_t mk_bytes = size_t(ntl) * d * ntr * 8;
   const size_t nu = size_t(nwg) * d;
   const size_t od_bytes = (nu * sizeof(F0Info) + 15) & ~size_t(15);
-  bool compact = ntl <= 16 && ntr <= 16 && wl <= 255 && d <= 255;
-  for (int f = 0; f < wr && compact; ++f)
-    for (int x = 0; x < d; ++x) {
-      int c = 0;
-      for (int q = 0; q < nterm[f]; ++q) c += terms[size_t(f) * F0_TMAX + q].x == x;
-      if (c > 4) compact = false;
-    }
-  if (!sc) return MPSE_OK;
+  const bool compact = ntl <= 16 && ntr <= 16 && wl <= 255 && d <= 255 && tab->compact;
   const int* skip = sc->skip;
   SolveScope::F0Cache& fc = sc->f0;
   char* base = nullptr;
   const bool hit = fc.buf && fc.L == h->L && fc.R == h->R && fc.W == h->W0 && fc.cmask == (const void*)FC && fc.Dl == Dl &&
-                   fc.Dr == Dr && fc.w == wr && fc.nsite == h->nsite;
+                   fc.Dr == Dr && fc.w == wr && fc.nsite == h->nsite && fc.terms == tab;
   const size_t o_fl = rt_bytes, o_fr = o_fl + fl_bytes, o_tm = o_fr + fr_bytes, o_nt = o_tm + tm_bytes, o_mk = o_nt + nt_bytes;
   const size_t o_od = o_mk + mk_bytes, tot_bytes = o_od + od_bytes;
   static const bool order_on = [] {
@@ -609,13 +672,8 @@
     fc = SolveScope::F0Cache();
     MPSE_TRY(mpse_malloc(ctx, tot_bytes, &p));
     fc.buf = p, fc.L = h->L, fc.R = h->R, fc.W = h->W0, fc.cmask = FC, fc.Dl = Dl, fc.Dr = Dr, fc.w = wr, fc.nsite = h->nsite;
+    fc.terms = tab;
     base = static_cast<char*>(p);
-    {
-      std::vector<char> up(tm_bytes + nt_bytes, 0);
-      memcpy(up.data(), terms.data(), tm_bytes);
-      memcpy(up.data() + tm_bytes, nterm.data(), size_t(wr) * sizeof(int));
-      MPSE_TRY(stage_h2d(ctx, base + o_tm, up.data(), up.size()));
-    }
     const long long nel = (long long)wr * Dr * Dr;
     int nb = (int)((nel + 255) / 256);
     if (nb > 2048) nb = 2048;
@@ -625,14 +683,12 @@
                        wr, ntl, ntr, skip);
     if (order_on)
       hipLaunchKernelGGL(k_f0_plan, dim3(1), dim3(1024), 0, ctx->stream, reinterpret_cast<const unsigned char*>(base + o_fl), FC,
-                         reinterpret_cast<const unsigned char*>(base + o_fr), reinterpret_cast<const F0Term*>(base + o_tm),
-                         reinterpret_cast<const int*>(base + o_nt), wl, wr, d, ntl, ntr, nkc, fc_pitch,
+                         reinterpret_cast<const unsigned char*>(base + o_fr), d_terms, d_nterm, wl, wr, d, ntl, ntr, nkc, fc_pitch,
                          reinterpret_cast<unsigned long long*>(base + o_mk), ctx->n_cu > 0 ? ctx->n_cu : 256,
                          reinterpret_cast<F0Info*>(base + o_od), compact ? 1 : 0, skip);
     else
       hipLaunchKernelGGL(k_f0_valid, dim3(1), dim3(1024), 0, ctx->stream, reinterpret_cast<const unsigned char*>(base + o_fl), FC,
-                         reinterpret_cast<const unsigned char*>(base + o_fr), reinterpret_cast<const F0Term*>(base + o_tm),
-                         reinterpret_cast<const int*>(base + o_nt), wl, wr, d, ntl, ntr, nkc, fc_pitch,
+                         reinterpret_cast<const unsigned char*>(base + o_fr), d_terms, d_nterm, wl, wr, d, ntl, ntr, nkc, fc_pitch,
                          reinterpret_cast<unsigned long long*>(base + o_mk), skip);
   }
   F0Args g{};
@@ -643,8 +699,8 @@
   g.FL = reinterpret_cast<const unsigned char*>(base + o_fl);
   g.FC = FC;
   g.FR = reinterpret_cast<const unsigned char*>(base + o_fr);
-  g.terms = reinterpret_cast<const F0Term*>(base + o_tm);
-  g.nterm = reinterpret_cast<const int*>(base + o_nt);
+  g.terms = d_terms;
+  g.nterm = d_nterm;
   g.mask = reinterpret_cast<const unsigned long long*>(base + o_mk);
   g.skip = skip;
   g.info = order_on ? reinterpret_cast<const F0Info*>(base + o_od) : nullptr;
diff --git a/renormalizer_amd/csrc/mpse_internal.h b/renormalizer_amd/csrc/mpse_internal.h
--- a/renormalizer_amd/csrc/mpse_internal.h
+++ b/renormalizer_amd/csrc/mpse_internal.h
@@ -75,8 +75,10 @@
   struct WSiteEntry {
     std::shared_ptr<void> info;
     size_t bytes = 0;
+    std::shared_ptr<void> f0_terms;
   };
   std::unordered_map<const void*, WSiteEntry> wsite_info;
+  std::shared_ptr<void> f0_bond_terms[17];
   std::vector<std::function<int()>> defer_ops[2];
   int defer_recording = -1;
   int defer_armed = -1;
@@ -263,6 +265,7 @@
     void* buf = nullptr;
     const void *L = nullptr, *R = nullptr, *W = nullptr, *cmask = nullptr;
     int Dl = 0, Dr = 0, w = 0, nsite = -1;
+    std::shared_ptr<void> terms;
   } f0;
 
   explicit SolveScope(mpse_ctx* c) : ctx(c) {}
@@ -443,7 +446,16 @@
 constexpr int GEMM_TRACE_WORDS = 10;
 int hh_qr(mpse_ctx* ctx, bool cplx, double* ws, double* q, HhParam* prm, const QrBlk* blks_host, int nblk, bool form_q,
           const QrBlk* blks_dev = nullptr);
+struct CholqrPrep {
+  TmpBuf M;
+  size_t db = 0, pb = 0, tb = 0, ib = 0, sb = 0;
+  int nblk = 0, max_gram = 1, max_T = 1, max_nrb = 1, max_P = 1;
+  long long max_sc = 1;
+  bool cplx = false, ready = false;
+  explicit CholqrPrep(mpse_ctx* c) : M(c) {}
+};
 bool cholqr_eligible(const mpse_ctx* ctx, const QrBlk* blks, int nblk);
-int cholqr_blocks(mpse_ctx* ctx, bool cplx, double* ws, const QrBlk* blks, int nblk, const long long* drows,
-                  const long long* dcols, int herm, void* U, void* Vt, long long K, long long ncol, bool* ok);
+int cholqr_prepare(mpse_ctx* ctx, bool cplx, const QrBlk* blks, int nblk, CholqrPrep* prep);
+int cholqr_blocks(mpse_ctx* ctx, double* ws, const CholqrPrep& prep, const long long* drows, const long long* dcols,
+                  int herm, void* U, void* Vt, long long K, long long ncol, bool* ok);
 int device_zero2(mpse_ctx* ctx, void* a, size_t abytes, void* b, size_t bbytes);
diff --git a/renormalizer_amd/csrc/mpse_qr.hip b/renormalizer_amd/csrc/mpse_qr.hip
--- a/renormalizer_amd/csrc/mpse_qr.hip
+++ b/renormalizer_amd/csrc/mpse_qr.hip
@@ -82,14 +82,29 @@
 
 namespace {
 
-template <bool CPLX>
-int block_qr_impl(mpse_ctx* ctx, const void* coef, int64_t nrow, int64_t ncol, int nblocks, const int64_t* row_idx,
-                  const int64_t* row_off, const int64_t* col_idx, const int64_t* col_off, int herm, bool hh_only, void* U,
-                  void* Vt,
-                  int64_t K) {
-  constexpr size_t es = CPLX ? 16 : 8;
-  int64_t ktot = 0, ws_tot = 0, q_tot = 0;
+struct QrPrepared {
+  mpse_ctx* ctx;
+  bool cplx = false, hh_only = false;
+  int herm = 0;
+  const void* coef = nullptr;
+  void *U = nullptr, *Vt = nullptr;
+  int64_t nrow = 0, ncol = 0, K = 0;
   std::vector<QrBlk> blks;
+  int64_t ws_tot = 0, q_tot = 0, nri = 0, max_el = 0, max_sc = 0;
+  size_t ib = 0;
+  double qr_flops = 0.0, qr_bytes = 0.0;
+  TmpBuf IDX, WS;
+  CholqrPrep chol;
+  explicit QrPrepared(mpse_ctx* c) : ctx(c), IDX(c), WS(c), chol(c) {}
+};
+
+int block_qr_prepare(QrPrepared& P, int nblocks, const int64_t* row_idx, const int64_t* row_off, const int64_t* col_idx,
+                     const int64_t* col_off) {
+  mpse_ctx* ctx = P.ctx;
+  const size_t es = P.cplx ? 16 : 8;
+  const int herm = P.herm;
+  int64_t ktot = 0;
+  std::vector<QrBlk>& blks = P.blks;
   std::vector<int> which;
   for (int b = 0; b < nblocks; ++b) {
     const int64_t m = row_off[b + 1] - row_off[b], n = col_off[b + 1] - col_off[b];
@@ -97,66 +112,80 @@
     const int64_t k = m < n ? m : n;
     if (k == 0) continue;
     const int64_t mm = herm ? n : m, nn = herm ? m : n;
-    blks.push_back(QrBlk{(long long)ws_tot, (long long)q_tot, (int)mm, (int)nn, (int)k, (int)ktot});
+    blks.push_back(QrBlk{(long long)P.ws_tot, (long long)P.q_tot, (int)mm, (int)nn, (int)k, (int)ktot});
     which.push_back(b);
-    ws_tot += mm * nn;
-    q_tot += mm * k;
+    P.ws_tot += mm * nn;
+    P.q_tot += mm * k;
     ktot += k;
   }
-  if (ktot != K) return mpse_fail(ctx, MPSE_ERR_SHAPE, "block_qr: K=%lld but blocks give %lld", (long long)K, (long long)ktot);
+  if (ktot != P.K)
+    return mpse_fail(ctx, MPSE_ERR_SHAPE, "block_qr: K=%lld but blocks give %lld", (long long)P.K, (long long)ktot);
   if (ktot == 0) return mpse_fail(ctx, MPSE_ERR_SHAPE, "Invalid quantum number");
-  MPSE_TRY(device_zero2(ctx, U, size_t(nrow * K) * es, Vt, size_t(K * ncol) * es));
   const int64_t nri = row_off[nblocks], nci = col_off[nblocks];
-  int64_t max_el = 0, max_sc = 0;
+  P.nri = nri;
   for (size_t i = 0; i < blks.size(); ++i) {
     blks[i].row_off = row_off[which[i]];
     blks[i].col_off = col_off[which[i]];
-    max_el = std::max<int64_t>(max_el, (int64_t)blks[i].mm * blks[i].nn);
-    max_sc = std::max<int64_t>(max_sc, (int64_t)blks[i].mm * blks[i].k + (int64_t)blks[i].k * blks[i].nn);
-  }
-  double qr_flops = 0.0, qr_bytes = 0.0;
+    P.max_el = std::max<int64_t>(P.max_el, (int64_t)blks[i].mm * blks[i].nn);
+    P.max_sc = std::max<int64_t>(P.max_sc, (int64_t)blks[i].mm * blks[i].k + (int64_t)blks[i].k * blks[i].nn);
+  }
   for (const QrBlk& B : blks) {
     const double m = B.mm, n = B.k;
-    qr_flops += (CPLX ? 4.0 : 1.0) * (4.0 * m * n * n - 4.0 * n * n * n / 3.0);
-    qr_bytes += double(es) * (2.0 * B.mm * B.nn + double(B.mm) * B.k);
-  }
-  ProfScope qprof(ctx, 5, qr_flops, qr_bytes);
+    P.qr_flops += (P.cplx ? 4.0 : 1.0) * (4.0 * m * n * n - 4.0 * n * n * n / 3.0);
+    P.qr_bytes += double(es) * (2.0 * B.mm * B.nn + double(B.mm) * B.k);
+  }
   const size_t ib = size_t(nri + nci) * sizeof(int64_t), db = blks.size() * sizeof(QrBlk);
+  P.ib = ib;
   static_assert(sizeof(QrBlk) % 8 == 0, "descriptors follow the 8-byte index lists");
   std::vector<char> host(ib + db);
   memcpy(host.data(), row_idx, size_t(nri) * sizeof(int64_t));
   memcpy(host.data() + size_t(nri) * sizeof(int64_t), col_idx, size_t(nci) * sizeof(int64_t));
   memcpy(host.data() + ib, blks.data(), db);
-  TmpBuf IDX(ctx), WS(ctx), Q(ctx), PRM(ctx);
-  MPSE_TRY(IDX.alloc(ib + db));
-  MPSE_TRY(WS.alloc(size_t(ws_tot) * es));
-  MPSE_TRY(stage_h2d(ctx, IDX.p, host.data(), ib + db));
-  const long long* drows = static_cast<const long long*>(IDX.p);
-  const long long* dcols = drows + nri;
-  const QrBlk* dblk = reinterpret_cast<const QrBlk*>(static_cast<const char*>(IDX.p) + ib);
-  double* ws = static_cast<double*>(WS.p);
+  MPSE_TRY(P.IDX.alloc(ib + db));
+  MPSE_TRY(P.WS.alloc(size_t(P.ws_tot) * es));
+  MPSE_TRY(stage_h2d(ctx, P.IDX.p, host.data(), ib + db));
+  if (!P.hh_only && cholqr_eligible(ctx, blks.data(), (int)blks.size()))
+    MPSE_TRY(cholqr_prepare(ctx, P.cplx, blks.data(), (int)blks.size(), &P.chol));
+  return MPSE_OK;
+}
+
+template <bool CPLX>
+int block_qr_launch(QrPrepared& P) {
+  constexpr size_t es = CPLX ? 16 : 8;
+  mpse_ctx* ctx = P.ctx;
+  const std::vector<QrBlk>& blks = P.blks;
+  const int herm = P.herm;
+  const int64_t K = P.K, ncol = P.ncol;
+  void *U = P.U, *Vt = P.Vt;
+  MPSE_TRY(device_zero2(ctx, U, size_t(P.nrow * K) * es, Vt, size_t(K * ncol) * es));
+  ProfScope qprof(ctx, 5, P.qr_flops, P.qr_bytes);
+  TmpBuf Q(ctx), PRM(ctx);
+  const long long* drows = static_cast<const long long*>(P.IDX.p);
+  const long long* dcols = drows + P.nri;
+  const QrBlk* dblk = reinterpret_cast<const QrBlk*>(static_cast<const char*>(P.IDX.p) + P.ib);
+  double* ws = static_cast<double*>(P.WS.p);
   ++ctx->qr_calls;
-  hipLaunchKernelGGL((k_gather_blocks<CPLX>), dim3(ew_blocks(max_el), (unsigned)blks.size()), dim3(256), 0, ctx->stream, ws,
-                     (const double*)coef, (long long)ncol, drows, dcols, dblk, herm);
-  if (!hh_only && cholqr_eligible(ctx, blks.data(), (int)blks.size())) {
+  hipLaunchKernelGGL((k_gather_blocks<CPLX>), dim3(ew_blocks(P.max_el), (unsigned)blks.size()), dim3(256), 0, ctx->stream,
+                     ws, (const double*)P.coef, (long long)ncol, drows, dcols, dblk, herm);
+  if (!P.hh_only && cholqr_eligible(ctx, blks.data(), (int)blks.size())) {
     bool ok = false;
-    MPSE_TRY(cholqr_blocks(ctx, CPLX, ws, blks.data(), (int)blks.size(), drows, dcols, herm, U, Vt, (long long)K,
-                           (long long)ncol, &ok));
+    if (!P.chol.ready) MPSE_TRY(cholqr_prepare(ctx, CPLX, blks.data(), (int)blks.size(), &P.chol));
+    MPSE_TRY(cholqr_blocks(ctx, ws, P.chol, drows, dcols, herm, U, Vt, (long long)K, (long long)ncol, &ok));
     ++ctx->qr_chol_calls;
     if (ok) {
       qprof.end();
       return MPSE_OK;
     }
     ++ctx->qr_chol_fallbacks;
-    hipLaunchKernelGGL((k_gather_blocks<CPLX>), dim3(ew_blocks(max_el), (unsigned)blks.size()), dim3(256), 0, ctx->stream,
-                       ws, (const double*)coef, (long long)ncol, drows, dcols, dblk, herm);
-  }
-  MPSE_TRY(Q.alloc(size_t(q_tot) * es));
-  MPSE_TRY(PRM.alloc(size_t(ktot + 1) * sizeof(HhParam)));
+    hipLaunchKernelGGL((k_gather_blocks<CPLX>), dim3(ew_blocks(P.max_el), (unsigned)blks.size()), dim3(256), 0, ctx->stream,
+                       ws, (const double*)P.coef, (long long)ncol, drows, dcols, dblk, herm);
+  }
+  MPSE_TRY(Q.alloc(size_t(P.q_tot) * es));
+  MPSE_TRY(PRM.alloc(size_t(K + 1) * sizeof(HhParam)));
   double* q = static_cast<double*>(Q.p);
   HhParam* prm = static_cast<HhParam*>(PRM.p);
   MPSE_TRY(hh_qr(ctx, CPLX, ws, q, prm, blks.data(), (int)blks.size(), true, dblk));
-  hipLaunchKernelGGL((k_scatter_blocks<CPLX>), dim3(ew_blocks(max_sc), (unsigned)blks.size()), dim3(256), 0, ctx->stream,
+  hipLaunchKernelGGL((k_scatter_blocks<CPLX>), dim3(ew_blocks(P.max_sc), (unsigned)blks.size()), dim3(256), 0, ctx->stream,
                      (double*)U, (double*)Vt, (const double*)q, (const double*)ws, (long long)K, (long long)ncol, drows, dcols,
                      dblk, herm);
   qprof.end();
@@ -205,27 +234,24 @@
                   const int64_t* col_off_host, int system_is_R, void* U, void* Vt, int64_t K) {
   if (!ctx || !coef || !U || !Vt || !row_idx_host || !row_off_host || !col_idx_host || !col_off_host)
     return MPSE_ERR_ARG;
-  if (MPSE_RECORDING(ctx) && nblocks > 0) {
-    std::vector<int64_t> roff(row_off_host, row_off_host + nblocks + 1), coff(col_off_host, col_off_host + nblocks + 1);
-    std::vector<int64_t> ridx(row_idx_host, row_idx_host + roff[nblocks]), cidx(col_idx_host, col_idx_host + coff[nblocks]);
-    ctx->defer_ops[ctx->defer_recording].push_back(
-        [ctx, dtype, coef, nrow, ncol, nblocks, ridx = std::move(ridx), roff = std::move(roff), cidx = std::move(cidx),
-         coff = std::move(coff), system_is_R, U, Vt, K] {
-          return mpse_block_qr(ctx, dtype, coef, nrow, ncol, nblocks, ridx.data(), roff.data(), cidx.data(), coff.data(),
-                               system_is_R, U, Vt, K);
-        });
-    return MPSE_OK;
-  }
   MPSE_BIND(ctx);
   if (nblocks <= 0) return mpse_fail(ctx, MPSE_ERR_SHAPE, "Invalid quantum number");
   if (system_is_R < 0 || system_is_R > 3) return mpse_fail(ctx, MPSE_ERR_ARG, "block_qr: system_is_R = %d", system_is_R);
-  if (dtype == MPSE_C128)
-    return block_qr_impl<true>(ctx, coef, nrow, ncol, nblocks, row_idx_host, row_off_host, col_idx_host, col_off_host,
-                               system_is_R & 1, (system_is_R & 2) != 0, U, Vt, K);
-  if (dtype == MPSE_F64)
-    return block_qr_impl<false>(ctx, coef, nrow, ncol, nblocks, row_idx_host, row_off_host, col_idx_host,
-                                col_off_host, system_is_R & 1, (system_is_R & 2) != 0, U, Vt, K);
-  return mpse_fail(ctx, MPSE_ERR_ARG, "block_qr: unknown dtype");
+  if (dtype != MPSE_C128 && dtype != MPSE_F64) return mpse_fail(ctx, MPSE_ERR_ARG, "block_qr: unknown dtype");
+  auto prep = std::make_shared<QrPrepared>(ctx);
+  prep->cplx = dtype == MPSE_C128, prep->herm = system_is_R & 1, prep->hh_only = (system_is_R & 2) != 0;
+  prep->coef = coef, prep->U = U, prep->Vt = Vt, prep->nrow = nrow, prep->ncol = ncol, prep->K = K;
+  MPSE_TRY(block_qr_prepare(*prep, nblocks, row_idx_host, row_off_host, col_idx_host, col_off_host));
+  auto launch = [](QrPrepared& p) { return p.cplx ? block_qr_launch<true>(p) : block_qr_launch<false>(p); };
+  if (MPSE_RECORDING(ctx)) {
+    ctx->defer_ops[ctx->defer_recording].push_back([prep, launch]() mutable {
+      const int st = launch(*prep);
+      prep.reset();
+      return st;
+    });
+    return MPSE_OK;
+  }
+  return launch(*prep);
 }
 
 int mpse_block_qr_optimistic(mpse_ctx* ctx, int on) {
```

Result: no change. 603.8 (-0.0%).
